# NRCan/geo-deep-learning

Hardware: AMD Instinct MI355X
Metric: 512x512 tiles/s, DOFA-base + UperNet, train step (higher is better)
Workload: dtype bf16; 1 GPU; DOFA-base + UperNet, 3-band 512x512 (configs[1]): training step = fwd + Dice(main)+0.4*Dice(aux) + bwd + clip 1.0 + Adam 6e-5, encoder frozen, DropPat; per_gpu_batch=64, global_batch=64, num_classes=5, parallelism=dp1, weights=random init, inputs_resident_in_hbm=True

## Files before the change

### geo-deep-learning_amd/csrc/attention_v2.hip

```cpp
#include "gdl_common.h"

namespace {

typedef __attribute__((ext_vector_type(4))) short s16x4_t;
typedef __attribute__((ext_vector_type(8))) short s16x8_t;
typedef __attribute__((address_space(3))) s16x4_t* lds_s16x4_ptr;

constexpr unsigned kOob = 0x80000000u;
constexpr int TILE_BYTES = 64 * 128;

__device__ __forceinline__ int tr_swz(int row) { return (((row >> 1) & 1) << 2) | ((row >> 2) & 3); }

__device__ __forceinline__ void decode_block(int nblk, int BH, int& blk, int& bh) {
  const int id = blockIdx.x;
  if ((BH & 7) == 0) {
    const int j = id >> 3;
    bh = (id & 7) + 8 * (j / nblk);
    blk = j % nblk;
  } else {
    bh = id / nblk;
    blk = id % nblk;
  }
}

struct Attn2Args {
  const uint16_t *q, *k, *v, *o, *dout;
  uint16_t *out, *dq, *dk, *dv;
  int64_t q_sB, q_sN, k_sB, k_sN, v_sB, v_sN, o_sB, o_sN, do_sB, do_sN;
  int64_t dq_sB, dq_sN, dk_sB, dk_sN, dv_sB, dv_sN;
  float* lse;
  float* dvec;
  int B, H, Nq, N;
  float scale, scale_log2e;
  int qsplit;
  float* dkv_part;
};

__device__ __forceinline__ void stage_piece(const srd_t& srd, int64_t tok_stride_bytes, int tok0, int ntok, int piece,
                                            unsigned lds_tile, int lane) {
  const int r = piece * 8 + (lane >> 3);
  const int chunk = (lane & 7) ^ tr_swz(r);
  const int tok = tok0 + r;
  const unsigned v = tok < ntok ? (unsigned)(tok * tok_stride_bytes + chunk * 16) : kOob;
  dma16_buf(v, srd, 0u, lds_tile + piece * 1024);
}

__device__ __forceinline__ bf16x8_t row_frag(const unsigned char* tile, int rt, int kk, int lane) {
  const int row = rt * 32 + (lane & 31);
  const uint4 v = *(const uint4*)(tile + row * 128 + (((2 * kk + (lane >> 5)) ^ tr_swz(row)) << 4));
  return __builtin_bit_cast(bf16x8_t, v);
}

__device__ __forceinline__ bf16x8_t col_frag(const unsigned char* tile, int ct, int tt, int s, int lane) {
  const int g = lane >> 4, l = lane & 15;
  const int ch = 32 * ct + 16 * (g & 1) + 4 * (l & 3);
  const int t0 = 32 * tt + 16 * s + 4 * (g >> 1) + (l >> 2);
  const unsigned char* p0 = tile + t0 * 128 + (((ch >> 3) ^ tr_swz(t0)) << 4) + (ch & 7) * 2;
  const int t1 = t0 + 8;
  const unsigned char* p1 = tile + t1 * 128 + (((ch >> 3) ^ tr_swz(t1)) << 4) + (ch & 7) * 2;
  const s16x4_t lo = __builtin_amdgcn_ds_read_tr16_b64_v4i16((lds_s16x4_ptr)p0);
  const s16x4_t hi = __builtin_amdgcn_ds_read_tr16_b64_v4i16((lds_s16x4_ptr)p1);
  const s16x8_t v = {lo[0], lo[1], lo[2], lo[3], hi[0], hi[1], hi[2], hi[3]};
  return __builtin_bit_cast(bf16x8_t, v);
}

__device__ __forceinline__ bf16x8_t acc_as_b(const f32x16_t& a, int s) {
  bf16x8_t r;
#pragma unroll
// ... 127 lines not shown
          ot[1][ct] = MFMA(va, pb1, ot[1][ct]);
        }
      }
  }
  if (!active) return;
#pragma unroll
  for (int qt = 0; qt < 2; ++qt) {
    const float l = l_run[qt] + __shfl_xor(l_run[qt], 32, 64);
    const float inv = 1.f / l;
    const int q = q0 + qt * 32 + frow;
    if (q >= f.Nq) continue;
    if (f.lse && fhalf == 0)
      f.lse[(int64_t)bh * f.Nq + q] = (m_run[qt] * f.scale_log2e + __builtin_amdgcn_logf(l)) * 0.6931471805599453f;
    uint16_t* orow = f.out + (int64_t)b * f.o_sB + (int64_t)q * f.o_sN + (int64_t)h * 64;
#pragma unroll
    for (int ct = 0; ct < 2; ++ct)
#pragma unroll
      for (int g = 0; g < 4; ++g) {
        const int d = ct * 32 + 8 * g + 4 * fhalf;
        *(uint2*)(orow + d) = make_uint2(pack_bf16x2(ot[qt][ct][4 * g] * inv, ot[qt][ct][4 * g + 1] * inv),
                                         pack_bf16x2(ot[qt][ct][4 * g + 2] * inv, ot[qt][ct][4 * g + 3] * inv));
      }
  }
}

template <int NW>
__global__ __launch_bounds__(64 * NW) __attribute__((amdgpu_waves_per_eu(NW == 2 ? 2 : 4, 4))) void flash_fwd3_kernel(const Attn2Args f, const float defer) {
  __shared__ __attribute__((aligned(16))) unsigned char smem[4 * TILE_BYTES];
  const int lane = threadIdx.x & 63;
  const int wave = __builtin_amdgcn_readfirstlane(threadIdx.x >> 6);
  int blk, bh;
  decode_block((f.Nq + 32 * NW - 1) / (32 * NW), f.B * f.H, blk, bh);
  const int b = bh / f.H, h = bh % f.H;
  const int q0 = blk * (32 * NW) + wave * 32;
  const bool active = q0 < f.Nq;
  const int frow = lane & 31, fhalf = lane >> 5;
  const uint16_t* qbase = f.q + (int64_t)b * f.q_sB + (int64_t)h * 64;
  const srd_t srd_k = make_srd(f.k + (int64_t)b * f.k_sB + (int64_t)h * 64, (unsigned)(((int64_t)f.N - 1) * f.k_sN * 2 + 128));
  const srd_t srd_v = make_srd(f.v + (int64_t)b * f.v_sB + (int64_t)h * 64, (unsigned)(((int64_t)f.N - 1) * f.v_sN * 2 + 128));
  const unsigned lds_base = __builtin_amdgcn_readfirstlane((unsigned)(size_t)(__attribute__((address_space(3))) void*)smem);

  bf16x8_t qf[4];
  {
    const int q = q0 + frow;
#pragma unroll
    for (int kk = 0; kk < 4; ++kk) {
      uint4 v = make_uint4(0, 0, 0, 0);
      if (q < f.Nq) v = *(const uint4*)(qbase + (int64_t)q * f.q_sN + kk * 16 + fhalf * 8);
      qf[kk] = __builtin_bit_cast(bf16x8_t, v);
    }
  }
  auto issue = [&](int stage, int kv0) {
#pragma unroll
    for (int i = 0; i < (8 + NW - 1) / NW; ++i) {
      const int p = wave + NW * i;
      if (p < 8) {
        stage_piece(srd_k, f.k_sN * 2, kv0, f.N, p, lds_base + (2 * stage) * TILE_BYTES, lane);
        stage_piece(srd_v, f.v_sN * 2, kv0, f.N, p, lds_base + (2 * stage + 1) * TILE_BYTES, lane);
      }
    }
  };
  f32x16_t ot[2] = {zero16(), zero16()};
  float m_run = -INFINITY, l_run = 0.f;
  const float sl2 = f.scale_log2e;
  const int ntiles = (f.N + 63) / 64;
  issue(0, 0);
// ... 431 lines not shown
    const float4 v = *(const float4*)(p + s * plane);
    a.x += v.x; a.y += v.y; a.z += v.z; a.w += v.w;
  }
  const int b = bh / f.H, h = bh % f.H;
  const bool is_v = d4 >= 16;
  const int d = (d4 & 15) * 4;
  uint16_t* dst = is_v ? f.dv + (int64_t)b * f.dv_sB + (int64_t)key * f.dv_sN + (int64_t)h * 64 + d
                       : f.dk + (int64_t)b * f.dk_sB + (int64_t)key * f.dk_sN + (int64_t)h * 64 + d;
  *(uint2*)dst = make_uint2(pack_bf16x2(a.x, a.y), pack_bf16x2(a.z, a.w));
}

int dkv_qsplit(int B, int H, int Nq, int Nkv) {
  const int64_t base = (int64_t)((Nkv + 127) / 128) * B * H;
  const int ntiles = (Nq + 63) / 64;
  int64_t s = (512 + base - 1) / base;
  if (s > ntiles / 4) s = ntiles / 4;
  if (s > 16) s = 16;
  return s < 1 ? 1 : (int)s;
}

bool strides_ok(int64_t a, int64_t b) { return a % 8 == 0 && b % 8 == 0; }

constexpr int kFlashFwdDefault = 3;
int g_flash_fwd = kFlashFwdDefault;
float g_flash_defer = 6.f;

}

extern "C" void gdl_debug_set_flash_fwd(int version, float defer) { g_flash_fwd = version < 0 ? kFlashFwdDefault : version; g_flash_defer = defer; }

extern "C" int gdl_flash_attn_fwd2(const void* q, int64_t q_sB, int64_t q_sN, const void* k, int64_t k_sB, int64_t k_sN,
                                   const void* v, int64_t v_sB, int64_t v_sN, void* o, int64_t o_sB, int64_t o_sN,
                                   float* lse, int B, int H, int Nq, int Nkv, float scale, gdl_stream_t stream) {
  GDL_CHECK_ARG(q && k && v && o, "gdl_flash_attn_fwd2: null pointer");
  GDL_CHECK_ARG(B > 0 && H > 0 && Nq > 0 && Nkv > 0, "gdl_flash_attn_fwd2: bad dims");
  GDL_CHECK_ARG(((uintptr_t)q % 16 == 0) && ((uintptr_t)k % 16 == 0) && ((uintptr_t)v % 16 == 0) && ((uintptr_t)o % 8 == 0) &&
                    strides_ok(q_sB, q_sN) && strides_ok(k_sB, k_sN) && strides_ok(v_sB, v_sN) && o_sB % 4 == 0 && o_sN % 4 == 0,
                "gdl_flash_attn_fwd2: pointers / strides must keep 16-byte alignment");
  GDL_CHECK_ARG(((int64_t)Nkv - 1) * k_sN * 2 + 128 < 0x7fffffffll && ((int64_t)Nkv - 1) * v_sN * 2 + 128 < 0x7fffffffll,
                "gdl_flash_attn_fwd2: one (batch, head) key / value slab spans more than 2 GiB");
  Attn2Args f = {};
  f.q = (const uint16_t*)q; f.k = (const uint16_t*)k; f.v = (const uint16_t*)v; f.out = (uint16_t*)o; f.lse = lse;
  f.q_sB = q_sB; f.q_sN = q_sN; f.k_sB = k_sB; f.k_sN = k_sN; f.v_sB = v_sB; f.v_sN = v_sN; f.o_sB = o_sB; f.o_sN = o_sN;
  f.B = B; f.H = H; f.Nq = Nq; f.N = Nkv;
  f.scale = scale; f.scale_log2e = scale * 1.4426950408889634f;
  const int nw = Nq > 128 ? 4 : 2;
  const unsigned grid = (unsigned)((Nq + 64 * nw - 1) / (64 * nw) * B * H);
  if (g_flash_fwd >= 4 && Nq > 64) {
    const dim3 g4((unsigned)((Nq + 127) / 128 * B * H));
    if (g_flash_fwd == 5) hipLaunchKernelGGL((flash_fwd4_kernel<4, true>), g4, dim3(256), 0, (hipStream_t)stream, f, g_flash_defer);
    else hipLaunchKernelGGL((flash_fwd4_kernel<4, false>), g4, dim3(256), 0, (hipStream_t)stream, f, g_flash_defer);
  } else if (g_flash_fwd >= 3) {
    if (Nq > 64) hipLaunchKernelGGL(flash_fwd3_kernel<4>, dim3((unsigned)((Nq + 127) / 128 * B * H)), dim3(256), 0, (hipStream_t)stream, f, g_flash_defer);
    else hipLaunchKernelGGL(flash_fwd3_kernel<2>, dim3((unsigned)((Nq + 63) / 64 * B * H)), dim3(128), 0, (hipStream_t)stream, f, g_flash_defer);
  } else if (nw == 4) hipLaunchKernelGGL(flash_fwd2_kernel<4>, dim3(grid), dim3(256), 0, (hipStream_t)stream, f);
  else hipLaunchKernelGGL(flash_fwd2_kernel<2>, dim3(grid), dim3(128), 0, (hipStream_t)stream, f);
  GDL_CHECK_LAUNCH("gdl_flash_attn_fwd2");
  return GDL_OK;
}

extern "C" int64_t gdl_flash_attn_bwd_workspace(int B, int H, int Nq, int Nkv) {
  if (B <= 0 || H <= 0 || Nq <= 0 || Nkv <= 0) return 0;
  const int s = dkv_qsplit(B, H, Nq, Nkv);
  return s > 1 ? (int64_t)s * B * H * Nkv * 128 * (int64_t)sizeof(float) : 0;
}

extern "C" int gdl_flash_attn_bwd(const void* q, int64_t q_sB, int64_t q_sN, const void* k, int64_t k_sB, int64_t k_sN,
                                  const void* v, int64_t v_sB, int64_t v_sN, const void* o, int64_t o_sB, int64_t o_sN,
                                  const void* dout, int64_t do_sB, int64_t do_sN, const float* lse, float* dvec,
                                  void* dq, int64_t dq_sB, int64_t dq_sN, void* dk, int64_t dk_sB, int64_t dk_sN,
                                  void* dv, int64_t dv_sB, int64_t dv_sN, int B, int H, int Nq, int Nkv, float scale,
                                  float* ws, int64_t ws_bytes, gdl_stream_t stream) {
  GDL_CHECK_ARG(q && k && v && o && dout && lse && dvec && dq && dk && dv, "gdl_flash_attn_bwd: null pointer");
  GDL_CHECK_ARG(B > 0 && H > 0 && Nq > 0 && Nkv > 0, "gdl_flash_attn_bwd: bad dims");
  GDL_CHECK_ARG(((uintptr_t)q % 16 == 0) && ((uintptr_t)k % 16 == 0) && ((uintptr_t)v % 16 == 0) && ((uintptr_t)dout % 16 == 0) &&
                    ((uintptr_t)dq % 8 == 0) && ((uintptr_t)dk % 8 == 0) && ((uintptr_t)dv % 8 == 0) &&
                    strides_ok(q_sB, q_sN) && strides_ok(k_sB, k_sN) && strides_ok(v_sB, v_sN) && strides_ok(do_sB, do_sN) &&
// ... 28 lines not shown
```

### geo-deep-learning_amd/csrc/conv3x3_sf.hip

```cpp
#include "conv_gemm_common.h"

using namespace gdlconv;

namespace {

template <typename T>
__global__ __launch_bounds__(512) void conv3x3_sf_kernel(const KArgs k) {
  constexpr int ES = TileTraits<T>::ES;
  constexpr int BKE = TileTraits<T>::BKE;
  constexpr int TM = 4, TN = 2, WARPS_N = 4;
  constexpr int BM = 256, BN = 256;
  constexpr int A_PIECES = 36;
  constexpr int A_BYTES = A_PIECES * 1024, B_BYTES = BN * 128;
  constexpr unsigned kOob = 0x80000000u;
  extern __shared__ __attribute__((aligned(16))) unsigned char smem[];

  const gdl_conv_args& a = k.a;
  const int tid = threadIdx.x, lane = tid & 63;
  const int wave = __builtin_amdgcn_readfirstlane(tid >> 6);
  const int wm = wave / WARPS_N, wn = wave % WARPS_N;
  const int lwave = wave & 3, half = wave >> 2;

  const int lid = xcd_remap(blockIdx.x, k.tiles_m * k.tiles_n);
  int tile_m, tile_n;
  tile_order(k, lid, tile_m, tile_n);
  const int m0 = tile_m * BM, n0 = tile_n * BN;
  const srd_t srd_a = make_srd(a.in, k.in_span);
  const srd_t srd_b = make_srd(a.w, k.w_span);
  const unsigned lds_base =
      __builtin_amdgcn_readfirstlane((unsigned)(size_t)(__attribute__((address_space(3))) void*)smem);
  const int W = a.W, HW = a.H * a.W;
  const int n_macro = k.kc * 3;
  const int KT = n_macro * 3;

  const int lrow = lane >> 3, lslot = lane & 7;
  unsigned b_voff[8];
#pragma unroll
  for (int i = 0; i < 8; ++i) {
    const int r = (i * 4 + lwave) * 8 + lrow;
    const int chunk = lslot ^ ((r >> 1) & 7);
    const int n = n0 + r;
    b_voff[i] = n < a.N ? (unsigned)((n * a.w_sN + chunk * (16 / ES)) * ES) : kOob;
  }
  auto issue_a = [&](int g, int part) {
    const int cc = g / 3, r = g - 3 * cc;
    const int q0 = m0 - 1 + (r - 1) * W;
    const unsigned lds = lds_base + (g & 1) * A_BYTES;
#pragma unroll
    for (int i = 0; i < 3; ++i) {
      const int p = part * 12 + lwave * 3 + i;
      const int j = p * 8 + lrow;
      const int chunk = lslot ^ ((j >> 1) & 7);
      const int q = q0 + j;
      const unsigned v = (unsigned)q < (unsigned)k.M ? (unsigned)((q * a.in_sW + cc * BKE + chunk * (16 / ES)) * ES)
                                                     : kOob;
      dma16_buf(v, srd_a, 0u, lds + p * 1024);
    }
  };
// ... 154 lines not shown
```

### geo-deep-learning_amd/csrc/conv_gemm.hip

```cpp
#include "conv_gemm_common.h"

using namespace gdlconv;

namespace {

typedef __attribute__((address_space(1))) const void* gptr_t;
typedef __attribute__((address_space(3))) void* lptr_t;

template <typename T, int WARPS_M, int WARPS_N, int TM, int TN, bool EXTRA, bool PP = false, bool CT = false,
          bool TP = false, bool TL = false, int S = 2>
__global__ __launch_bounds__(64 * WARPS_M * WARPS_N) void conv_gemm_kernel(const KArgs k) {
  constexpr int ES = TileTraits<T>::ES;
  constexpr int BKE = TileTraits<T>::BKE;
  constexpr int BM = WARPS_M * TM * 32, BN = WARPS_N * TN * 32;
  constexpr int NWALL = WARPS_M * WARPS_N;
  constexpr int NW = PP ? NWALL / 2 : NWALL;
  constexpr int CA = BM / (8 * NW), CB = BN / (8 * NW);
  static_assert(BM % (8 * NW) == 0 && BN % (8 * NW) == 0, "tile/waves mismatch");
  static_assert(!PP || NWALL == 8, "ping-pong needs two waves per SIMD");
  static_assert(!TP || (NW == 4 && !PP && !CT), "tap packing relies on the 4-wave DMA geometry");
  static_assert(S == 2 || (S == 4 && !PP && !TL), "two or four LDS stages; ping-pong loaders and the timeline probe use two");
  static_assert(S == 2 || 3 * (CA + CB) < 64, "vmcnt is a 6-bit counter");

  extern __shared__ __attribute__((aligned(16))) unsigned char smem[];
  constexpr int STAGE_BYTES = (BM + BN) * 128;

  const gdl_conv_args& a = k.a;
  const int tid = threadIdx.x, lane = tid & 63;
  const int wave = __builtin_amdgcn_readfirstlane(tid >> 6);
  const int wm = wave / WARPS_N, wn = wave % WARPS_N;

  const int lid = xcd_remap(blockIdx.x, k.tiles_m * k.tiles_n);
  int tile_m, tile_n;
  tile_order(k, lid, tile_m, tile_n);
  const int m0 = tile_m * BM, n0 = tile_n * BN;
  const int z = blockIdx.y;
  const int z0 = z / a.nz_inner, z1 = z % a.nz_inner;
  const int64_t out_zoff = z0 * a.out_sZ0 + z1 * a.out_sZ1;
  constexpr unsigned kOob = 0x80000000u;
  const srd_t srd_a = make_srd((const unsigned char*)a.in + (z0 * a.in_sZ0 + z1 * a.in_sZ1) * ES, k.in_span);
  const srd_t srd_b = make_srd((const unsigned char*)a.w + (z0 * a.w_sZ0 + z1 * a.w_sZ1) * ES, k.w_span);
  const unsigned lds_base =
      __builtin_amdgcn_readfirstlane((unsigned)(size_t)(__attribute__((address_space(3))) void*)smem);

  const int lrow = lane >> 3, lslot = lane & 7;
  const int lwave = PP ? (wave & 3) : wave;
  const int half = PP ? (wave >> 2) : 0;
  int a_voff[CA];
  unsigned a_mask[CA];
  unsigned a_tail = 0, b_tail = 0;
  const int tp_chunk = lslot ^ ((((lwave & 1) << 2) + (lrow >> 1)) & 7);
  const int tp_ppt = TP ? a.C / (16 / ES) : 1;
  const int tp_tap = tp_chunk / tp_ppt, tp_tpk = 8 / tp_ppt;
  const int HoWo = a.Ho * a.Wo;
#pragma unroll
  for (int i = 0; i < CA; ++i) {
    const int r = (i * NW + lwave) * 8 + lrow;
    const int chunk = TP ? tp_chunk % tp_ppt : lslot ^ ((r >> 1) & 7);
    if (CT && chunk * (16 / ES) < k.c_tail) a_tail |= 1u << i;
    const int m = m0 + r;
    const bool ok = m < k.M;
    const int mm = ok ? m : 0;
    if (k.in_dense) {
      a_voff[i] = ok ? (int)((mm * a.in_sW + chunk * (16 / ES)) * ES) : (int)kOob;
      a_mask[i] = ok ? 1u : 0u;
    } else {
      const int b = mm / HoWo, rem = mm - b * HoWo, oy = rem / a.Wo, ox = rem - oy * a.Wo;
// ... 246 lines not shown
extern "C" void gdl_debug_set_conv_korder(int tap_inner) { g_tap_inner = tap_inner; }

extern "C" int gdl_conv_gemm(const gdl_conv_args* ap, gdl_stream_t stream) {
  GDL_CHECK_ARG(ap != nullptr, "gdl_conv_gemm: null args");
  const gdl_conv_args& a = *ap;
  GDL_CHECK_ARG(a.dtype == GDL_F32 || a.dtype == GDL_BF16, "gdl_conv_gemm: bad dtype %d", a.dtype);
  GDL_CHECK_ARG(a.out_dtype == GDL_F32 || a.out_dtype == GDL_BF16, "gdl_conv_gemm: bad out_dtype");
  const int es = (int)gdl_elem_size(a.dtype);
  const int bke = 128 / es, al = 16 / es;
  GDL_CHECK_ARG(a.in && a.w && a.out, "gdl_conv_gemm: null tensor");
  GDL_CHECK_ARG(a.B > 0 && a.H > 0 && a.W > 0 && a.C > 0 && a.N > 0 && a.Ho > 0 && a.Wo > 0,
                "gdl_conv_gemm: non-positive dims");
  GDL_CHECK_ARG(a.R > 0 && a.S > 0 && a.stride > 0 && a.pad >= 0, "gdl_conv_gemm: bad filter");
  GDL_CHECK_ARG(a.C % al == 0, "gdl_conv_gemm: C=%d must be a multiple of %d", a.C, al);
  GDL_CHECK_ARG(a.in_sB % al == 0 && a.in_sH % al == 0 && a.in_sW % al == 0 && a.w_sN % al == 0 &&
                    a.in_sZ0 % al == 0 && a.in_sZ1 % al == 0 && a.w_sZ0 % al == 0 && a.w_sZ1 % al == 0,
                "gdl_conv_gemm: strides must keep 16-byte alignment");
  GDL_CHECK_ARG(((uintptr_t)a.in % 16 == 0) && ((uintptr_t)a.w % 16 == 0),
                "gdl_conv_gemm: operand pointers must be 16-byte aligned");
  GDL_CHECK_ARG(a.nz >= 1 && a.nz_inner >= 1, "gdl_conv_gemm: nz/nz_inner must be >= 1");
  GDL_CHECK_ARG(a.act >= GDL_ACT_NONE && a.act <= GDL_ACT_RESID_RELU, "gdl_conv_gemm: bad act %d", a.act);
  GDL_CHECK_ARG(a.act != GDL_ACT_RESID_RELU || a.resid, "gdl_conv_gemm: GDL_ACT_RESID_RELU needs `resid`");
  GDL_CHECK_ARG(a.act != GDL_ACT_MUL_GELU_GRAD || (a.resid && !a.aux_out),
                "gdl_conv_gemm: GDL_ACT_MUL_GELU_GRAD takes the pre-activation tensor in `resid`");
  GDL_CHECK_ARG((int64_t)a.B * a.Ho * a.Wo < (1ll << 31), "gdl_conv_gemm: M too large");
  GDL_CHECK_ARG(!a.stats_partial || gdl_conv_gemm_stats_rows(ap) > 0,
                "gdl_conv_gemm: stats_partial set on a call that cannot emit BatchNorm statistics (gdl_conv_gemm_stats_rows() == 0: "
                "needs bf16 in/out, bias-only epilogue, pixel-dense 16-byte aligned output, whole 128/256-row tiles)");
  GDL_CHECK_ARG(a.pad == 0 || a.R * a.S <= 32, "gdl_conv_gemm: padded filters are limited to 32 taps (got %dx%d)", a.R, a.S);
  const int64_t kSpanMax = 0x7ffffff0ll;
  const int64_t in_span = (((int64_t)a.B - 1) * a.in_sB + ((int64_t)a.H - 1) * a.in_sH + ((int64_t)a.W - 1) * a.in_sW + a.C) * es;
  const int64_t w_span = (((int64_t)a.N - 1) * a.w_sN + (int64_t)a.R * a.S * a.C) * es;
  GDL_CHECK_ARG(w_span <= kSpanMax, "gdl_conv_gemm: weight matrix spans more than 2 GiB");
  if (in_span > kSpanMax) {
    GDL_CHECK_ARG(a.B > 1 && a.nz == 1, "gdl_conv_gemm: one image spans more than 2 GiB");
    const int b1 = a.B / 2;
    const int64_t oes = (int64_t)gdl_elem_size(a.out_dtype);
    gdl_conv_args lo = a, hi = a;
    lo.B = b1;
    hi.B = a.B - b1;
    hi.in = (const unsigned char*)a.in + (int64_t)b1 * a.in_sB * es;
    hi.out = (unsigned char*)a.out + (int64_t)b1 * a.out_sB * oes;
    if (a.aux_out) hi.aux_out = (unsigned char*)a.aux_out + (int64_t)b1 * a.out_sB * oes;
    if (a.resid) hi.resid = (const unsigned char*)a.resid + (int64_t)b1 * a.res_sB * (int64_t)gdl_elem_size(a.resid_dtype);
    if (a.batch_scale) hi.batch_scale = a.batch_scale + b1;
    const int st = gdl_conv_gemm(&lo, stream);
    return st != GDL_OK ? st : gdl_conv_gemm(&hi, stream);
  }
  KArgs k;
  k.a = a;
  k.M = a.B * a.Ho * a.Wo;
  k.kc = (a.C + bke - 1) / bke;
  k.c_tail = a.C % bke;
  k.KT = a.R * a.S * k.kc;
  k.tap_inner = g_tap_inner;
  k.n_group = 0;
  k.tiles_m = k.tiles_n = 0;
  k.dbg = g_dbg;
  k.epi_v2 = g_epi_v2;
  k.probe = g_probe;
  k.in_span = (unsigned)in_span;
  k.w_span = (unsigned)w_span;
  k.in_dense = (a.R == 1 && a.S == 1 && a.stride == 1 && a.pad == 0 && a.H == a.Ho && a.W == a.Wo &&
                a.in_sH == (int64_t)a.W * a.in_sW && a.in_sB == (int64_t)a.H * a.in_sH);
  k.out_dense = (a.out_sH == (int64_t)a.Wo * a.out_sW && a.out_sB == (int64_t)a.Ho * a.out_sH);
  k.res_dense = !a.resid || (a.res_sH == (int64_t)a.Wo * a.res_sW && a.res_sB == (int64_t)a.Ho * a.res_sH);
  hipStream_t s = (hipStream_t)stream;
  const int variant = gdl_conv_gemm_plan(ap, nullptr);
  const bool tap_packed = g_tap_packing && variant == 5 && a.R * a.S > 1 && a.R * a.S <= 32 && !k.in_dense &&
                          a.C < bke && bke % a.C == 0 && a.C >= al;
  if (tap_packed) {
    k.kc = (a.R * a.S * a.C + bke - 1) / bke;
    k.KT = k.kc;
    k.c_tail = 0;
  }
  if (variant == 7) return conv3x3_narrow_launch(k, s);
  if (variant == 6) return conv_gemm_dual_launch(k, s);
  if (variant == 8) return conv_gemm_w4_launch(k, s);
  if (variant == 9) return conv_gemm_persist_launch(k, s);
  if (variant == 10) return conv_gemm_w4p_launch(k, s);
  if (variant == 12) {
    const bool extra = a.aux_out || a.act == GDL_ACT_MUL_GELU_GRAD;
    return extra ? launch_x<bf16_tag, 2, 2, 1, 1, true, false, false, false, false, 4>(k, s)
                 : launch_x<bf16_tag, 2, 2, 1, 1, false, false, false, false, false, 4>(k, s);
  }
  if (a.dtype == GDL_BF16) {
    if (variant == 4) return conv3x3_sf_launch(k, s);
    if (variant == 3 && k.dbg == 7) return launch_x<bf16_tag, 2, 4, 4, 2, false, true, false, false, true>(k, s);
    if (variant == 3) return launch_x<bf16_tag, 2, 4, 4, 2, false, true>(k, s);
    if (variant == 2) return launch_x<bf16_tag, 2, 4, 4, 2, false>(k, s);
    if (variant == 5 && tap_packed) return launch_x<bf16_tag, 4, 1, 2, 2, false, false, false, true>(k, s);
    if (variant == 5) return k.c_tail ? launch_x<bf16_tag, 4, 1, 2, 2, false, false, true>(k, s) : launch_x<bf16_tag, 4, 1, 2, 2, false>(k, s);
    if (variant == 1) return launch<bf16_tag, 2, 2, 2, 2>(k, s);
    return launch<bf16_tag, 2, 2, 1, 1>(k, s);
  }
  if (variant == 4) return conv3x3_sf_launch(k, s);
  if (variant == 3) return launch_x<float, 2, 4, 4, 2, false, true>(k, s);
  if (variant == 2) return launch_x<float, 2, 4, 4, 2, false>(k, s);
  if (variant == 5 && tap_packed) return launch_x<float, 4, 1, 2, 2, false, false, false, true>(k, s);
  if (variant == 5) return k.c_tail ? launch_x<float, 4, 1, 2, 2, false, false, true>(k, s) : launch_x<float, 4, 1, 2, 2, false>(k, s);
  if (variant == 1) return launch<float, 2, 2, 2, 2>(k, s);
  return launch<float, 2, 2, 1, 1>(k, s);
}

static std::atomic<int> g_forced_variant{-1};
static std::atomic<int> g_w4_enabled{1};
extern "C" void gdl_debug_set_conv_w4(int on) { g_w4_enabled = on; }
static std::atomic<int> g_persist_enabled{1};
extern "C" void gdl_debug_set_conv_persist(int on) { g_persist_enabled = on; }
static std::atomic<int> g_w4p_enabled{0};
static std::atomic<int> g_w4p_min_n{768};
extern "C" void gdl_debug_set_conv_w4p(int on) { g_w4p_enabled = on != 0; if (on > 1) g_w4p_min_n = on; }
// ... 86 lines not shown
```

### geo-deep-learning_amd/csrc/conv_gemm_common.h

```cpp
#pragma once
#include <type_traits>

#include "gdl_common.h"

namespace gdlconv {

struct KArgs {
  gdl_conv_args a;
  int M;
  int kc;
  int c_tail;
  int KT;
  int tiles_m, tiles_n;
  int n_group;
  int in_dense, out_dense, res_dense;
  unsigned in_span, w_span;
  unsigned out_span;
  int tap_inner;
  int dbg;
  int epi_v2;
  unsigned long long* probe;
};

template <typename T> struct TileTraits;
// ... 11 lines not shown
struct GeluTerms { float half_pe, e; };
__device__ __forceinline__ GeluTerms gelu_terms_fast(float x) {
  const float z = fabsf(x) * 0.70710678118654752440f;
  const float t = __builtin_amdgcn_rcpf(fmaf(0.3275911f, z, 1.0f));
  float p = fmaf(0.5f * 1.061405429f, t, 0.5f * -1.453152027f);
  p = fmaf(p, t, 0.5f * 1.421413741f);
  p = fmaf(p, t, 0.5f * -0.284496736f);
  p = fmaf(p, t, 0.5f * 0.254829592f);
  const float e = __builtin_amdgcn_exp2f(-1.44269504088896341f * z * z);
  return {p * t * e, e};
}
__device__ __forceinline__ float gelu_fast(float x) {
  const float h = gelu_terms_fast(x).half_pe;
  return __builtin_fmaf(-fabsf(x), h, fmaxf(x, 0.f));
}
__device__ __forceinline__ float gelu_grad_fast(float x) {
  const GeluTerms g = gelu_terms_fast(x);
  return (x >= 0.f ? 1.0f - g.half_pe : g.half_pe) + x * 0.3989422804014327f * g.e;
}
__device__ __forceinline__ float4 gelu4_fast(float4 v) {
  return make_float4(gelu_fast(v.x), gelu_fast(v.y), gelu_fast(v.z), gelu_fast(v.w));
}
__device__ __forceinline__ float4 mul_gelu_grad4_fast(float4 v, float4 u) {
  return make_float4(v.x * gelu_grad_fast(u.x), v.y * gelu_grad_fast(u.y), v.z * gelu_grad_fast(u.z),
                     v.w * gelu_grad_fast(u.w));
}

__device__ __forceinline__ int xcd_remap(int id, int n) {
  const int q = n >> 3, r = n & 7, xcd = id & 7, idx = id >> 3;
  return (xcd < r ? xcd * (q + 1) : r * (q + 1) + (xcd - r) * q) + idx;
}


__device__ __forceinline__ void tile_order(const KArgs& k, int lid, int& tile_m, int& tile_n) {
  const int ng = k.n_group;
  if (ng <= 0 || ng >= k.tiles_n) { tile_n = lid % k.tiles_n; tile_m = lid / k.tiles_n; return; }
  const int per_group = k.tiles_m * ng;
  const int g = lid / per_group, idx = lid - g * per_group;
  const int width = min(ng, k.tiles_n - g * ng);
  tile_m = idx / width;
  tile_n = g * ng + idx - tile_m * width;
}
int conv_n_group(const gdl_conv_args& a, int bm, int bn, int conc);

bool conv3x3_sf_applicable(const gdl_conv_args& a);
int conv3x3_sf_launch(const KArgs& k, hipStream_t stream);
bool conv_gemm_dual_applicable(const gdl_conv_args& a);
int conv_gemm_dual_launch(const KArgs& k, hipStream_t stream);
bool conv_gemm_w4_applicable(const gdl_conv_args& a);
int conv_gemm_w4_launch(const KArgs& k, hipStream_t stream);
bool conv_gemm_persist_applicable(const gdl_conv_args& a);
int conv_gemm_persist_launch(const KArgs& k, hipStream_t stream);
bool conv_gemm_w4p_applicable(const gdl_conv_args& a);
int conv_gemm_w4p_launch(const KArgs& k, hipStream_t stream);
bool conv3x3_narrow_applicable(const gdl_conv_args& a);
int conv3x3_narrow_launch(const KArgs& k, hipStream_t stream);


template <int TM, bool EXTRA>
__device__ __forceinline__ bool conv_epilogue_rows(const KArgs& k, f32x16_t (&acc)[TM][2], int m0, int n0, int wm,
                                                   int wn, int lane, int64_t out_zoff, unsigned char* lds,
                                                   unsigned char* ldc) {
  const gdl_conv_args& a = k.a;
  const bool out_bf16 = a.out_dtype == GDL_BF16;
  const bool mulgrad = EXTRA && a.act == GDL_ACT_MUL_GELU_GRAD;
  const bool plain = !a.resid && !a.batch_scale;
  const bool fast = a.dtype == GDL_BF16;
  const int HoWo = a.Ho * a.Wo;
  const bool vec_ok = ((uintptr_t)a.out % 16 == 0) && ((uintptr_t)a.aux_out % 16 == 0) && (a.out_sW % 8 == 0) &&
                      (out_zoff % 8 == 0) && (a.N % 16 == 0);
  const bool res_ok = !a.resid || (((uintptr_t)a.resid % 16 == 0) && (a.res_sW % 4 == 0));
  const bool vecs_ok = ((uintptr_t)a.bias % 16 == 0) && ((uintptr_t)a.scale % 16 == 0) && ((uintptr_t)a.shift % 16 == 0);
  if (!(k.out_dense && k.res_dense && vec_ok && res_ok && vecs_ok && (!a.batch_scale || HoWo >= 32))) return false;
  const int frow = lane & 31, fhalf = lane >> 5;
  const int n_w = n0 + wn * 64;
  const bool packed = plain && out_bf16;
  if (lane < 16) {
    const int n = n_w + 4 * lane;
    const bool in = n < a.N;
    float4 vb = make_float4(0.f, 0.f, 0.f, 0.f), vs = make_float4(1.f, 1.f, 1.f, 1.f), vh = vb;
    if (a.bias && in) vb = *(const float4*)(a.bias + n);
    if (a.scale && in) vs = *(const float4*)(a.scale + n);
    if (a.scale && a.shift && in) vh = *(const float4*)(a.shift + n);
    *(float4*)(ldc + lane * 16) = vb;
    if (a.scale) {
      *(float4*)(ldc + 256 + lane * 16) = vs;
      *(float4*)(ldc + 512 + lane * 16) = vh;
    }
  }
  asm volatile("s_waitcnt lgkmcnt(0)" ::: "memory");
  __builtin_amdgcn_wave_barrier();
  auto channel_terms = [&](const f32x16_t& cacc, int g, int c, float (&v)[4], float (&pre)[4]) {
    const float4 b4 = *(const float4*)(ldc + c * 4);
    const float b[4] = {b4.x, b4.y, b4.z, b4.w};
    float s[4] = {1.f, 1.f, 1.f, 1.f}, h[4] = {0.f, 0.f, 0.f, 0.f};
    if (a.scale) {
      const float4 s4 = *(const float4*)(ldc + 256 + c * 4), h4 = *(const float4*)(ldc + 512 + c * 4);
      s[0] = s4.x; s[1] = s4.y; s[2] = s4.z; s[3] = s4.w;
      h[0] = h4.x; h[1] = h4.y; h[2] = h4.z; h[3] = h4.w;
    }
#pragma unroll
    for (int e = 0; e < 4; ++e) {
      float x = cacc[4 * g + e] * a.alpha + b[e];
      pre[e] = x;
      if (a.scale) x = x * s[e] + h[e];
      if (a.act == GDL_ACT_RELU) x = fmaxf(x, 0.f);
      v[e] = x;
    }
    if (a.act == GDL_ACT_GELU) {
      const float4 t = fast ? gelu4_fast(make_float4(v[0], v[1], v[2], v[3])) : gelu4(make_float4(v[0], v[1], v[2], v[3]));
      v[0] = t.x; v[1] = t.y; v[2] = t.z; v[3] = t.w;
    }
  };
#pragma unroll
  for (int i = 0; i < TM; ++i) {
    const int mp = m0 + (wm * TM + i) * 32;
    if (mp >= k.M) break;
    float rv[8][4];
    float rs0 = 1.f, rs1 = 1.f;
    int rem0 = 0;
    if (!packed && !plain) {
      if (a.batch_scale) {
        const int b0 = mp / HoWo;
        rem0 = mp - b0 * HoWo;
        rs0 = a.batch_scale[b0];
        rs1 = b0 + 1 < a.B ? a.batch_scale[b0 + 1] : 0.f;
      }
#pragma unroll
      for (int t = 0; t < 8; ++t) {
        const int m = mp + (lane >> 4) + 4 * t, n = n_w + 4 * (lane & 15);
        rv[t][0] = rv[t][1] = rv[t][2] = rv[t][3] = 0.f;
        if (a.resid && m < k.M && n < a.N) {
          const int64_t ro = (int64_t)m * a.res_sW + n;
          if (a.resid_dtype == GDL_BF16) {
            const uint2 u = *(const uint2*)((const uint16_t*)a.resid + ro);
            rv[t][0] = __uint_as_float(u.x << 16); rv[t][1] = __uint_as_float(u.x & 0xffff0000u);
            rv[t][2] = __uint_as_float(u.y << 16); rv[t][3] = __uint_as_float(u.y & 0xffff0000u);
          } else {
            const float4 u = *(const float4*)((const float*)a.resid + ro);
            rv[t][0] = u.x; rv[t][1] = u.y; rv[t][2] = u.z; rv[t][3] = u.w;
          }
        }
      }
    }
    auto to_lds = [&](int which) {
#pragma unroll
      for (int j = 0; j < 2; ++j) {
        if (packed) {
#pragma unroll
          for (int p2 = 0; p2 < 2; ++p2) {
            float va[4], vb[4], pa[4], pb[4];
            channel_terms(acc[i][j], 2 * p2, 32 * j + 16 * p2 + 4 * fhalf, va, pa);
            channel_terms(acc[i][j], 2 * p2 + 1, 32 * j + 16 * p2 + 8 + 4 * fhalf, vb, pb);
            const float (&xa)[4] = which ? pa : va;
            const float (&xb)[4] = which ? pb : vb;
            unsigned a0 = pack_bf16x2(xa[0], xa[1]), a1 = pack_bf16x2(xa[2], xa[3]);
            unsigned b0 = pack_bf16x2(xb[0], xb[1]), b1 = pack_bf16x2(xb[2], xb[3]);
            const auto s0 = __builtin_amdgcn_permlane32_swap(a0, b0, false, false);
            const auto s1 = __builtin_amdgcn_permlane32_swap(a1, b1, false, false);
            const int slot = 4 * j + 2 * p2 + fhalf;
            *(uint4*)(lds + frow * 128 + ((slot ^ (frow & 7)) << 4)) = make_uint4(s0[0], s1[0], s0[1], s1[1]);
          }
        } else {
#pragma unroll
          for (int g = 0; g < 4; ++g) {
            float v[4], pre[4];
            channel_terms(acc[i][j], g, 32 * j + 8 * g + 4 * fhalf, v, pre);
            const float (&x)[4] = which ? pre : v;
            const int slot = 8 * j + 2 * g + fhalf;
            *(float4*)(lds + frow * 256 + ((slot ^ (frow & 7)) << 4)) = make_float4(x[0], x[1], x[2], x[3]);
          }
        }
      }
    };
    auto from_lds = [&](void* base, bool row_terms) {
      asm volatile("s_waitcnt lgkmcnt(0)" ::: "memory");
      __builtin_amdgcn_wave_barrier();
      if (packed) {
#pragma unroll
        for (int t = 0; t < 4; ++t) {
          const int rr = (lane >> 3) + 8 * t, slot = lane & 7;
          const uint4 v = *(const uint4*)(lds + rr * 128 + ((slot ^ (rr & 7)) << 4));
          const int m = mp + rr, n = n_w + 8 * slot;
          if (m < k.M && n < a.N) *(uint4*)((uint16_t*)base + (int64_t)m * a.out_sW + out_zoff + n) = v;
        }
      } else {
#pragma unroll
        for (int t = 0; t < 8; ++t) {
          const int rr = (lane >> 4) + 4 * t, slot = lane & 15;
          const float4 q = *(const float4*)(lds + rr * 256 + ((slot ^ (rr & 7)) << 4));
          float v[4] = {q.x, q.y, q.z, q.w};
          const int m = mp + rr, n = n_w + 4 * slot;
          if (m >= k.M || n >= a.N) continue;
          if (row_terms && !plain) {
            if (a.batch_scale) {
              const float rs = rem0 + rr >= HoWo ? rs1 : rs0;
#pragma unroll
              for (int e = 0; e < 4; ++e) v[e] *= rs;
            }
            if (EXTRA && mulgrad) {
              const float4 u = make_float4(rv[t][0], rv[t][1], rv[t][2], rv[t][3]);
              const float4 x = fast ? mul_gelu_grad4_fast(make_float4(v[0], v[1], v[2], v[3]), u)
                                    : mul_gelu_grad4(make_float4(v[0], v[1], v[2], v[3]), u);
              v[0] = x.x; v[1] = x.y; v[2] = x.z; v[3] = x.w;
            } else {
#pragma unroll
              for (int e = 0; e < 4; ++e) {
                float x = v[e] + rv[t][e];
                if (a.act == GDL_ACT_RESID_RELU) x = fmaxf(x, 0.f);
                v[e] = x;
              }
            }
          }
          const int64_t off = (int64_t)m * a.out_sW + out_zoff + n;
          if (out_bf16) *(uint2*)((uint16_t*)base + off) = make_uint2(pack_bf16x2(v[0], v[1]), pack_bf16x2(v[2], v[3]));
          else *(float4*)((float*)base + off) = make_float4(v[0], v[1], v[2], v[3]);
        }
      }
      __builtin_amdgcn_wave_barrier();
    };
    if (EXTRA && a.aux_out) {
      to_lds(1);
      from_lds(a.aux_out, false);
    }
    to_lds(0);
    from_lds(a.out, true);
  }
  return true;
}


#ifndef GDL_EPI_MASK
#define GDL_EPI_MASK 15
#endif
#define GDL_EPI_ON(bit) ((GDL_EPI_MASK & (bit)) != 0)
constexpr int EPI_RUNTIME = 0, EPI_FIXED = 1, EPI_SCALE = 2, EPI_DROPPATH = 4, EPI_RELU = 8, EPI_GELU = 16;
constexpr int EPI_STATS = 32;

template <int TM, int CH, bool RESID, int EF = EPI_RUNTIME>
__device__ __forceinline__ void conv_epilogue_rows2_impl(const KArgs& k, f32x16_t (&acc)[TM][2], int m0, int n0, int wm, int wn,
                                                        int lane, int64_t out_zoff, unsigned char* lds) {
#pragma clang fp contract(off)
  constexpr int NT = CH == 8 ? 4 : 8;
  constexpr int LPR = 64 / CH;
  const gdl_conv_args& a = k.a;
  constexpr bool RT = EF == EPI_RUNTIME;
  const bool has_scale = RT ? a.scale != nullptr : (EF & EPI_SCALE) != 0;
  const bool has_bs = RT ? a.batch_scale != nullptr : (EF & EPI_DROPPATH) != 0;
  const int act = RT ? a.act : (EF & EPI_RELU) ? GDL_ACT_RELU : (EF & EPI_GELU) ? GDL_ACT_GELU : GDL_ACT_NONE;
  const bool plain = !RESID && !has_bs;
  const bool fast = a.dtype == GDL_BF16;
  const int HoWo = a.Ho * a.Wo;
  const int frow = lane & 31, fhalf = lane >> 5;
  const int srow = lane / LPR, slot = lane % LPR;
  const int n_l = n0 + wn * 64 + CH * slot;
  float cb[CH], cs[CH], chh[CH];
#pragma unroll
  for (int e = 0; e < CH; ++e) { cb[e] = 0.f; cs[e] = 1.f; chh[e] = 0.f; }
  {
#pragma unroll
    for (int q = 0; q < CH / 4; ++q) {
      if (a.bias) { const float4 t = *(const float4*)(a.bias + n_l + 4 * q); cb[4 * q] = t.x; cb[4 * q + 1] = t.y; cb[4 * q + 2] = t.z; cb[4 * q + 3] = t.w; }
      if (has_scale) { const float4 t = *(const float4*)(a.scale + n_l + 4 * q); cs[4 * q] = t.x; cs[4 * q + 1] = t.y; cs[4 * q + 2] = t.z; cs[4 * q + 3] = t.w; }
      if (has_scale && a.shift) { const float4 t = *(const float4*)(a.shift + n_l + 4 * q); chh[4 * q] = t.x; chh[4 * q + 1] = t.y; chh[4 * q + 2] = t.z; chh[4 * q + 3] = t.w; }
    }
  }
  constexpr int RW = 4;
  constexpr int OES = CH == 8 ? 2 : 4;
  const int m_w = m0 + wm * TM * 32;
  const __amdgpu_buffer_rsrc_t res_rs = __builtin_amdgcn_make_buffer_rsrc(
      (void*)((const unsigned char*)a.resid + ((int64_t)m_w * a.res_sW + n0 + wn * 64) * OES), 0, 0x7fffffff, 0x00020000);
  const __amdgpu_buffer_rsrc_t out_rs = __builtin_amdgcn_make_buffer_rsrc(
      (void*)((unsigned char*)a.out + ((int64_t)m_w * a.out_sW + out_zoff + n0 + wn * 64) * OES), 0, 0x7fffffff, 0x00020000);
  const unsigned res_lo = (unsigned)((srow * (int)a.res_sW + CH * slot) * OES);
  const unsigned out_lo = (unsigned)((srow * (int)a.out_sW + CH * slot) * OES);
  typedef __attribute__((ext_vector_type(4))) unsigned epi_u4;
  auto load_resid_t = [&](int mp, int t, uint32_t (&rw)[NT][RW]) {
    const unsigned ru = (unsigned)((mp - m_w + (64 / LPR) * t) * (int)a.res_sW * OES);
    const epi_u4 u = __builtin_amdgcn_raw_buffer_load_b128(res_rs, res_lo, ru, 0);
    rw[t][0] = u.x; rw[t][1] = u.y; rw[t][2] = u.z; rw[t][3] = u.w;
  };
  auto resid_value = [&](const uint32_t (&w)[RW], int e) -> float {
    if constexpr (CH == 8) return __uint_as_float((e & 1) ? (w[e >> 1] & 0xffff0000u) : (w[e >> 1] << 16));
    else return __uint_as_float(w[e]);
  };
  float rs0 = 1.f, rs1 = 1.f;
  int rem0 = 0;
  if (has_bs) {
    const int b0 = m0 / HoWo;
    rem0 = m0 - b0 * HoWo;
    rs0 = a.batch_scale[b0];
    rs1 = b0 + 1 < a.B ? a.batch_scale[b0 + 1] : 0.f;
  }
  float st1[8] = {0.f, 0.f, 0.f, 0.f, 0.f, 0.f, 0.f, 0.f}, st2[8] = {0.f, 0.f, 0.f, 0.f, 0.f, 0.f, 0.f, 0.f};
  uint32_t rva[NT][RW];
  if constexpr (RESID) {
#pragma unroll
    for (int t = 0; t < NT; ++t) load_resid_t(m0 + wm * TM * 32, t, rva);
  }
#pragma unroll
  for (int i = 0; i < TM; ++i) {
    const int mp = m0 + (wm * TM + i) * 32;
#pragma unroll
    for (int j = 0; j < 2; ++j)
#pragma unroll
      for (int g = 0; g < 4; ++g) {
        const int sl = 8 * j + 2 * g + fhalf;
        *(float4*)(lds + frow * 256 + ((sl ^ (frow & 7)) << 4)) =
            make_float4(acc[i][j][4 * g], acc[i][j][4 * g + 1], acc[i][j][4 * g + 2], acc[i][j][4 * g + 3]);
      }
    asm volatile("s_waitcnt lgkmcnt(0)" ::: "memory");
    __builtin_amdgcn_wave_barrier();
#pragma unroll
    for (int t = 0; t < NT; ++t) {
      const int rr = srow + (64 / LPR) * t;
      float v[CH];
#pragma unroll
      for (int q = 0; q < CH / 4; ++q) {
        const int sl = (CH / 4) * slot + q;
        const float4 x = *(const float4*)(lds + rr * 256 + ((sl ^ (rr & 7)) << 4));
        v[4 * q] = x.x; v[4 * q + 1] = x.y; v[4 * q + 2] = x.z; v[4 * q + 3] = x.w;
      }
#pragma unroll
      for (int e = 0; e < CH; ++e) {
        float x = __builtin_fmaf(v[e], a.alpha, cb[e]);
        if (has_scale) x = __builtin_fmaf(x, cs[e], chh[e]);
        if (act == GDL_ACT_RELU) x = fmaxf(x, 0.f);
        v[e] = x;
      }
      if (act == GDL_ACT_GELU) {
#pragma unroll
        for (int q = 0; q < CH / 4; ++q) {
          const float4 x4 = make_float4(v[4 * q], v[4 * q + 1], v[4 * q + 2], v[4 * q + 3]);
          const float4 y4 = fast ? gelu4_fast(x4) : gelu4(x4);
          v[4 * q] = y4.x; v[4 * q + 1] = y4.y; v[4 * q + 2] = y4.z; v[4 * q + 3] = y4.w;
        }
      }
      if (!plain) {
        if (has_bs) {
          const float rs = rem0 + (wm * TM + i) * 32 + rr >= HoWo ? rs1 : rs0;
#pragma unroll
          for (int e = 0; e < CH; ++e) v[e] *= rs;
        }
        if constexpr (RESID) {
#pragma unroll
          for (int e = 0; e < CH; ++e) {
            float x = v[e] + resid_value(rva[t], e);
            if (act == GDL_ACT_RESID_RELU) x = fmaxf(x, 0.f);
            v[e] = x;
          }
          if (i + 1 < TM) load_resid_t(mp + 32, t, rva);
        }
      }
      const unsigned ou = (unsigned)((i * 32 + (64 / LPR) * t) * (int)a.out_sW * OES);
      epi_u4 o;
      if constexpr (CH == 8) {
        o = epi_u4{pack_bf16x2(v[0], v[1]), pack_bf16x2(v[2], v[3]), pack_bf16x2(v[4], v[5]), pack_bf16x2(v[6], v[7])};
      } else {
        o = epi_u4{__float_as_uint(v[0]), __float_as_uint(v[1]), __float_as_uint(v[2]), __float_as_uint(v[3])};
      }
      if constexpr ((EF & EPI_STATS) != 0 && CH == 8) {
        const uint32_t ow[4] = {o.x, o.y, o.z, o.w};
#pragma unroll
        for (int e = 0; e < 4; ++e) {
          const float lo = __uint_as_float(ow[e] << 16), hi = __uint_as_float(ow[e] & 0xffff0000u);
          st1[2 * e] += lo; st2[2 * e] = __builtin_fmaf(lo, lo, st2[2 * e]);
          st1[2 * e + 1] += hi; st2[2 * e + 1] = __builtin_fmaf(hi, hi, st2[2 * e + 1]);
        }
      }
      __builtin_amdgcn_raw_buffer_store_b128(o, out_rs, out_lo + ou, 0, 0);
    }
    __builtin_amdgcn_wave_barrier();
  }
  if constexpr ((EF & EPI_STATS) != 0 && CH == 8) {
#pragma unroll
    for (int e = 0; e < 8; ++e) {
#pragma unroll
      for (int o2 = 8; o2 < 64; o2 <<= 1) { st1[e] += __shfl_xor(st1[e], o2, 64); st2[e] += __shfl_xor(st2[e], o2, 64); }
    }
    if (lane < 8) {
      const int64_t row = (int64_t)(m0 + wm * TM * 32) / (TM * 32);
      float* dst = a.stats_partial + (row * 2) * a.N + n0 + wn * 64 + lane * 8;
      *(float4*)dst = make_float4(st1[0], st1[1], st1[2], st1[3]);
      *(float4*)(dst + 4) = make_float4(st1[4], st1[5], st1[6], st1[7]);
      *(float4*)(dst + a.N) = make_float4(st2[0], st2[1], st2[2], st2[3]);
      *(float4*)(dst + a.N + 4) = make_float4(st2[4], st2[5], st2[6], st2[7]);
    }
  }
}

template <int TM>
__device__ __forceinline__ bool conv_epilogue_rows2(const KArgs& k, f32x16_t (&acc)[TM][2], int m0, int n0, int wm, int wn, int lane,
                                                   int64_t out_zoff, unsigned char* lds) {
  const gdl_conv_args& a = k.a;
  const bool out_bf16 = a.out_dtype == GDL_BF16;
  const int HoWo = a.Ho * a.Wo;
  const bool vec_ok = ((uintptr_t)a.out % 16 == 0) && (a.out_sW % 8 == 0) && (out_zoff % 8 == 0) && (a.N % 16 == 0);
  const bool res_ok = !a.resid || (((uintptr_t)a.resid % 16 == 0) && (a.res_sW % 8 == 0) && (a.resid_dtype == a.out_dtype));
  const bool vecs_ok = ((uintptr_t)a.bias % 16 == 0) && ((uintptr_t)a.scale % 16 == 0) && ((uintptr_t)a.shift % 16 == 0);
  if (!k.epi_v2 || a.aux_out || a.act == GDL_ACT_MUL_GELU_GRAD ||
      !(k.out_dense && k.res_dense && vec_ok && res_ok && vecs_ok && (!a.batch_scale || HoWo >= 256)))
    return false;
  if (m0 + (wm + 1) * TM * 32 > k.M || n0 + (wn + 1) * 64 > a.N) return false;
  const bool sc = a.scale != nullptr, bs = a.batch_scale != nullptr, rs = a.resid != nullptr;
  if (a.stats_partial) {
    conv_epilogue_rows2_impl<TM, 8, false, EPI_FIXED | EPI_STATS>(k, acc, m0, n0, wm, wn, lane, out_zoff, lds);
    return true;
  }
  if (k.epi_v2 != 2) {
    if (GDL_EPI_ON(1) && !rs && !bs && !sc && a.act == GDL_ACT_NONE) {
      if (out_bf16) conv_epilogue_rows2_impl<TM, 8, false, EPI_FIXED>(k, acc, m0, n0, wm, wn, lane, out_zoff, lds);
      else conv_epilogue_rows2_impl<TM, 4, false, EPI_FIXED>(k, acc, m0, n0, wm, wn, lane, out_zoff, lds);
      return true;
    }
    if (GDL_EPI_ON(2) && !rs && !bs && !sc && a.act == GDL_ACT_GELU && out_bf16) {
      conv_epilogue_rows2_impl<TM, 8, false, EPI_FIXED | EPI_GELU>(k, acc, m0, n0, wm, wn, lane, out_zoff, lds);
      return true;
    }
    if (GDL_EPI_ON(4) && !rs && !bs && sc && a.act == GDL_ACT_RELU && out_bf16) {
      conv_epilogue_rows2_impl<TM, 8, false, EPI_FIXED | EPI_SCALE | EPI_RELU>(k, acc, m0, n0, wm, wn, lane, out_zoff, lds);
      return true;
    }
    if (GDL_EPI_ON(8) && rs && sc && a.act == GDL_ACT_NONE && !out_bf16) {
      if (bs) conv_epilogue_rows2_impl<TM, 4, true, EPI_FIXED | EPI_SCALE | EPI_DROPPATH>(k, acc, m0, n0, wm, wn, lane, out_zoff, lds);
      else conv_epilogue_rows2_impl<TM, 4, true, EPI_FIXED | EPI_SCALE>(k, acc, m0, n0, wm, wn, lane, out_zoff, lds);
      return true;
    }
  }
  if (a.resid) {
    if (out_bf16) conv_epilogue_rows2_impl<TM, 8, true>(k, acc, m0, n0, wm, wn, lane, out_zoff, lds);
    else conv_epilogue_rows2_impl<TM, 4, true>(k, acc, m0, n0, wm, wn, lane, out_zoff, lds);
  } else {
    if (out_bf16) conv_epilogue_rows2_impl<TM, 8, false>(k, acc, m0, n0, wm, wn, lane, out_zoff, lds);
    else conv_epilogue_rows2_impl<TM, 4, false>(k, acc, m0, n0, wm, wn, lane, out_zoff, lds);
  }
  return true;
}

template <int TM, int TN, bool EXTRA>
__device__ __forceinline__ void conv_epilogue(const KArgs& k, f32x16_t (&acc)[TM][TN], int m0, int n0, int wm, int wn,
                                              int lane, int64_t out_zoff, unsigned char* lds_wave = nullptr,
                                              unsigned char* lds_consts = nullptr) {
  const gdl_conv_args& a = k.a;
  const int frow = lane & 31, fhalf = lane >> 5;
  const int HoWo = a.Ho * a.Wo;
  if constexpr (TN == 2) {
    if (lds_wave && conv_epilogue_rows2<TM>(k, acc, m0, n0, wm, wn, lane, out_zoff, lds_wave)) return;
    if (lds_wave && conv_epilogue_rows<TM, EXTRA>(k, acc, m0, n0, wm, wn, lane, out_zoff, lds_wave, lds_consts)) return;
  }
  const bool out_bf16 = a.out_dtype == GDL_BF16;
  const int oes = out_bf16 ? 2 : 4;
  const bool mulgrad = EXTRA && a.act == GDL_ACT_MUL_GELU_GRAD;
  const bool plain = !a.resid && !a.batch_scale;
  const bool vec_ok = ((uintptr_t)a.out % 16 == 0) && ((uintptr_t)a.aux_out % 16 == 0) && (a.out_sW % 8 == 0) &&
                      (a.out_sH % 8 == 0) && (a.out_sB % 8 == 0) && (out_zoff % 8 == 0) && (a.N % 16 == 0);
  const bool res_vec = !a.resid || (((uintptr_t)a.resid % 16 == 0) && (a.res_sW % 4 == 0) && (a.res_sH % 4 == 0) &&
                                    (a.res_sB % 4 == 0));
  int64_t row_o[TM], row_r[TM];
  float row_s[TM];
  bool m_ok[TM];
#pragma unroll
  for (int i = 0; i < TM; ++i) {
    const int m = m0 + (wm * TM + i) * 32 + frow;
    m_ok[i] = m < k.M;
    row_s[i] = 1.f;
    if (k.out_dense && k.res_dense && !a.batch_scale) {
      row_o[i] = (int64_t)m * a.out_sW + out_zoff;
      row_r[i] = (int64_t)m * a.res_sW;
    } else {
      const int mm = m_ok[i] ? m : 0;
      const int b = mm / HoWo, rem = mm - b * HoWo, oy = rem / a.Wo, ox = rem - oy * a.Wo;
      row_o[i] = (int64_t)b * a.out_sB + (int64_t)oy * a.out_sH + (int64_t)ox * a.out_sW + out_zoff;
      row_r[i] = (int64_t)b * a.res_sB + (int64_t)oy * a.res_sH + (int64_t)ox * a.res_sW;
      if (a.batch_scale) row_s[i] = a.batch_scale[b];
    }
  }
  auto load4 = [&](const float* p, int n, float dflt, float (&o)[4]) {
    if (!p) { o[0] = o[1] = o[2] = o[3] = dflt; return; }
    if (n + 3 < a.N && ((uintptr_t)p % 16 == 0)) {
      const float4 t = *(const float4*)(p + n);
      o[0] = t.x; o[1] = t.y; o[2] = t.z; o[3] = t.w;
    } else {
#pragma unroll
      for (int e = 0; e < 4; ++e) o[e] = n + e < a.N ? p[n + e] : dflt;
    }
  };
  auto finish = [&](int i, int j, int g, int n, const float (&bias4)[4], const float (&sc4)[4], const float (&sh4)[4],
                    float (&v)[4], float (&pre)[4]) {
#pragma unroll
    for (int e = 0; e < 4; ++e) {
      float x = acc[i][j][4 * g + e] * a.alpha + bias4[e];
      pre[e] = x;
      if (a.scale) x = x * sc4[e] + sh4[e];
      if (a.act == GDL_ACT_RELU) x = fmaxf(x, 0.f);
      v[e] = x;
    }
    if (a.act == GDL_ACT_GELU) {
      const float4 t = gelu4(make_float4(v[0], v[1], v[2], v[3]));
      v[0] = t.x; v[1] = t.y; v[2] = t.z; v[3] = t.w;
    }
    if (!plain && m_ok[i]) {
      float rv[4] = {0.f, 0.f, 0.f, 0.f};
      if (a.resid) {
        const int64_t ro = row_r[i] + n;
// ... 98 lines not shown
```

### geo-deep-learning_amd/csrc/conv_gemm_dual.hip

```cpp
#include "conv_gemm_common.h"

using namespace gdlconv;

namespace {

constexpr int DBM = 256, DBN = 128;
constexpr int A_STAGE = DBM * 128;
constexpr int B_OFF = 2 * A_STAGE;
constexpr int DUAL_LDS = B_OFF + DBN * 128;

template <bool DENSE>
__global__ __launch_bounds__(256, 2) void conv_gemm_dual_kernel(const KArgs k) {
  constexpr int ES = 2, BKE = 64;
  constexpr int TM = 4, TN = 2, WARPS_N = 2;
  constexpr int CA = 8, CB = 4;
  constexpr unsigned kOob = 0x80000000u;
  extern __shared__ __attribute__((aligned(16))) unsigned char smem[];

  const gdl_conv_args& a = k.a;
  const int tid = threadIdx.x, lane = tid & 63;
  const int wave = __builtin_amdgcn_readfirstlane(tid >> 6);
  const int wm = wave / WARPS_N, wn = wave % WARPS_N;

  const int lid = xcd_remap(blockIdx.x, k.tiles_m * k.tiles_n);
  int tile_m, tile_n;
  tile_order(k, lid, tile_m, tile_n);
  const int m0 = tile_m * DBM, n0 = tile_n * DBN;
  const int z = blockIdx.y;
  const int z0 = z / a.nz_inner, z1 = z % a.nz_inner;
  const int64_t out_zoff = z0 * a.out_sZ0 + z1 * a.out_sZ1;
  const srd_t srd_a = make_srd((const unsigned char*)a.in + (z0 * a.in_sZ0 + z1 * a.in_sZ1) * ES, k.in_span);
  const srd_t srd_b = make_srd((const unsigned char*)a.w + (z0 * a.w_sZ0 + z1 * a.w_sZ1) * ES, k.w_span);
  const unsigned lds_base =
      __builtin_amdgcn_readfirstlane((unsigned)(size_t)(__attribute__((address_space(3))) void*)smem);
  if (k.dbg == 8 && (lid & 1)) __builtin_amdgcn_s_setprio(1);
  if ((k.dbg == 9 || k.dbg == 10) && blockIdx.x < 512 && blockIdx.y == 0) {
    const unsigned slot = (blockIdx.x >> 3) & 63;
    const unsigned long long period = (unsigned long long)k.KT * 2600 + 12000;
    const unsigned long long wait = k.dbg == 9 ? (slot >= 32 ? period / 2 : 0) : period * slot / 64;
    const unsigned long long t_end = __builtin_readcyclecounter() + wait;
    while (__builtin_readcyclecounter() < t_end) __builtin_amdgcn_s_sleep(16);
  }

  const int lrow = lane >> 3, lslot = lane & 7;
  const int HoWo = a.Ho * a.Wo;
  int a_voff[CA];
  unsigned a_mask[DENSE ? 1 : CA];
#pragma unroll
  for (int i = 0; i < CA; ++i) {
    const int r = (i * 4 + wave) * 8 + lrow;
    const int chunk = lslot ^ ((r >> 1) & 7);
    const int m = m0 + r;
    const bool ok = m < k.M;
    const int mm = ok ? m : 0;
    if constexpr (DENSE) {
      a_voff[i] = ok ? (int)((mm * a.in_sW + chunk * 8) * ES) : (int)kOob;
    } else {
      const int b = mm / HoWo, rem = mm - b * HoWo, oy = rem / a.Wo, ox = rem - oy * a.Wo;
      const int iy0 = oy * a.stride - a.pad, ix0 = ox * a.stride - a.pad;
// ... 151 lines not shown
```

### geo-deep-learning_amd/csrc/conv_gemm_persist.hip

```cpp
#include "conv_gemm_common.h"

using namespace gdlconv;

namespace {

constexpr int PS_STAGE = 65536;
constexpr int PS_LDS = 2 * PS_STAGE + 8192;

__global__ __launch_bounds__(512) void conv_gemm_persist_kernel(const KArgs) {
  constexpr int ES = 2;
  constexpr int TM = 4, TN = 2, WARPS_N = 4;
  extern __shared__ __attribute__((aligned(16))) unsigned char smem[];
  typedef const __attribute__((address_space(4))) KArgs* kargs_ptr;
  using yes = std::integral_constant<bool, true>;
  using no = std::integral_constant<bool, false>;

  f32x16_t acc[TM][TN];
  int v = blockIdx.x;
  bool first_tile = true;
  for (;;) {
    kargs_ptr kp = (kargs_ptr)__builtin_amdgcn_kernarg_segment_ptr();
    int tid = threadIdx.x;
    asm volatile("" : "+s"(kp), "+v"(tid));
    const KArgs& k = *(const KArgs*)kp;
    const gdl_conv_args& a = k.a;
    const int lane = tid & 63;
    const int wave = __builtin_amdgcn_readfirstlane(tid >> 6);
    const int wm = wave / WARPS_N, wn = wave % WARPS_N;
    const int ntiles = k.tiles_m * k.tiles_n;
    const srd_t srd_a = make_srd(a.in, k.in_span);
    const srd_t srd_b = make_srd(a.w, k.w_span);
    const unsigned lds_base =
        __builtin_amdgcn_readfirstlane((unsigned)(size_t)(__attribute__((address_space(3))) void*)smem);

    const int lrow = lane >> 3, lslot = lane & 7;
    const int lwave = wave & 3, half = wave >> 2;
    const int chunk = lslot ^ ((((lwave & 1) << 2) + (lrow >> 1)) & 7);
    const unsigned a_row = (unsigned)a.in_sW * ES, b_row = (unsigned)a.w_sN * ES;
    const unsigned a_lane = (unsigned)(lwave * 8 + lrow) * a_row + chunk * 16;
    const unsigned b_lane = (unsigned)(lwave * 8 + lrow) * b_row + chunk * 16;
    auto issue = [&](int stage, unsigned a_v, unsigned b_v, unsigned wk) {
      const unsigned lds_a = lds_base + stage * PS_STAGE + lwave * 1024;
      const unsigned lds_b = lds_a + 256 * 128;
#pragma unroll
      for (int i = 0; i < 8; ++i) dma16_buf(a_v + i * 32 * a_row, srd_a, wk, lds_a + i * 4096);
#pragma unroll
      for (int i = 0; i < 8; ++i) dma16_buf(b_v + i * 32 * b_row, srd_b, wk, lds_b + i * 4096);
    };

    const int frow = lane & 31, fhalf = lane >> 5;
    const int fswz = (frow >> 1) & 7;
    const int a_lds0 = (wm * TM * 32 + frow) * 128;
    const int b_lds0 = 256 * 128 + (wn * TN * 32 + frow) * 128;
    uint4 fa[2][TM], fb[2][TN];
    auto fetch = [&](const unsigned char* st, int kk, int buf) {
      const int coff = (((2 * kk + fhalf) ^ fswz) << 4);
#pragma unroll
      for (int i = 0; i < TM; ++i) fa[buf][i] = *(const uint4*)(st + a_lds0 + i * 32 * 128 + coff);
#pragma unroll
      for (int j = 0; j < TN; ++j) fb[buf][j] = *(const uint4*)(st + b_lds0 + j * 32 * 128 + coff);
    };
    auto mfmas = [&](int buf, auto first) {
      constexpr bool FIRST = decltype(first)::value;
      const f32x16_t zero = {0.f, 0.f, 0.f, 0.f, 0.f, 0.f, 0.f, 0.f, 0.f, 0.f, 0.f, 0.f, 0.f, 0.f, 0.f, 0.f};
#pragma unroll
      for (int i = 0; i < TM; ++i)
#pragma unroll
        for (int j = 0; j < TN; ++j)
          acc[i][j] = __builtin_amdgcn_mfma_f32_32x32x16_bf16(__builtin_bit_cast(bf16x8_t, fb[buf][j]),
                                                              __builtin_bit_cast(bf16x8_t, fa[buf][i]), FIRST ? zero : acc[i][j], 0, 0, 0);
    };

    int tile_m, tile_n;
    tile_order(k, xcd_remap(v, ntiles), tile_m, tile_n);
    const int m0 = tile_m * 256, n0 = tile_n * 256;
    const unsigned a_v = a_lane + (unsigned)m0 * a_row, b_v = b_lane + (unsigned)n0 * b_row;
    if (first_tile && half == 0) issue(0, a_v, b_v, 0u);
    first_tile = false;

    const unsigned long long t0c = k.probe ? __builtin_readcyclecounter() : 0;
    const unsigned long long t0r = k.probe ? __builtin_amdgcn_s_memrealtime() : 0;
    if (half == 0) asm volatile("s_waitcnt vmcnt(0)" ::: "memory");
    __syncthreads();
    if (k.KT > 1 && half == 1) issue(1, a_v, b_v, 128u);
    __builtin_amdgcn_s_waitcnt(0xC07F);
    fetch(smem, 0, 0);
    auto kstep = [&](auto first, int kt) {
      const unsigned char* st = smem + (kt & 1) * PS_STAGE;
#pragma unroll
      for (int kk = 0; kk < 3; ++kk) {
        fetch(st, kk + 1, (kk + 1) & 1);
        __builtin_amdgcn_sched_barrier(0);
        if (kk == 0) mfmas(0, first); else mfmas(kk & 1, no{});
        __builtin_amdgcn_sched_barrier(0);
      }
      if (kt + 1 < k.KT) {
        asm volatile("s_waitcnt vmcnt(0)" ::: "memory");
        __syncthreads();
        if (kt + 2 < k.KT && half == (kt & 1)) issue(kt & 1, a_v, b_v, (unsigned)(kt + 2) * 128u);
        fetch(smem + ((kt + 1) & 1) * PS_STAGE, 0, 0);
      }
      __builtin_amdgcn_sched_barrier(0);
      mfmas(1, no{});
      __builtin_amdgcn_sched_barrier(0);
    };
    kstep(yes{}, 0);
    for (int kt = 1; kt < k.KT; ++kt) kstep(no{}, kt);
    if (k.probe && tid == 0 && v < 2048) {
      k.probe[2 * v] = __builtin_readcyclecounter() - t0c;
      k.probe[2 * v + 1] = __builtin_amdgcn_s_memrealtime() - t0r;
    }
    __syncthreads();
    const int vn = v + (int)gridDim.x;
    const bool more = vn < ntiles;
    if (more && half == 0 && k.dbg != 11) {
      int tm2, tn2;
      tile_order(k, xcd_remap(vn, ntiles), tm2, tn2);
      issue(0, a_lane + (unsigned)(tm2 * 256) * a_row, b_lane + (unsigned)(tn2 * 256) * b_row, 0u);
    }
    {
      kargs_ptr kq = (kargs_ptr)__builtin_amdgcn_kernarg_segment_ptr();
      int tid_e = threadIdx.x, m0_e = m0, n0_e = n0;
      asm volatile("" : "+s"(kq), "+v"(tid_e), "+s"(m0_e), "+s"(n0_e));
      const KArgs& ke = *(const KArgs*)kq;
      const int wave_e = __builtin_amdgcn_readfirstlane(tid_e >> 6);
      conv_epilogue<TM, TN, false>(ke, acc, m0_e, n0_e, wave_e / WARPS_N, wave_e % WARPS_N, tid_e & 63, 0,
                                   smem + PS_STAGE + wave_e * 8192, smem + 2 * PS_STAGE + wave_e * 1024);
      if (ke.probe && tid_e == 0 && v < 2048) {
        ke.probe[4096 + v] = __builtin_readcyclecounter() - t0c;
        ke.probe[8192 + 2 * v] = t0r;
        ke.probe[8192 + 2 * v + 1] = __builtin_amdgcn_s_memrealtime();
      }
      if (!more) break;
      if (ke.dbg == 11 && wave_e < 4) first_tile = true;
    }
    v = vn;
  }
}

int num_cus() {
  static int n = [] {
    int dev = 0, cus = 0;
    if (hipGetDevice(&dev) != hipSuccess || hipDeviceGetAttribute(&cus, hipDeviceAttributeMultiprocessorCount, dev) != hipSuccess || cus <= 0)
      cus = 256;
    return cus;
  }();
  return n;
}

}
// ... 25 lines not shown
```

### geo-deep-learning_amd/csrc/conv_gemm_w4.hip

```cpp
#include "conv_gemm_common.h"

using namespace gdlconv;

namespace {

constexpr int W4_STAGE = 65536;
constexpr int W4_LDS = 2 * W4_STAGE;

template <bool DENSE>
__global__ __launch_bounds__(256) __attribute__((amdgpu_waves_per_eu(1, 1))) void conv_gemm_w4_kernel(const KArgs k) {
  constexpr int ES = 2, BKE = 64;
  constexpr unsigned kOob = 0x80000000u;
  extern __shared__ __attribute__((aligned(16))) unsigned char smem[];

  const gdl_conv_args& a = k.a;
  const int tid = threadIdx.x, lane = tid & 63;
  const int wave = __builtin_amdgcn_readfirstlane(tid >> 6);
  const int wm = wave >> 1, wn = wave & 1;

  const int lid = xcd_remap(blockIdx.x, k.tiles_m * k.tiles_n);
  int tile_m, tile_n;
  tile_order(k, lid, tile_m, tile_n);
  const int m0 = tile_m * 256, n0 = tile_n * 256;
  const int z = blockIdx.y;
  const int z0 = z / a.nz_inner, z1 = z % a.nz_inner;
  const int64_t out_zoff = z0 * a.out_sZ0 + z1 * a.out_sZ1;
  const srd_t srd_a = make_srd((const unsigned char*)a.in + (z0 * a.in_sZ0 + z1 * a.in_sZ1) * ES, k.in_span);
  const srd_t srd_b = make_srd((const unsigned char*)a.w + (z0 * a.w_sZ0 + z1 * a.w_sZ1) * ES, k.w_span);
  const unsigned lds_base =
      __builtin_amdgcn_readfirstlane((unsigned)(size_t)(__attribute__((address_space(3))) void*)smem);

  const int lrow = lane >> 3, lslot = lane & 7;
  const int HoWo = a.Ho * a.Wo;
  int a_voff[8];
  unsigned a_mask[DENSE ? 1 : 8];
  unsigned b_voff[8];
#pragma unroll
  for (int i = 0; i < 8; ++i) {
    const int r = (i * 4 + wave) * 8 + lrow;
    const int chunk = lslot ^ ((r >> 1) & 7);
    const int m = m0 + r;
    const bool ok = m < k.M;
    const int mm = ok ? m : 0;
    if constexpr (DENSE) {
      a_voff[i] = ok ? (int)((mm * a.in_sW + chunk * 8) * ES) : (int)kOob;
    } else {
      const int b = mm / HoWo, rem = mm - b * HoWo, oy = rem / a.Wo, ox = rem - oy * a.Wo;
      const int iy0 = oy * a.stride - a.pad, ix0 = ox * a.stride - a.pad;
      a_voff[i] = (int)((b * a.in_sB + iy0 * a.in_sH + ix0 * a.in_sW + chunk * 8) * ES);
      unsigned mask = 0;
      if (ok) {
        if (a.pad == 0) {
          mask = 0xffffffffu;
        } else {
          for (int tr = 0; tr < a.R; ++tr)
// ... 170 lines not shown
```

### geo-deep-learning_amd/csrc/conv_gemm_w4p.hip

```cpp
#include "conv_gemm_common.h"

using namespace gdlconv;

namespace {

constexpr int P_STAGE = 65536;
constexpr int P_LDS = 2 * P_STAGE;

typedef __attribute__((ext_vector_type(4))) unsigned pu4;

template <int V> using ic = std::integral_constant<int, V>;
using yes = std::integral_constant<bool, true>;
using no = std::integral_constant<bool, false>;

template <bool SR, bool ST, bool K12>
__global__ __launch_bounds__(256) __attribute__((amdgpu_waves_per_eu(1, 1))) void conv_gemm_w4p_kernel(const KArgs k) {
#pragma clang fp contract(off)
  constexpr int ES = 2;
  constexpr int CH = 8;
  constexpr int OES = 2;
  constexpr int LPR = 64 / CH;
  constexpr int RPG = 64 / LPR;
  constexpr int NT = 32 / RPG;
  constexpr int HW = 4;
// ... 216 lines not shown
      if constexpr (p + 1 < 8) wr(ic<p + 1>{});
      __builtin_amdgcn_wave_barrier();
      if constexpr (p < 8) rd(pc);
      __builtin_amdgcn_wave_barrier();
      if constexpr (p >= 1) fin(ic<p - 1>{});
    };
    wr(ic<0>{});
    iter(ic<0>{}); iter(ic<1>{}); iter(ic<2>{}); iter(ic<3>{}); iter(ic<4>{}); iter(ic<5>{}); iter(ic<6>{}); iter(ic<7>{}); iter(ic<8>{});
    if constexpr (ST) {
#pragma unroll
      for (int h = 0; h < 2; ++h) {
#pragma unroll
        for (int e = 0; e < 8; ++e) {
#pragma unroll
          for (int o2 = 8; o2 < 64; o2 <<= 1) { st1[h][e] += __shfl_xor(st1[h][e], o2, 64); st2[h][e] += __shfl_xor(st2[h][e], o2, 64); }
        }
        if (lane < 8) {
          const int64_t row = (int64_t)(m0 + wm * 128) / 128;
          float* dst = a.stats_partial + (row * 2) * a.N + n_w + h * 64 + lane * 8;
          *(float4*)dst = make_float4(st1[h][0], st1[h][1], st1[h][2], st1[h][3]);
          *(float4*)(dst + 4) = make_float4(st1[h][4], st1[h][5], st1[h][6], st1[h][7]);
          *(float4*)(dst + a.N) = make_float4(st2[h][0], st2[h][1], st2[h][2], st2[h][3]);
          *(float4*)(dst + a.N + 4) = make_float4(st2[h][4], st2[h][5], st2[h][6], st2[h][7]);
        }
      }
    }
    d_out_lane = (unsigned)(m0 + wm * 128 + srow) * ((unsigned)a.out_sW * OES) + (unsigned)((n_w + CH * slot) * OES);
    d_span = k.out_span;
  };

  int v = blockIdx.x;
  {
    int tm, tn;
    tile_order(k, xcd_remap(v, ntiles), tm, tn);
    unsigned a_lane, b_lane;
    lane_ab(a_lane, b_lane);
    a_v = a_lane + (unsigned)(tm * 256) * a_row;
    b_v = b_lane + (unsigned)(tn * 256) * b_row;
    cc = 0;
    begin_kstep();
    const Fresh f = fresh();
#pragma unroll
    for (int p = 0; p < 16; ++p) piece_at(f, 0, p, a_v, b_v, cur_wk);
  }
  for (;;) {
    int tile_m, tile_n;
    tile_order(k, xcd_remap(v, ntiles), tile_m, tile_n);
    const int m0 = tile_m * 256, n0 = tile_n * 256;
    cc = 1;
    const unsigned long long t0c = k.probe ? __builtin_readcyclecounter() : 0;
    const unsigned long long t0r = k.probe ? __builtin_amdgcn_s_memrealtime() : 0;
    asm volatile("s_waitcnt vmcnt(0)" ::: "memory");
    __builtin_amdgcn_s_barrier();
    {
      begin_kstep();
      const Fresh f = fresh();
#pragma unroll
      for (int p = 0; p < 4; ++p) piece_at(f, 1, p, a_v, b_v, cur_wk);
    }
    __builtin_amdgcn_s_waitcnt(0xC07F);
    {
      unsigned fab0, fbb0;
      frag_bases(fab0, fbb0);
#pragma unroll
      for (int i = 0; i < 4; ++i) {
        fa[0][i] = *(const uint4*)(smem + fab0 + i * 4096);
        fb[0][i] = *(const uint4*)(smem + fbb0 + i * 4096);
      }
    }
#pragma unroll
    for (int h = 0; h < 2; ++h)
#pragma unroll
      for (int i = 0; i < 4; ++i)
#pragma unroll
        for (int j = 0; j < 2; ++j)
#pragma unroll
          for (int r = 0; r < 16; ++r) acc[h][i][j][r] = 0.f;

    step(yes{}, yes{}, ic<0>{}, 0); step(yes{}, yes{}, ic<1>{}, 1); step(yes{}, yes{}, ic<2>{}, 2); step(yes{}, yes{}, ic<3>{}, 3);
    step(yes{}, yes{}, ic<4>{}, 4); step(yes{}, yes{}, ic<5>{}, 5); step(yes{}, yes{}, ic<6>{}, 6); step(yes{}, yes{}, ic<7>{}, 7);
    step(yes{}, yes{}, ic<8>{}, 8); step(yes{}, yes{}, ic<9>{}, 9);
    if constexpr (K12) {
      step(yes{}, no{}, ic<10>{}, 10);
      step(no{}, no{}, ic<-1>{}, 11);
    } else {
      step(yes{}, yes{}, ic<10>{}, 10);
      int kt = 11;
      for (; kt + 2 < k.KT; ++kt) step(yes{}, yes{}, ic<-1>{}, kt);
      step(yes{}, no{}, ic<-1>{}, kt); ++kt;
      step(no{}, no{}, ic<-1>{}, kt);
    }
    if (k.probe && tid == 0 && v < 2048) {
      k.probe[2 * v] = __builtin_readcyclecounter() - t0c;
      k.probe[2 * v + 1] = __builtin_amdgcn_s_memrealtime() - t0r;
    }
    __builtin_amdgcn_s_barrier();
    const int vn = v + (int)gridDim.x;
    const bool more = vn < ntiles;
    if (more) {
      int tm2, tn2;
      tile_order(k, xcd_remap(vn, ntiles), tm2, tn2);
      unsigned a_lane, b_lane;
      lane_ab(a_lane, b_lane);
      a_v = a_lane + (unsigned)(tm2 * 256) * a_row;
      b_v = b_lane + (unsigned)(tn2 * 256) * b_row;
      const Fresh f = fresh();
#pragma unroll
      for (int p = 0; p < 16; ++p) piece_at(f, 0, p, a_v, b_v, 0u);
    }
    if (k.dbg != 21) park(m0, n0);
    if (k.dbg == 20) d_span = 0;
    if (k.probe && tid == 0 && v < 2048) {
      k.probe[4096 + v] = __builtin_readcyclecounter() - t0c;
      k.probe[8192 + 2 * v] = t0r;
      k.probe[8192 + 2 * v + 1] = __builtin_amdgcn_s_memrealtime();
    }
    if (!more) break;
    v = vn;
  }
  const Fresh f = fresh();
  auto all = [&](auto self, auto uc) {
    constexpr int u = decltype(uc)::value;
    if constexpr (u < UNITS) { drain_store(f, uc); self(self, ic<u + 1>{}); }
  };
  all(all, ic<0>{});
}

int num_cus() {
  static int n = [] {
    int dev = 0, cus = 0;
    if (hipGetDevice(&dev) != hipSuccess || hipDeviceGetAttribute(&cus, hipDeviceAttributeMultiprocessorCount, dev) != hipSuccess || cus <= 0)
      cus = 256;
    return cus;
  }();
// ... 65 lines not shown
```

### geo-deep-learning_amd/csrc/misc.hip

```cpp
#include <type_traits>

#include <atomic>
#include <cmath>

#include "gdl_common.h"
#include "bilinear_index.h"

namespace {

template <typename T>
__global__ __launch_bounds__(256) void v_transpose_kernel(const T* __restrict__ v, int N, int H, int hd,
                                                          int64_t v_sB, int64_t v_sN, T* __restrict__ vt, int Npad) {
  __shared__ T tile[32][33];
  const int bh = blockIdx.z, b = bh / H, h = bh % H;
  const int n0 = blockIdx.x * 32, d0 = blockIdx.y * 32;
  const int tx = threadIdx.x & 31, ty = threadIdx.x >> 5;
  const int64_t rowstride = v_sN;
  const T* src = v + (int64_t)b * v_sB + (int64_t)h * hd;
  for (int j = ty; j < 32; j += 8) {
    const int n = n0 + j, d = d0 + tx;
    tile[j][tx] = (n < N && d < hd) ? src[(int64_t)n * rowstride + d] : (T)0;
  }
  __syncthreads();
  T* dst = vt + ((int64_t)bh * hd) * Npad;
// ... 1348 lines not shown

extern "C" int gdl_clip_coef(const float* sumsq, float max_norm, float* coef, gdl_stream_t stream) {
  GDL_CHECK_ARG(sumsq && coef, "gdl_clip_coef: null pointer");
  hipLaunchKernelGGL(clip_coef_kernel, dim3(1), dim3(1), 0, (hipStream_t)stream, sumsq, max_norm, coef);
  GDL_CHECK_LAUNCH("gdl_clip_coef");
  return GDL_OK;
}

extern "C" int gdl_adam_step(float* p, const float* g, float* m, float* v, int64_t n, float lr, float beta1,
                             float beta2, float eps, float weight_decay, float bc1, float bc2,
                             const float* clip_coef, gdl_stream_t stream) {
  GDL_CHECK_ARG(p && g && m && v, "gdl_adam_step: null pointer");
  if (n <= 0) return GDL_OK;
  hipLaunchKernelGGL(adam_kernel, dim3(grid_for(n, 1024)), dim3(256), 0, (hipStream_t)stream, p, g, m, v, n, lr, beta1, beta2,
                     eps, weight_decay, bc1, bc2, clip_coef);
  GDL_CHECK_LAUNCH("gdl_adam_step");
  return GDL_OK;
}

extern "C" int gdl_iou_counts(const int64_t* pred, const int64_t* target, int B, int64_t P, int K, int64_t* counts,
                              gdl_stream_t stream) {
  GDL_CHECK_ARG(pred && target && counts && B > 0 && P > 0, "gdl_iou_counts: bad args");
  GDL_CHECK_ARG(K > 0 && K <= 64, "gdl_iou_counts: 1..64 classes");
  GDL_CHECK_ARG(P / 64 < (1ll << 32), "gdl_iou_counts: sample too large");
  hipStream_t s = (hipStream_t)stream;
  (void)hipMemsetAsync(counts, 0, (size_t)B * 3 * K * sizeof(int64_t), s);
  int64_t chunks = (P + 65535) / 65536;
  if (chunks > 1024) chunks = 1024;
  hipLaunchKernelGGL(iou_counts_kernel, dim3((unsigned)chunks, B), dim3(256), 0, s, pred, target, P, K,
                     (unsigned long long*)counts);
  GDL_CHECK_LAUNCH("gdl_iou_counts");
  return GDL_OK;
}
```

### geo-deep-learning_amd/csrc/norm.hip

```cpp
#include "gdl_common.h"

namespace {

template <int VPL>
__global__ __launch_bounds__(256) void layernorm_fwd_kernel(const float* __restrict__ x,
                                                            int64_t x_stride,
                                                            const float* __restrict__ gamma,
                                                            const float* __restrict__ beta, void* y,
                                                            int y_dtype, int64_t rows, int D,
                                                            float eps) {
  const int lane = threadIdx.x & 63;
  const int lpp = (VPL == 1 && D <= 128) ? (D <= 64 ? 16 : 32) : 64;
  const int nsub = 64 / lpp, cl = lane % lpp;
  const int64_t row = ((int64_t)blockIdx.x * 4 + (threadIdx.x >> 6)) * nsub + lane / lpp;
  if (row >= rows) return;
  auto group_sum = [&](float t) {
    for (int o = lpp >> 1; o > 0; o >>= 1) t += __shfl_xor(t, o, 64);
    return t;
  };
  const float* xr = x + row * x_stride;
  float4 v[VPL];
  float s = 0.f;
#pragma unroll
  for (int i = 0; i < VPL; ++i) {
    const int c = (i * 64 + cl) * 4;
    v[i] = c < D ? *(const float4*)(xr + c) : make_float4(0, 0, 0, 0);
    s += (v[i].x + v[i].y) + (v[i].z + v[i].w);
  }
  const float mean = group_sum(s) / (float)D;
  float q = 0.f;
#pragma unroll
  for (int i = 0; i < VPL; ++i) {
    const int c = (i * 64 + cl) * 4;
    if (c < D) {
      const float a = v[i].x - mean, b = v[i].y - mean, cc = v[i].z - mean, d = v[i].w - mean;
      q += (a * a + b * b) + (cc * cc + d * d);
    }
  }
  const float rstd = rsqrtf(group_sum(q) / (float)D + eps);
#pragma unroll
  for (int i = 0; i < VPL; ++i) {
    const int c = (i * 64 + cl) * 4;
    if (c >= D) continue;
    const float4 g = *(const float4*)(gamma + c), b = *(const float4*)(beta + c);
    const float o0 = (v[i].x - mean) * rstd * g.x + b.x, o1 = (v[i].y - mean) * rstd * g.y + b.y;
    const float o2 = (v[i].z - mean) * rstd * g.z + b.z, o3 = (v[i].w - mean) * rstd * g.w + b.w;
    if (y_dtype == GDL_BF16) {
      *(uint2*)((uint16_t*)y + row * D + c) = make_uint2(pack_bf16x2(o0, o1), pack_bf16x2(o2, o3));
    } else {
      *(float4*)((float*)y + row * D + c) = make_float4(o0, o1, o2, o3);
    }
  }
}
// ... 881 lines not shown
  if (n > 2048 / cg) n = 2048 / cg;
  return (int)n;
}

int bn_gelu_blocks(int64_t P, int C, int dtype) {
  const int G = C / (dtype == GDL_BF16 ? 8 : 4), R = BNG_T / G;
  int64_t n = P / (4 * R);
  if (n > 4096) n = 4096;
  if (n < 1) n = 1;
  return (int)n;
}

bool bn_gelu_shape_ok(int dtype, int C, int64_t a, int64_t b, int64_t c, const void* p0, const void* p1, const void* p2) {
  const int v = dtype == GDL_BF16 ? 8 : 4;
  return (dtype == GDL_F32 || dtype == GDL_BF16) && C > 0 && C % v == 0 && C / v <= BNG_T && a % v == 0 && b % v == 0 && c % v == 0 &&
         (uintptr_t)p0 % 16 == 0 && (uintptr_t)p1 % 16 == 0 && (uintptr_t)p2 % 16 == 0;
}

}

extern "C" void gdl_debug_set_bn_wide(int on) { g_bn_wide = on; }

extern "C" int gdl_layernorm_fwd(const float* x, int64_t x_stride, const float* gamma,
                                 const float* beta, void* y, int y_dtype, int64_t rows, int D, float eps,
                                 gdl_stream_t stream) {
  GDL_CHECK_ARG(x && gamma && beta && y, "gdl_layernorm_fwd: null pointer");
  GDL_CHECK_ARG(D > 0 && D % 4 == 0 && D <= 2048, "gdl_layernorm_fwd: D=%d must be a multiple of 4, <= 2048", D);
  GDL_CHECK_ARG(x_stride % 4 == 0, "gdl_layernorm_fwd: x_stride must be a multiple of 4");
  if (rows <= 0) return GDL_OK;
  hipStream_t s = (hipStream_t)stream;
  const int rpb = 4 * (D <= 64 ? 4 : (D <= 128 ? 2 : 1));
  const unsigned grid = (unsigned)((rows + rpb - 1) / rpb);
  const int vpl = (D + 255) / 256;
#define LN_LAUNCH(V) hipLaunchKernelGGL(layernorm_fwd_kernel<V>, dim3(grid), dim3(256), 0, s, x, x_stride, gamma, beta, y, y_dtype, rows, D, eps)
  if (vpl <= 1) LN_LAUNCH(1);
  else if (vpl <= 2) LN_LAUNCH(2);
  else if (vpl <= 4) LN_LAUNCH(4);
  else LN_LAUNCH(8);
#undef LN_LAUNCH
  GDL_CHECK_LAUNCH("gdl_layernorm_fwd");
  return GDL_OK;
}

extern "C" int64_t gdl_bn_stats_workspace(int64_t P, int C) {
  return (int64_t)bn_nsplit(P, C) * 2 * C * sizeof(float);
}

extern "C" int gdl_bn_small_fwd(const void* x, void* y, int dtype, int64_t P, int C, int64_t x_sP, int64_t y_sP, const float* gamma,
                                const float* beta, float eps, int relu, float* mean, float* var, float* running_mean,
                                float* running_var, float momentum, gdl_stream_t stream) {
  GDL_CHECK_ARG(x && y && gamma && beta && mean && var, "gdl_bn_small_fwd: null pointer");
  GDL_CHECK_ARG(dtype == GDL_F32 || dtype == GDL_BF16, "gdl_bn_small_fwd: bad dtype");
  GDL_CHECK_ARG(C % 4 == 0 && x_sP % 4 == 0 && y_sP % 4 == 0 && P > 0, "gdl_bn_small_fwd: C and strides must be multiples of 4");
  if (dtype == GDL_BF16)
    hipLaunchKernelGGL(bn_small_fwd_kernel<uint16_t>, dim3(C / 4), dim3(BNS_T), 0, (hipStream_t)stream, x, y, P, C, x_sP, y_sP, gamma, beta,
                       eps, relu, mean, var, running_mean, running_var, momentum);
  else
    hipLaunchKernelGGL(bn_small_fwd_kernel<float>, dim3(C / 4), dim3(BNS_T), 0, (hipStream_t)stream, x, y, P, C, x_sP, y_sP, gamma, beta,
                       eps, relu, mean, var, running_mean, running_var, momentum);
  GDL_CHECK_LAUNCH("gdl_bn_small_fwd");
  return GDL_OK;
}

extern "C" int gdl_bn_small_bwd(const void* x, const void* dy, void* dx, int dtype, int64_t P, int C, int64_t x_sP, int64_t dy_sP,
                                int64_t dx_sP, const float* mean, const float* var, const float* gamma, const float* beta, float eps,
                                int relu, float* dgamma, float* dbeta, gdl_stream_t stream) {
  GDL_CHECK_ARG(x && dy && dx && mean && var && gamma && beta && dgamma && dbeta, "gdl_bn_small_bwd: null pointer");
  GDL_CHECK_ARG(dtype == GDL_F32 || dtype == GDL_BF16, "gdl_bn_small_bwd: bad dtype");
  GDL_CHECK_ARG(C % 4 == 0 && x_sP % 4 == 0 && dy_sP % 4 == 0 && dx_sP % 4 == 0 && P > 0, "gdl_bn_small_bwd: C and strides must be multiples of 4");
  if (dtype == GDL_BF16)
    hipLaunchKernelGGL(bn_small_bwd_kernel<uint16_t>, dim3(C / 4), dim3(BNS_T), 0, (hipStream_t)stream, x, dy, dx, P, C, x_sP, dy_sP, dx_sP,
                       mean, var, gamma, beta, eps, relu, dgamma, dbeta);
  else
// ... 234 lines not shown
```

### geo-deep-learning_amd/gdlhip/_lib.py

```python

from __future__ import annotations

import ctypes as C
import os
from pathlib import Path

LIB_PATH = Path(os.environ.get("GDL_LIB_PATH") or Path(__file__).resolve().parent / "libgdlhip.so")

F32, BF16 = 0, 1
ACT_NONE, ACT_RELU, ACT_GELU, ACT_MUL_GELU_GRAD, ACT_RESID_RELU = 0, 1, 2, 3, 4

c_i, c_l, c_f, c_p = C.c_int, C.c_int64, C.c_float, C.c_void_p


class ConvArgs(C.Structure):

    _fields_ = [
        ("inp", c_p), ("dtype", c_i), ("B", c_i), ("H", c_i), ("W", c_i), ("C", c_i),
        ("in_sB", c_l), ("in_sH", c_l), ("in_sW", c_l),
        ("Ho", c_i), ("Wo", c_i), ("R", c_i), ("S", c_i), ("stride", c_i), ("pad", c_i),
        ("w", c_p), ("w_sN", c_l), ("N", c_i),
        ("out", c_p), ("out_dtype", c_i), ("out_sB", c_l), ("out_sH", c_l), ("out_sW", c_l),
        ("alpha", c_f), ("bias", c_p), ("scale", c_p), ("shift", c_p), ("act", c_i),
        ("batch_scale", c_p), ("resid", c_p), ("resid_dtype", c_i),
        ("res_sB", c_l), ("res_sH", c_l), ("res_sW", c_l),
        ("nz", c_i), ("nz_inner", c_i),
        ("in_sZ0", c_l), ("in_sZ1", c_l), ("w_sZ0", c_l), ("w_sZ1", c_l),
        ("out_sZ0", c_l), ("out_sZ1", c_l),
        ("aux_out", c_p), ("stats_partial", c_p),
    ]


class WgradArgs(C.Structure):

    _fields_ = [
        ("inp", c_p), ("dy", c_p), ("dtype", c_i), ("B", c_i), ("H", c_i), ("W", c_i), ("C", c_i),
        ("in_sB", c_l), ("in_sH", c_l), ("in_sW", c_l),
        ("Ho", c_i), ("Wo", c_i), ("R", c_i), ("S", c_i), ("stride", c_i), ("pad", c_i),
        ("N", c_i), ("dy_sB", c_l), ("dy_sH", c_l), ("dy_sW", c_l),
        ("dw", c_p), ("dw_sN", c_l), ("accumulate", c_i),
        ("workspace", c_p), ("workspace_bytes", c_l),
        ("nz", c_i), ("nz_inner", c_i),
        ("in_sZ0", c_l), ("in_sZ1", c_l), ("dy_sZ0", c_l), ("dy_sZ1", c_l), ("dw_sZ0", c_l), ("dw_sZ1", c_l),
    ]


class DiceOptions(C.Structure):

    _fields_ = [
        ("has_ignore_index", c_i), ("ignore_index", c_l), ("smooth", c_f), ("log_loss", c_i),
        ("classes", C.POINTER(c_i)), ("num_classes", c_i),
    ]


OVERLAP_JACCARD, OVERLAP_TVERSKY = 1, 2


class OverlapOptions(C.Structure):

    _fields_ = [
        ("kind", c_i), ("has_ignore", c_i), ("ignore_index", c_l), ("smooth", c_f), ("log_loss", c_i),
        ("alpha", c_f), ("beta", c_f), ("gamma", c_f), ("classes", C.POINTER(c_i)), ("nclasses", c_i),
    ]


FOCAL_AUTO, FOCAL_GATHER, FOCAL_TILE = 0, 1, 2
_FOCAL_OPT = (c_f, c_i, c_f, c_i, c_f, c_i, c_l, c_i)
_LOVASZ_OPT = (c_i, c_i, c_l)

SIGNATURES = {
    "gdl_version": (c_i, []),
    "gdl_last_error": (C.c_char_p, []),
    "gdl_conv_gemm": (c_i, [C.POINTER(ConvArgs), c_p]),
    "gdl_conv_gemm_plan": (c_i, [C.POINTER(ConvArgs), C.POINTER(c_l)]),
    "gdl_conv_gemm_stats_rows": (c_l, [C.POINTER(ConvArgs)]),
    "gdl_conv_wgrad_workspace": (c_l, [C.POINTER(WgradArgs)]),
    "gdl_conv_wgrad": (c_i, [C.POINTER(WgradArgs), c_p]),
    "gdl_layernorm_fwd": (c_i, [c_p, c_l, c_p, c_p, c_p, c_i, c_l, c_i, c_f, c_p]),
    "gdl_colreduce_workspace": (c_l, [c_l, c_i, c_i]),
    "gdl_layernorm_bwd": (c_i, [c_p, c_l, c_p, c_i, c_p, c_p, c_l, c_p, c_l, c_l, c_i, c_f, c_p, c_p, c_i, c_p, c_l,
                                c_p]),
    "gdl_colsum": (c_i, [c_p, c_i, c_l, c_i, c_l, c_p, c_i, c_p, c_l, c_p]),
    "gdl_layerscale_bwd": (c_i, [c_p, c_p, c_i, c_p, c_p, c_l, c_l, c_i, c_p, c_i, c_p, c_i, c_p, c_l, c_p]),
    "gdl_softmax_bwd_rows": (c_i, [c_p, c_p, c_p, c_i, c_l, c_i, c_i, c_f, c_p]),
    "gdl_dwconv3x3_gelu_bwd": (c_i, [c_p, c_p, c_i, c_i, c_i, c_i, c_i, c_p, c_p, c_p, c_p, c_p, c_i, c_p, c_l,
                                     c_p]),
    "gdl_col2im": (c_i, [c_p, c_i, c_i, c_i, c_i, c_i, c_i, c_i, c_i, c_i, c_i, c_i, c_p, c_i, c_l, c_l, c_l, c_p]),
    "gdl_chan_weights_fwd": (c_i, [c_p, c_i, c_i, c_i, c_i, c_i, c_p, c_p, c_p, c_p, c_p, c_l, c_p, c_p, c_p, c_p, c_p]),
    "gdl_chan_weights_bwd": (c_i, [c_p, c_i, c_i, c_i, c_i, c_i, c_p, c_p, c_p, c_p, c_p, c_p, c_p, c_p, c_p, c_p, c_p,
                                   c_p]),
    "gdl_chan_pool_fwd": (c_i, [c_p, c_i, c_i, c_l, c_i, c_i, c_p, c_p, c_l, c_p, c_p, c_f, c_p, c_p, c_p]),
    "gdl_chan_pool_workspace": (c_l, [c_i, c_i, c_l, c_i, c_i]),
    "gdl_chan_pool_bwd": (c_i, [c_p, c_i, c_i, c_l, c_i, c_i, c_p, c_p, c_l, c_p, c_p, c_f, c_p, c_p, c_p, c_p, c_l,
                                c_p]),
    "gdl_maxpool3x3s2_fwd": (c_i, [c_p, c_i, c_i, c_i, c_i, c_i, c_l, c_l, c_l, c_p, c_l, c_l, c_l, c_p]),
    "gdl_maxpool3x3s2_bwd": (c_i, [c_p, c_p, c_p, c_i, c_i, c_i, c_i, c_i, c_l, c_l, c_l, c_l, c_l, c_l, c_l, c_l, c_l,
                                   c_p]),
    "gdl_nearest2x_fwd": (c_i, [c_p, c_i, c_i, c_i, c_i, c_i, c_l, c_l, c_l, c_p, c_l, c_l, c_l, c_p]),
    "gdl_nearest2x_bwd": (c_i, [c_p, c_i, c_i, c_i, c_i, c_i, c_l, c_l, c_l, c_p, c_l, c_l, c_l, c_p]),
    "gdl_add_relu": (c_i, [c_p, c_p, c_p, c_i, c_l, c_p]),
    "gdl_relu_bwd": (c_i, [c_p, c_p, c_p, c_i, c_l, c_p]),
    "gdl_pad_channels": (c_i, [c_p, c_i, c_l, c_i, c_p, c_i, c_i, c_p]),
    "gdl_bn_stats": (c_i, [c_p, c_i, c_l, c_i, c_l, c_p, c_p, c_p, c_p, c_f, c_p, c_l, c_p]),
    "gdl_bn_stats_workspace": (c_l, [c_l, c_i]),
    "gdl_bn_apply": (c_i, [c_p, c_p, c_i, c_l, c_i, c_l, c_l, c_p, c_p, c_p, c_p, c_f, c_i, c_p]),
    "gdl_bn_bwd_reduce": (c_i, [c_p, c_p, c_i, c_l, c_i, c_l, c_l, c_p, c_p, c_p, c_p, c_f, c_i,
                                c_p, c_p, c_p, c_l, c_p]),
    "gdl_bn_bwd_dx": (c_i, [c_p, c_p, c_p, c_i, c_l, c_i, c_l, c_l, c_l, c_p, c_p, c_p, c_p, c_f,
                            c_i, c_p, c_p, c_l, c_p]),
    "gdl_syncbn_pack": (c_i, [c_p, c_p, C.c_double, c_i, c_p, c_p]),
    "gdl_syncbn_unpack": (c_i, [c_p, c_i, c_p, c_p, c_p, c_p, c_f, c_p]),
    "gdl_bn_bwd_dx_sync": (c_i, [c_p, c_p, c_p, c_i, c_l, c_i, c_l, c_l, c_l, c_p, c_p, c_p, c_p, c_f, c_i, c_p, c_p, c_p, c_p]),
    "gdl_bn_small_fwd": (c_i, [c_p, c_p, c_i, c_l, c_i, c_l, c_l, c_p, c_p, c_f, c_i, c_p, c_p, c_p, c_p, c_f, c_p]),
    "gdl_bn_small_bwd": (c_i, [c_p, c_p, c_p, c_i, c_l, c_i, c_l, c_l, c_l, c_p, c_p, c_p, c_p, c_f, c_i, c_p, c_p, c_p]),
    "gdl_bilinear_fwd": (c_i, [c_p, c_i, c_i, c_i, c_i, c_i, c_l, c_l, c_l, c_p, c_i, c_i, c_i,
                               c_l, c_l, c_l, c_i, c_p]),
    "gdl_bilinear_fwd_add": (c_i, [c_p, c_i, c_i, c_i, c_i, c_i, c_l, c_l, c_l, c_p, c_p, c_i, c_i, c_i,
                                   c_l, c_l, c_l, c_p]),
    "gdl_resize_conv3x3_bwd_gather": (c_i, [c_p, c_i, c_i, c_i, c_i, c_i, c_p, c_i, c_i, c_p]),
    "gdl_resize_conv3x3_bwd_gather_one_pass": (c_i, [c_i, c_i, c_i, c_i, c_i, c_i, c_i]),
    "gdl_resize_conv3x3_bwd_gather_bn": (c_i, [c_p, c_p, c_i, c_i, c_i, c_i, c_i, c_p, c_i, c_i, c_p, c_p, c_p, c_p, c_f, c_i, c_p, c_p,
                                               c_l, c_p, c_p]),
    "gdl_resize_conv3x3_bwd_gather_workspace": (c_l, [c_i, c_i, c_i, c_i, c_i]),
    "gdl_resize_conv3x3_bwd_gather2": (c_i, [c_p, c_i, c_i, c_i, c_i, c_i, c_p, c_i, c_i, c_p, c_l, c_p]),
    "gdl_resize_conv3x3_fwd_sum": (c_i, [c_p, c_p, c_p, c_i, c_i, c_i, c_i, c_p, c_i, c_i, c_p, c_i, c_p]),
    "gdl_resize_conv3x3_fwd_sum_any": (c_i, [c_p, c_i, c_i, c_i, c_i, c_i, c_p, c_i, c_i, c_i, c_p, c_i, c_p]),
    "gdl_resize_conv3x3_fwd_sum_bn_rows": (c_l, [c_i, c_i, c_i]),
    "gdl_resize_conv3x3_fwd_sum_bn": (c_i, [c_p, c_p, c_p, c_i, c_i, c_i, c_i, c_p, c_i, c_i, c_p, c_p, c_l, c_p, c_p, c_p, c_p, c_f, c_p]),
    "gdl_bn_stats_finalize": (c_i, [c_p, c_i, c_i, c_l, c_p, c_p, c_p, c_p, c_f, c_p]),
    "gdl_copy_cast": (c_i, [c_p, c_i, c_i, c_i, c_i, c_i, c_l, c_l, c_l, c_p, c_i, c_l, c_l, c_l, c_p]),
    "gdl_bilinear_sum_fwd": (c_i, [c_p, c_p, c_p, c_i, c_i, c_i, c_i, c_p, c_i, c_i, c_p]),
    "gdl_bilinear_bwd": (c_i, [c_p, c_i, c_i, c_i, c_i, c_i, c_l, c_l, c_l, c_p, c_i, c_i, c_i,
                               c_l, c_l, c_l, c_i, c_p]),
    "gdl_adaptive_avgpool_fwd": (c_i, [c_p, c_i, c_i, c_i, c_i, c_i, c_l, c_l, c_l, c_p, c_i, c_i,
                                       c_p]),
    "gdl_adaptive_avgpool_bwd": (c_i, [c_p, c_i, c_i, c_i, c_i, c_p, c_i, c_i, c_i, c_l, c_l, c_l,
                                       c_i, c_p]),
    "gdl_v_transpose": (c_i, [c_p, c_i, c_i, c_i, c_i, c_i, c_l, c_l, c_p, c_i, c_p]),
    "gdl_softmax_rows": (c_i, [c_p, c_p, c_i, c_l, c_i, c_i, c_p]),
    "gdl_flash_attn_fwd": (c_i, [c_p, c_l, c_l, c_p, c_l, c_l, c_p, c_p, c_i, c_i, c_i, c_i, c_i, c_f, c_p]),
    "gdl_flash_attn_fwd2": (c_i, [c_p, c_l, c_l, c_p, c_l, c_l, c_p, c_l, c_l, c_p, c_l, c_l, c_p, c_i, c_i, c_i, c_i, c_f, c_p]),
    "gdl_flash_attn_bwd": (c_i, [c_p, c_l, c_l, c_p, c_l, c_l, c_p, c_l, c_l, c_p, c_l, c_l, c_p, c_l, c_l, c_p, c_p,
                                 c_p, c_l, c_l, c_p, c_l, c_l, c_p, c_l, c_l, c_i, c_i, c_i, c_i, c_f, c_p, c_l, c_p]),
    "gdl_flash_attn_bwd_workspace": (c_l, [c_i, c_i, c_i, c_i]),
    "gdl_patchify": (c_i, [c_p, c_i, c_i, c_i, c_i, c_i, c_i, c_i, c_i, c_i, c_p, c_i, c_i, c_p]),
    "gdl_dwconv3x3": (c_i, [c_p, c_i, c_i, c_i, c_i, c_i, c_p, c_p, c_i, c_p, c_i, c_p]),
    "gdl_dofa_pack_kernel": (c_i, [c_p, c_i, c_i, c_i, c_f, c_p, c_i, c_i, c_p]),
    "gdl_dofa_unpack_grad": (c_i, [c_p, c_i, c_i, c_i, c_f, c_i, c_p, c_p]),
    "gdl_sincos_embed": (c_i, [c_p, c_p, c_i, c_i, c_p, c_p]),
    "gdl_bn_fold": (c_i, [c_p, c_p, c_p, c_p, c_f, c_i, c_p, c_p, c_p]),
    "gdl_pack_dgrad": (c_i, [c_p, c_i, c_i, c_i, c_i, c_p, c_i, c_p]),
    "gdl_cast": (c_i, [c_p, c_i, c_p, c_i, c_l, c_p]),
    "gdl_scale_f32": (c_i, [c_p, c_p, c_l, c_f, c_p]),
    "gdl_add_rows": (c_i, [c_p, c_l, c_l, c_p, c_l, c_l, c_p, c_l, c_l, c_i, c_p]),
    "gdl_normalize_u8": (c_i, [c_p, c_p, c_i, c_i, c_l, c_p, c_p, c_p]),
    "gdl_normalize_raw": (c_i, [c_p, c_i, c_p, c_i, c_i, c_l, c_p, c_p, c_p]),
    "gdl_augment": (c_i, [c_p, c_i, c_p, c_p, c_p, c_i, c_i, c_i, c_i, c_p, c_p, c_p, c_p]),
    "gdl_scale_outer": (c_i, [c_p, c_i, c_p, c_l, c_l, c_p]),
    "gdl_head_1x1": (c_i, [c_p, c_i, c_l, c_i, c_l, c_p, c_p, c_p, c_l, c_p, c_i, c_p]),
    "gdl_head_1x1_bwd_workspace": (c_l, [c_l, c_i, c_i]),
    "gdl_head_1x1_bwd": (c_i, [c_p, c_i, c_p, c_l, c_i, c_l, c_p, c_p, c_l, c_p, c_l, c_p, c_p, c_i,
                               c_p, c_l, c_p]),
    "gdl_bilinear_fwd_add_bn_ok": (c_i, [c_i, c_i, c_i, c_i, c_i, c_i, c_i]),
    "gdl_bilinear_fwd_add_bn": (c_i, [c_p, c_i, c_i, c_i, c_i, c_i, c_p, c_p, c_p, c_p, c_p, c_f, c_i, c_p, c_i, c_i, c_p]),
    "gdl_head_1x1_bn_ok": (c_i, [c_i, c_l, c_i, c_i]),
    "gdl_head_1x1_bn": (c_i, [c_p, c_i, c_l, c_i, c_p, c_p, c_p, c_p, c_f, c_i, c_p, c_p, c_p, c_i, c_p]),
    "gdl_bn_head_bwd_ok": (c_i, [c_i, c_l, c_i, c_i]),
    "gdl_bn_head_bwd_workspace": (c_l, [c_l, c_i, c_i]),
    "gdl_bn_head_bwd_reduce": (c_i, [c_p, c_i, c_p, c_l, c_i, c_i, c_p, c_p, c_p, c_p, c_p, c_f, c_i, c_p, c_p, c_p, c_p, c_p, c_l, c_p]),
    "gdl_bn_head_bwd_dx": (c_i, [c_p, c_i, c_p, c_p, c_l, c_i, c_i, c_p, c_p, c_p, c_p, c_p, c_f, c_i, c_p, c_p, c_l, c_p]),
    "gdl_upsample_logits": (c_i, [c_p, c_i, c_i, c_i, c_i, c_p, c_i, c_i, c_p]),
    "gdl_upsample_logits_bwd_workspace": (c_l, [c_i, c_i, c_i, c_i]),
    "gdl_upsample_logits_bwd": (c_i, [c_p, c_i, c_i, c_i, c_i, c_p, c_i, c_i, c_p, c_l, c_p]),
    "gdl_softmax_argmax": (c_i, [c_p, c_i, c_i, c_l, c_p, c_p]),
# ... 158 lines not shown
```

### geo-deep-learning_amd/gdlhip/nn.py

```python

from __future__ import annotations

import contextlib
import math
import os

import logging
import weakref
from typing import NamedTuple

import torch
import torch.distributed as dist
from torch import Tensor, nn
from torch.autograd import Function

from . import ops
from .ops import ACT_GELU, ACT_NONE, ACT_RELU, ACT_RESID_RELU


_log = logging.getLogger(__name__)
_WARNED_FP16 = False
_WARNED_FALLBACK: set = set()


def warn_unfused(what: str, why: str) -> None:
    if (what, why) not in _WARNED_FALLBACK:
        _WARNED_FALLBACK.add((what, why))
        _log.warning("gdlhip: %s runs UNFUSED (%s): correct, but several times slower", what, why)


LAUNCH_FUSION = os.environ.get("GDL_LAUNCH_FUSION", "1") != "0"
_COUNTER_BATCH: list | None = None


@contextlib.contextmanager
def counter_batch():
    global _COUNTER_BATCH
    if _COUNTER_BATCH is not None or not LAUNCH_FUSION:
        yield
        return
    _COUNTER_BATCH = []
    try:
        yield
    finally:
        pending, _COUNTER_BATCH = _COUNTER_BATCH, None
        if pending:
            torch._foreach_add_(pending, 1)


def bump(counter: Tensor | None) -> None:
    if counter is None:
        return
    if _COUNTER_BATCH is None:
        counter.add_(1)
    else:
        _COUNTER_BATCH.append(counter)


_KEEP_CACHE: dict = {}


def drop_path_scales(probs: list[float], batch: int, device) -> list[tuple[Tensor | None, Tensor | None]]:
    live = [i for i, p_ in enumerate(probs) if p_ > 0.0]
    out: list[tuple[Tensor | None, Tensor | None]] = [(None, None)] * len(probs)
    if not live:
        return out
    if not LAUNCH_FUSION:
        for i in live:
            out[i] = tuple((torch.empty(batch, device=device, dtype=torch.float32).bernoulli_(1.0 - probs[i]) / (1.0 - probs[i]))
                           for _ in (0, 1))
        return out
    key = (str(device), tuple(probs[i] for i in live))
    keep = _KEEP_CACHE.get(key)
    if keep is None:
        keep = torch.tensor([1.0 - probs[i] for i in live for _ in (0, 1)], dtype=torch.float32, device=device).view(-1, 1)
        _KEEP_CACHE[key] = keep
    scales = torch.bernoulli(keep.expand(-1, batch)) / keep
    for j, i in enumerate(live):
        out[i] = (scales[2 * j], scales[2 * j + 1])
    return out


def compute_dtype() -> torch.dtype:
    if torch.is_autocast_enabled("cuda"):
        global _WARNED_FP16
        if not _WARNED_FP16 and torch.get_autocast_dtype("cuda") == torch.float16:
            _log.warning("gdlhip: fp16 autocast is computed in bf16 (f32 accumulation) by the HIP kernels; no loss scaling is "
                         "needed or applied")
            _WARNED_FP16 = True
        return torch.bfloat16
    return torch.float32


_RAW_WRITES: dict = {}
_CACHE: dict = {}
_CACHE_BUILDS = [0]


def mark_updated(p: Tensor) -> None:
    if id(p) not in _RAW_WRITES:
        weakref.finalize(p, _RAW_WRITES.pop, id(p), None)
    _RAW_WRITES[id(p)] = _RAW_WRITES.get(id(p), 0) + 1


def _mark_running(running_mean: Tensor | None, running_var: Tensor | None) -> None:
    if running_mean is not None:
        mark_updated(running_mean)
        mark_updated(running_var)


def cached(params: tuple, kind: str, builder):
    key = (kind, *[id(p) for p in params])
    ver = tuple((p._version, _RAW_WRITES.get(id(p), 0), p.data_ptr()) for p in params)
# ... 1727 lines not shown
```

### geo-deep-learning_amd/gdlhip/ops.py

```python

from __future__ import annotations

import ctypes as C
import os
from typing import NamedTuple

import torch
from torch import Tensor

from . import _lib
from ._lib import (ACT_GELU, ACT_MUL_GELU_GRAD, ACT_NONE, ACT_RELU, ACT_RESID_RELU, BF16, F32, ConvArgs,
                   WgradArgs, check)

_DT = {torch.float32: F32, torch.bfloat16: BF16}


def dt(t: Tensor | torch.dtype) -> int:
    d = t if isinstance(t, torch.dtype) else t.dtype
    try:
        return _DT[d]
    except KeyError:
        raise ValueError(f"gdlhip: unsupported dtype {d}") from None


# ... 25 lines not shown
                        f"gdlhip.ops.normalize_raw or the host path of SampleProcessor)")
    return img.float().contiguous()


def as_nhwc(x: Tensor) -> Tensor:
    v = x.permute(0, 2, 3, 1)
    return v if v.stride(-1) == 1 else v.contiguous()


def as_nchw(x: Tensor) -> Tensor:
    return x.permute(0, 3, 1, 2)


def _nhwc4(x: Tensor, name: str) -> Tensor:
    if x.dim() == 2:
        x = x.unsqueeze(0).unsqueeze(0)
    if x.dim() != 4 or (x.stride(-1) != 1 and x.shape[-1] != 1):
        raise ValueError(f"{name}: expected NHWC tensor with unit channel stride, got "
                         f"shape {tuple(x.shape)} strides {x.stride()}")
    B, H, W, Cc = x.shape
    sB, sH, sW, _ = x.stride()
    nW = sW if W > 1 else Cc
    nH = sH if H > 1 else W * nW
    nB = sB if B > 1 else H * nH
    if (nB, nH, nW) != (sB, sH, sW) or x.stride(-1) != 1:
        x = x.as_strided((B, H, W, Cc), (nB, nH, nW, 1))
    return x


def conv_gemm(x: Tensor, w: Tensor, *, R: int = 1, S: int = 1, stride: int = 1, pad: int = 0,
              bias: Tensor | None = None, scale: Tensor | None = None, shift: Tensor | None = None,
              act: int = ACT_NONE, batch_scale: Tensor | None = None, resid: Tensor | None = None,
              out: Tensor | None = None, out_dtype: torch.dtype | None = None,
              alpha: float = 1.0, aux_out: Tensor | None = None, want_stats: bool = False):
    _need_cuda(x, w)
    two_d = x.dim() == 2
    x4 = _nhwc4(x, "conv_gemm input")
    B, H, W, Cc = x4.shape
    N = w.shape[0]
    if w.dim() != 2 or w.shape[1] != R * S * Cc or w.stride(1) != 1 or w.dtype != x.dtype:
        raise ValueError(f"conv_gemm: weight must be [{N}, {R * S * Cc}] {x.dtype} K-contiguous, "
                         f"got {tuple(w.shape)} {w.dtype}")
    Ho = (H + 2 * pad - R) // stride + 1
    Wo = (W + 2 * pad - S) // stride + 1
    if out is None:
        out = torch.empty((B, Ho, Wo, N), device=x.device, dtype=out_dtype or x.dtype)
        out4 = out
    else:
        out4 = _nhwc4(out, "conv_gemm out")
        if tuple(out4.shape) != (B, Ho, Wo, N):
            raise ValueError(f"conv_gemm: out shape {tuple(out4.shape)} != {(B, Ho, Wo, N)}")
    a = ConvArgs()
    a.inp, a.dtype = x4.data_ptr(), dt(x)
    a.B, a.H, a.W, a.C = B, H, W, Cc
    a.in_sB, a.in_sH, a.in_sW = x4.stride(0), x4.stride(1), x4.stride(2)
    a.Ho, a.Wo, a.R, a.S, a.stride, a.pad = Ho, Wo, R, S, stride, pad
    a.w, a.w_sN, a.N = w.data_ptr(), w.stride(0), N
    a.out, a.out_dtype = out4.data_ptr(), dt(out4)
    a.out_sB, a.out_sH, a.out_sW = out4.stride(0), out4.stride(1), out4.stride(2)
    a.alpha = alpha
    a.bias = None if bias is None else _f32vec(bias, N, "bias").data_ptr()
    a.scale = None if scale is None else _f32vec(scale, N, "scale").data_ptr()
    a.shift = None if shift is None else _f32vec(shift, N, "shift").data_ptr()
    a.act = act
    a.batch_scale = None if batch_scale is None else _f32vec(batch_scale, B, "batch_scale").data_ptr()
    if resid is not None:
        r4 = _nhwc4(resid, "conv_gemm resid")
        if r4.shape[-1] != N or r4.shape[1:3] != out4.shape[1:3]:
            raise ValueError("conv_gemm: resid shape mismatch")
        a.resid, a.resid_dtype = r4.data_ptr(), dt(r4)
        a.res_sB = r4.stride(0) if r4.shape[0] == B else 0
        a.res_sH, a.res_sW = r4.stride(1), r4.stride(2)
    if aux_out is not None:
        x4a = _nhwc4(aux_out, "conv_gemm aux_out")
        if x4a.shape != out4.shape or x4a.stride() != out4.stride() or x4a.dtype != out4.dtype:
            raise ValueError("conv_gemm: aux_out must match out in shape, strides and dtype")
        a.aux_out = x4a.data_ptr()
    a.nz, a.nz_inner = 1, 1
    partials, rows = None, 0
    if want_stats:
        rows = int(_lib.load().gdl_conv_gemm_stats_rows(C.byref(a)))
        if rows:
            partials = torch.empty((rows, 2, N), device=x.device, dtype=torch.float32)
            a.stats_partial = partials.data_ptr()
    _launch_conv_gemm(a, "gdl_conv_gemm")
    if two_d and out4 is out:
        out = out.view(Wo, N)
    return (out, partials, rows) if want_stats else out


class KernelTimer:

    VARIANT = {0: "conv_gemm_kernel<{dt},2,2,1,1> (64x64 tiles)", 1: "conv_gemm_kernel<{dt},2,2,2,2> (128x128 tiles)",
               2: "conv_gemm_kernel<{dt},2,4,4,2> (256x256 tiles)",
               3: "conv_gemm_kernel<{dt},2,4,4,2,pingpong> (256x256 tiles, alternating loader halves)",
               4: "conv3x3_sf_kernel<{dt}> (256x256 tiles, 3x3 taps share one staged activation tile)",
               5: "conv_gemm_kernel<{dt},4,1,2,2> (256x64 tiles, narrow outputs)",
               6: "conv_gemm_dual_kernel (256x128 tiles, four waves, two workgroups resident per CU)",
               8: "conv_gemm_w4_kernel (256x256 tiles, one wave per SIMD, every load in an MFMA shadow)",
               9: "conv_gemm_persist_kernel (256x256 ping-pong tiles, one persistent workgroup per CU, next tile's first stage under the epilogue)",
               10: "conv_gemm_w4p_kernel (256x256 tiles, one persistent workgroup per CU, one wave per SIMD, finished tile parked in registers and stored from the next tile's MFMA shadows)",
               7: "conv3x3_narrow_kernel (direct 3x3, C <= 32, one staged window per 4 x 64 pixels x 32 output channels)",
               12: "conv_gemm_kernel<{dt},2,2,1,1,stages=4> (64x64 tiles, four LDS stages: few tiles, long K)"}

    def __init__(self) -> None:
        self.records: list = []
        self.variants: list = []

    def launch(self, a: ConvArgs, what: str) -> None:
        lib = _lib.load()
        fl = C.c_int64()
# ... 116 lines not shown
    nbytes = lib.gdl_conv_wgrad_workspace(C.byref(a))
    ws = torch.empty(max(nbytes, 4) // 4, device=x.device, dtype=torch.float32)
    a.workspace, a.workspace_bytes = ws.data_ptr(), nbytes
    check(lib.gdl_conv_wgrad(C.byref(a), _stream()), "gdl_conv_wgrad(grouped)")
    return dw


def conv_wgrad(x: Tensor, dy: Tensor, *, R: int, S: int, stride: int = 1, pad: int = 0,
               dw: Tensor | None = None, accumulate: bool = False) -> Tensor:
    _need_cuda(x, dy)
    x4, dy4 = _nhwc4(x, "wgrad x"), _nhwc4(dy, "wgrad dy")
    if x4.dtype != dy4.dtype:
        raise ValueError("conv_wgrad: x and dy dtypes differ")
    B, H, W, Cc = x4.shape
    _, Ho, Wo, N = dy4.shape
    if dw is None:
        dw = torch.empty((N, R * S * Cc), device=x.device, dtype=torch.float32)
    a = WgradArgs()
    a.inp, a.dy, a.dtype = x4.data_ptr(), dy4.data_ptr(), dt(x4)
    a.B, a.H, a.W, a.C = B, H, W, Cc
    a.in_sB, a.in_sH, a.in_sW = x4.stride(0), x4.stride(1), x4.stride(2)
    a.Ho, a.Wo, a.R, a.S, a.stride, a.pad, a.N = Ho, Wo, R, S, stride, pad, N
    a.dy_sB, a.dy_sH, a.dy_sW = dy4.stride(0), dy4.stride(1), dy4.stride(2)
    a.dw, a.dw_sN, a.accumulate = dw.data_ptr(), dw.stride(0), int(accumulate)
    a.nz, a.nz_inner = 1, 1
    lib = _lib.load()
    nbytes = lib.gdl_conv_wgrad_workspace(C.byref(a))
    ws = torch.empty(max(nbytes, 4) // 4, device=x.device, dtype=torch.float32)
    a.workspace, a.workspace_bytes = ws.data_ptr(), nbytes
    check(lib.gdl_conv_wgrad(C.byref(a), _stream()), "gdl_conv_wgrad")
    return dw


def layernorm(x: Tensor, gamma: Tensor, beta: Tensor, eps: float, out_dtype: torch.dtype) -> Tensor:
    _need_cuda(x)
    if x.dtype != torch.float32 or x.stride(-1) != 1:
        raise ValueError("layernorm: x must be f32 with unit last stride")
    D = x.shape[-1]
    x2 = x.reshape(-1, D)
    y = torch.empty((x2.shape[0], D), device=x.device, dtype=out_dtype)
    check(_lib.load().gdl_layernorm_fwd(_p(x2), x2.stride(0), _p(_f32vec(gamma, D, "gamma")),
                                        _p(_f32vec(beta, D, "beta")), _p(y), dt(y), x2.shape[0], D,
                                        eps, _stream()), "gdl_layernorm_fwd")
    return y.reshape(x.shape)


def _pix(x: Tensor, name: str):
    x4 = _nhwc4(x, name)
    B, H, W, Cc = x4.shape
    sB, sH, sW = x4.stride(0), x4.stride(1), x4.stride(2)
    if W > 1:
        sP = sW
    elif H > 1:
        sP = sH
    else:
        sP = sB if B > 1 else Cc
    ok = (H == 1 or W == 1 or sH == W * sP) and (B == 1 or H * W == 1 or sB == H * W * sP)
    if not ok:
        raise ValueError(f"{name}: pixels must be uniformly strided, got strides {x4.stride()}")
    return B * H * W, Cc, sP


def bn_stats(x: Tensor, running_mean: Tensor | None = None, running_var: Tensor | None = None,
             momentum: float = 0.1):
    _need_cuda(x)
    P, Cc, sP = _pix(x, "bn_stats x")
    mean = torch.empty(Cc, device=x.device, dtype=torch.float32)
    var = torch.empty_like(mean)
    lib = _lib.load()
    nbytes = lib.gdl_bn_stats_workspace(P, Cc)
    ws = torch.empty(nbytes // 4, device=x.device, dtype=torch.float32)
# ... 599 lines not shown
    a.inp, a.dtype = q.data_ptr(), dt(q)
    a.B, a.H, a.W, a.C = 1, 1, Nq, hd
    a.in_sB, a.in_sH, a.in_sW = Nq * q.stride(1), Nq * q.stride(1), q.stride(1)
    a.Ho, a.Wo, a.R, a.S, a.stride, a.pad = 1, Nq, 1, 1, 1, 0
    a.w, a.w_sN, a.N = k.data_ptr(), k.stride(1), Nkv
    a.out, a.out_dtype = scores.data_ptr(), dt(scores)
    a.out_sB, a.out_sH, a.out_sW = Nq * npad, Nq * npad, npad
    a.alpha, a.act = float(hd) ** -0.5, ACT_NONE
    a.nz, a.nz_inner = B * num_heads, num_heads
    a.in_sZ0, a.in_sZ1 = q.stride(0), hd
    a.w_sZ0, a.w_sZ1 = k.stride(0), hd
    a.out_sZ0, a.out_sZ1 = num_heads * Nq * npad, Nq * npad
    batched_gemm_raw(a)
    check(lib.gdl_softmax_rows(_p(scores), _p(scores), dt(scores), B * num_heads * Nq, Nkv, npad,
                               _stream()), "gdl_softmax_rows")
    out = torch.empty((B, Nq, D), device=q.device, dtype=q.dtype)
    a = ConvArgs()
    a.inp, a.dtype = scores.data_ptr(), dt(scores)
    a.B, a.H, a.W, a.C = 1, 1, Nq, npad
    a.in_sB, a.in_sH, a.in_sW = Nq * npad, Nq * npad, npad
    a.Ho, a.Wo, a.R, a.S, a.stride, a.pad = 1, Nq, 1, 1, 1, 0
    a.w, a.w_sN, a.N = vt.data_ptr(), npad, hd
    a.out, a.out_dtype = out.data_ptr(), dt(out)
    a.out_sB, a.out_sH, a.out_sW = Nq * D, Nq * D, D
    a.alpha, a.act = 1.0, ACT_NONE
    a.nz, a.nz_inner = B * num_heads, num_heads
    a.in_sZ0, a.in_sZ1 = num_heads * Nq * npad, Nq * npad
    a.w_sZ0, a.w_sZ1 = num_heads * hd * npad, hd * npad
    a.out_sZ0, a.out_sZ1 = Nq * D, hd
    batched_gemm_raw(a)
    return out


def attention_flash(q: Tensor, k: Tensor, v: Tensor, num_heads: int, return_lse: bool = False):
    B, Nq, Nkv, D, hd = _attn_check(q, k, v, num_heads)
    if q.dtype != torch.bfloat16 or hd != 64:
        raise ValueError("attention_flash: needs bf16 and head_dim 64")
    out = torch.empty((B, Nq, D), device=q.device, dtype=q.dtype)
    lse = torch.empty((B, num_heads, Nq), device=q.device, dtype=torch.float32) if return_lse else None
    check(_lib.load().gdl_flash_attn_fwd2(_p(q), q.stride(0), q.stride(1), _p(k), k.stride(0), k.stride(1),
                                          _p(v), v.stride(0), v.stride(1), _p(out), out.stride(0), out.stride(1),
                                          _p(lse), B, num_heads, Nq, Nkv, float(hd) ** -0.5, _stream()),
          "gdl_flash_attn_fwd2")
    return (out, lse) if return_lse else out


def attention_flash_v1(q: Tensor, k: Tensor, v: Tensor, num_heads: int) -> Tensor:
    B, Nq, Nkv, D, hd = _attn_check(q, k, v, num_heads)
    npad = (Nkv + 63) // 64 * 64
    vt = _v_transposed(v, num_heads, hd, npad)
    out = torch.empty((B, Nq, D), device=q.device, dtype=q.dtype)
    check(_lib.load().gdl_flash_attn_fwd(_p(q), q.stride(0), q.stride(1), _p(k), k.stride(0), k.stride(1),
                                         _p(vt), _p(out), B, num_heads, Nq, Nkv, npad, float(hd) ** -0.5,
                                         _stream()), "gdl_flash_attn_fwd")
    return out


def flash_ok(q: Tensor, num_heads: int) -> bool:
    return q.dtype == torch.bfloat16 and q.shape[2] // num_heads == 64


def attention(q: Tensor, k: Tensor, v: Tensor, num_heads: int, return_lse: bool = False):
    if flash_ok(q, num_heads):
        return attention_flash(q, k, v, num_heads, return_lse)
    out = attention_unfused(q, k, v, num_heads)
    return (out, None) if return_lse else out


def attention_flash_bwd(q: Tensor, k: Tensor, v: Tensor, o: Tensor, do: Tensor, lse: Tensor, num_heads: int,
                        dq: Tensor, dk: Tensor, dv: Tensor) -> None:
    B, Nq, Nkv, D, hd = _attn_check(q, k, v, num_heads)
    for t, n in ((o, Nq), (do, Nq), (dq, Nq), (dk, Nkv), (dv, Nkv)):
        if t.shape != (B, n, D) or t.dtype != torch.bfloat16 or t.stride(2) != 1:
            raise ValueError("attention_flash_bwd: tensor shape / dtype / stride mismatch")
    if lse.shape != (B, num_heads, Nq) or lse.dtype != torch.float32 or not lse.is_contiguous():
        raise ValueError("attention_flash_bwd: lse must be contiguous f32 [B,H,Nq]")
    dvec = torch.empty_like(lse)
    nbytes = _lib.load().gdl_flash_attn_bwd_workspace(B, num_heads, Nq, Nkv)
    ws = torch.empty(nbytes // 4, device=q.device, dtype=torch.float32) if nbytes else None
    check(_lib.load().gdl_flash_attn_bwd(
        _p(q), q.stride(0), q.stride(1), _p(k), k.stride(0), k.stride(1), _p(v), v.stride(0), v.stride(1),
        _p(o), o.stride(0), o.stride(1), _p(do), do.stride(0), do.stride(1), _p(lse), _p(dvec),
        _p(dq), dq.stride(0), dq.stride(1), _p(dk), dk.stride(0), dk.stride(1), _p(dv), dv.stride(0), dv.stride(1),
        B, num_heads, Nq, Nkv, float(hd) ** -0.5, _p(ws), nbytes, _stream()), "gdl_flash_attn_bwd")


def split_qkv(qkv: Tensor):
    D = qkv.shape[-1] // 3
    return qkv[..., :D], qkv[..., D:2 * D], qkv[..., 2 * D:]


def dwconv3x3(x: Tensor, w9: Tensor, bias: Tensor, gelu: bool, out_dtype: torch.dtype | None = None) -> Tensor:
    _need_cuda(x)
    if x.dim() != 4 or not x.is_contiguous():
        raise ValueError("dwconv3x3: contiguous NHWC input expected")
    B, H, W, Cc = x.shape
    if w9.shape != (9, Cc) or w9.dtype != torch.float32 or not w9.is_contiguous():
# ... 1120 lines not shown
```

### geo-deep-learning_amd/gdlhip/tnn.py

```python

from __future__ import annotations

import torch
from torch import Tensor
from torch.autograd import Function

from . import ops
from .nn import cached, conv_weight_matrix, gemm_weight, to_compute
from .ops import ACT_GELU, ACT_MUL_GELU_GRAD, ACT_NONE


def _wmat32(weight: Tensor) -> Tensor:
    w = weight.detach() if weight.dim() == 2 else conv_weight_matrix(weight)
    return w if w.is_contiguous() else w.contiguous()


def t_weight(weight: Tensor, cd: torch.dtype) -> Tensor:
    def build():
        wm = _wmat32(weight)
        return ops.pack_dgrad(wm, wm.shape[0], 1, wm.shape[1], cd)
    return cached((weight,), f"wT:{cd}", build)


def flipped_weight(weight: Tensor, cd: torch.dtype) -> Tensor:
    def build():
        n, c, r, s = weight.shape
        return ops.pack_dgrad(conv_weight_matrix(weight), n, r * s, c, cd)
    return cached((weight,), f"dgrad:{cd}", build)


def _dense(g: Tensor) -> Tensor:
    if g.is_contiguous():
        return g
    shape = g.shape
    g4 = g if g.dim() == 4 else g.reshape(shape[0], 1, -1, shape[-1]) if g.dim() == 3 else g.unsqueeze(0).unsqueeze(0)
    return ops.copy_cast(g4, out_dtype=g.dtype).view(shape)


def _to_cd(g: Tensor, cd: torch.dtype) -> Tensor:
# ... 238 lines not shown
        dkv = torch.empty_like(kv)
        ops.attention_bwd(q, kv[..., :c], kv[..., c:], da, heads, dq, dkv[..., :c], dkv[..., c:], o=a, lse=lse)
        kv_in = xn if sr > 1 else h1
        dkvw, dkvb = linear_dw(kv_in, dkv)
        dxn = linear_dx(dkv, kvw)
        dqw, dqb = linear_dw(h1, dq)
        extra = ()
        if sr > 1:
            srw, srb, nsw, nsb = prm[16:20]
            dred, dnsw, dnsb = ops.layernorm_bwd(red.view(b, -1, c), dxn, nsw.detach(), eps_sr)
            dred = (dred if cd == torch.float32 else ops.cast(dred, cd)).view(red.shape)
            h1_img = h1.view(b, hh, ww, c)
            dsrw = _as_param_grad(ops.conv_wgrad(h1_img, dred, R=sr, S=sr, stride=sr), srw)
            dsrb = ops.colsum(dred)
            side = conv_dx(dred, srw, sr, 0, (hh, ww)).view(b, n, c)
            extra = (dsrw, dsrb, dnsw, dnsb)
        else:
            side = dxn
        dh1 = linear_dx(dq, qw, resid=side)
        gx, dn1w, dn1b = ops.layernorm_bwd(x, dh1, n1w.detach(), eps1, dres=gx1)
        ddww = dw9.t().reshape(dww.shape)
        return (gx, None, None, None, None, None, None, None, None, None,
                dn1w, dn1b, dqw, dqb, dkvw, dkvb, dpw, dpb, dn2w, dn2b, df1w, df1b, ddww, ddwb, df2w, df2b, *extra)


def mit_block(x: Tensor, s1, s2, hh: int, ww: int, heads: int, sr: int, eps1: float, eps_sr: float,
              cd: torch.dtype, params: tuple) -> Tensor:
    return _MitBlock.apply(x, s1, s2, hh, ww, heads, sr, eps1, eps_sr, cd, *params)


class _VitBlock(Function):

    @staticmethod
    def forward(ctx, x, s1, s2, heads, eps, cd, *prm):
        n1w, n1b, qkvw, qkvb, pw, pb, g1, n2w, n2b, f1w, f1b, f2w, f2b, g2 = prm
        b, n, c = x.shape
        d = [None if p is None else p.detach() for p in prm]
        h1 = ops.layernorm(x, d[0], d[1], eps, cd)
        qkv = ops.linear(h1, gemm_weight(qkvw, cd), d[3])
        qv, kv_, vv = ops.split_qkv(qkv)
        a, lse = ops.attention(qv, kv_, vv, heads, return_lse=True)
        train = any(ctx.needs_input_grad)
        x1, z1 = torch.empty_like(x), (torch.empty_like(x) if train else None)
        ops.conv_gemm(a.view(b, 1, n, c), gemm_weight(pw, cd), bias=d[5], scale=d[6], batch_scale=s1,
                      resid=x.view(b, 1, n, c), out=x1.view(b, 1, n, c),
                      aux_out=z1.view(b, 1, n, c) if train else None)
        h2 = ops.layernorm(x1, d[7], d[8], eps, cd)
        u = torch.empty((b, n, f1w.shape[0]), device=x.device, dtype=cd) if train else None
        f = ops.linear(h2, gemm_weight(f1w, cd), d[10], act=ACT_GELU, aux_out=u)
        x2, z2 = torch.empty_like(x), (torch.empty_like(x) if train else None)
        ops.conv_gemm(f.view(b, 1, n, -1), gemm_weight(f2w, cd), bias=d[12], scale=d[13], batch_scale=s2,
                      resid=x1.view(b, 1, n, c), out=x2.view(b, 1, n, c),
                      aux_out=z2.view(b, 1, n, c) if train else None)
        if train:
            ctx.save_for_backward(x, s1, s2, h1, qkv, a, z1, x1, h2, u, f, z2, lse, *prm)
            ctx.cfg = (heads, eps, cd)
        return x2

    @staticmethod
    def backward(ctx, gx2):
        x, s1, s2, h1, qkv, a, z1, x1, h2, u, f, z2, lse, *prm = ctx.saved_tensors
        n1w, n1b, qkvw, qkvb, pw, pb, g1, n2w, n2b, f1w, f1b, f2w, f2b, g2 = prm
        heads, eps, cd = ctx.cfg
        b, n, c = x.shape
        gx2 = _dense(gx2)
        dz2, dg2 = ops.layerscale_bwd(gx2, z2, None if g2 is None else g2.detach(), s2, cd)
        df2w, df2b = linear_dw(f, dz2)
        du = linear_dx(dz2, f2w, resid=u, act=ACT_MUL_GELU_GRAD)
        df1w, df1b = linear_dw(h2, du)
        dh2 = linear_dx(du, f1w)
        gx1, dn2w, dn2b = ops.layernorm_bwd(x1, dh2, n2w.detach(), eps, dres=gx2)
        dz1, dg1 = ops.layerscale_bwd(gx1, z1, None if g1 is None else g1.detach(), s1, cd)
        dpw, dpb = linear_dw(a, dz1)
        da = linear_dx(dz1, pw)
        dqkv = torch.empty_like(qkv)
        qv, kv_, vv = ops.split_qkv(qkv)
        dq_, dk_, dv_ = ops.split_qkv(dqkv)
        ops.attention_bwd(qv, kv_, vv, da, heads, dq_, dk_, dv_, o=a, lse=lse)
        dqkvw, dqkvb = linear_dw(h1, dqkv)
        dh1 = linear_dx(dqkv, qkvw)
        gx, dn1w, dn1b = ops.layernorm_bwd(x, dh1, n1w.detach(), eps, dres=gx1)
        return (gx, None, None, None, None, None,
                dn1w, dn1b, dqkvw, dqkvb, dpw, dpb, dg1, dn2w, dn2b, df1w, df1b, df2w, df2b, dg2)


def vit_block(x: Tensor, s1, s2, heads: int, eps: float, cd: torch.dtype, params: tuple) -> Tensor:
    return _VitBlock.apply(x, s1, s2, heads, eps, cd, *params)


class _DofaTokens(Function):

    @staticmethod
    def forward(ctx, cols, wq, bias, cls_token, pos_embed):
        b, n, kp = cols.shape
        d = wq.shape[0]
        tok = torch.empty((b, n + 1, d), device=cols.device, dtype=torch.float32)
        ops.add_rows(cls_token.detach().view(1, d), None, tok[:, 0, :], b)
        wq_c = wq.detach() if wq.dtype == cols.dtype else ops.cast(wq.detach().contiguous(), cols.dtype)
        ops.conv_gemm(cols.view(b, 1, n, kp), wq_c, bias=bias.detach(),
                      resid=pos_embed.detach()[0, 1:, :].view(1, 1, n, d), out=tok[:, 1:, :].unsqueeze(1))
        ctx.save_for_backward(cols)
        return tok

    @staticmethod
    def backward(ctx, g):
        (cols,) = ctx.saved_tensors
        g = _dense(g)
        d = g.shape[-1]
        dcls = ops.colsum(g[:, 0, :]).view(1, 1, d) if ctx.needs_input_grad[3] else None
        dwq = dbias = None
        if ctx.needs_input_grad[1] or ctx.needs_input_grad[2]:
            dwq, dbias = linear_dw(cols, _to_cd(g[:, 1:, :], cols.dtype))
        return None, dwq, dbias, dcls, None


def dofa_tokens(cols: Tensor, wq: Tensor, bias: Tensor, cls_token: Tensor, pos_embed: Tensor) -> Tensor:
    return _DofaTokens.apply(cols, wq, bias, cls_token, pos_embed)


class _Tap(Function):
# ... 102 lines not shown
```

### geo-deep-learning_amd/geo_deep_learning/models/encoders/dofa_v2.py

```python

from __future__ import annotations

import torch
from torch import Tensor, nn

from gdlhip import nn as gnn
from gdlhip import ops, tnn


def position_embedding(embed_dim: int, pos: Tensor) -> Tensor:
    if embed_dim % 2 != 0:
        msg = "embed_dim must be even"
        raise ValueError(msg)
    return ops.sincos_embed(pos, embed_dim)


class FCResLayer(nn.Module):

    def __init__(self, linear_size: int = 128) -> None:
        super().__init__()
        self.l_size = linear_size
        self.w1 = nn.Linear(self.l_size, self.l_size)
        self.w2 = nn.Linear(self.l_size, self.l_size)

# ... 150 lines not shown
class _Mlp(nn.Module):
    def __init__(self, dim: int, hidden: int) -> None:
        super().__init__()
        self.fc1 = nn.Linear(dim, hidden)
        self.fc2 = nn.Linear(hidden, dim)


class Block(nn.Module):

    def __init__(self, dim: int, num_heads: int, mlp_ratio: float = 4.0, qkv_bias: bool = True,
                 proj_drop: float = 0.0, attn_drop: float = 0.0, drop_path: float = 0.0,
                 norm_layer=nn.LayerNorm, init_values: float | None = 1e-5) -> None:
        super().__init__()
        if not qkv_bias or proj_drop or attn_drop or init_values is None:
            msg = "gdlhip Block implements the DOFA configuration (qkv_bias, LayerScale, no dropout)"
            raise NotImplementedError(msg)
        self.norm1 = norm_layer(dim)
        self.attn = _Attention(dim, num_heads)
        self.ls1 = _LayerScale(dim, init_values)
        self.norm2 = norm_layer(dim)
        self.mlp = _Mlp(dim, int(dim * mlp_ratio))
        self.ls2 = _LayerScale(dim, init_values)
        self.drop_prob = float(drop_path)

    def _drop_scale(self, batch: int, device, mask: Tensor | None) -> Tensor | None:
        if self.drop_prob == 0.0 or not self.training:
            return None
        keep = 1.0 - self.drop_prob
        if mask is None:
            mask = torch.empty(batch, device=device, dtype=torch.float32).bernoulli_(keep)
        return (mask.to(device=device, dtype=torch.float32) / keep).contiguous()

    def forward(self, x: Tensor, masks: tuple[Tensor, Tensor] | None = None,
                scales: tuple[Tensor | None, Tensor | None] | None = None) -> Tensor:
        b = x.shape[0]
        if scales is not None and masks is None:
            s1, s2 = scales
        else:
            s1 = self._drop_scale(b, x.device, None if masks is None else masks[0])
            s2 = self._drop_scale(b, x.device, None if masks is None else masks[1])
        at, m = self.attn, self.mlp
        prm = (self.norm1.weight, self.norm1.bias, at.qkv.weight, at.qkv.bias, at.proj.weight, at.proj.bias,
               self.ls1.gamma, self.norm2.weight, self.norm2.bias, m.fc1.weight, m.fc1.bias, m.fc2.weight, m.fc2.bias,
               self.ls2.gamma)
        return tnn.vit_block(x, s1, s2, at.num_heads, self.norm1.eps, gnn.compute_dtype(), prm)


class DOFAv2(nn.Module):

    def __init__(
        self,
        encoder_name: str = "dofa_base",
        img_size: int | tuple[int, int] = 224,
        patch_size: int = 14,
        embed_dim: int = 768,
        depth: int = 12,
        num_heads: int = 12,
        mlp_ratio: float = 4.0,
        drop_rate: float = 0.0,
        drop_path_rate: float = 0.1,
        out_indices: list[int] | None = None,
        norm_layer: nn.Module = nn.LayerNorm,
        init_values: float = 1e-5,
        *,
        convert_patch_to_16: bool = False,
        pretrained: bool = True,
    ) -> None:
        super().__init__()
        if drop_rate != 0.0:
            msg = "gdlhip DOFAv2: drop_rate must be 0 (the reference's value)"
            raise NotImplementedError(msg)
        self.encoder_name = encoder_name
        self.pretrained = pretrained
        if isinstance(img_size, int):
            img_size = (img_size, img_size)
        self.img_size = tuple(img_size)
        self.patch_size = patch_size
        self.embed_dim = embed_dim
# ... 131 lines not shown
        gen = pe.weight_generator
        if len(gen.transformer_encoder.layers) != 1:
            msg = "gdlhip DOFAv2: the generator backward is built for num_layers=1 (the reference's value)"
            raise NotImplementedError(msg)
        layer = gen.transformer_encoder.layers[0]
        sa = layer.self_attn
        dev = pe.fclayer.w1.weight.device
        pos = (host * 1000).to(dev)
        emb = position_embedding(pe.dynamic_embed_dim, pos)
        prm = (pe.fclayer.w1.weight, pe.fclayer.w1.bias, pe.fclayer.w2.weight, pe.fclayer.w2.bias, gen.weight_tokens,
               gen.bias_token, sa.in_proj_weight, sa.in_proj_bias, sa.out_proj.weight, sa.out_proj.bias,
               layer.linear1.weight, layer.linear1.bias, layer.linear2.weight, layer.linear2.bias, layer.norm1.weight,
               layer.norm1.bias, layer.norm2.weight, layer.norm2.bias, gen.fc_weight.weight, gen.fc_weight.bias,
               gen.fc_bias.weight, gen.fc_bias.bias)
        kpad = pe.k_padded(host.numel(), pe.kernel_size, cd)
        return tnn.dofa_generator(emb, sa.num_heads, pe.kernel_size * pe.kernel_size, pe.embed_dim, pe.scaler, kpad,
                                  layer.norm1.eps, layer.norm2.eps, prm)

    def _tokens(self, x: Tensor, wavelengths: Tensor, drop_masks):
        cd = gnn.compute_dtype()
        b, c, h, w_ = x.shape
        k = self.patch_size
        gh, gw = (h + 2 - k) // k + 1, (w_ + 2 - k) // k + 1
        n = gh * gw
        if n + 1 != self.pos_embed.shape[1]:
            msg = f"image {h}x{w_} gives {n} patches but pos_embed has {self.pos_embed.shape[1] - 1}"
            raise ValueError(msg)
        if torch.is_grad_enabled() and any(p.requires_grad for p in self.patch_embed.parameters()):
            wq, bias = self._trainable_operands(wavelengths, cd)
        else:
            wq, bias = self._dynamic_operands(wavelengths, x.device, cd)
        cols = ops.patchify(ops.image_f32(x, "DOFAv2"), k, 1, gh, gw, wq.shape[1], cd)
        tok = tnn.dofa_tokens(cols.view(b, n, -1), wq, bias, self.cls_token, self.pos_embed)
        scales = None
        if self.training and drop_masks is None:
            scales = gnn.drop_path_scales([blk.drop_prob for blk in self.blocks], b, tok.device)
        for i, blk in enumerate(self.blocks):
            tok = blk(tok, None if drop_masks is None else drop_masks[i], None if scales is None else scales[i])
            yield i, tok

    def forward_features_nhwc(self, x: Tensor, wavelengths: Tensor, drop_masks=None) -> list[Tensor]:
        cd = gnn.compute_dtype()
        feats = []
        for i, tok in self._tokens(x, wavelengths, drop_masks):
            if i in self.out_indices:
                feats.append(tnn.tap(tok, int((tok.shape[1] - 1) ** 0.5), cd))
        return feats

    def forward_features(self, x: Tensor, wavelengths: Tensor,
                         drop_masks: list[tuple[Tensor, Tensor]] | None = None) -> list[Tensor]:
        feats = []
        for i, tok in self._tokens(x, wavelengths, drop_masks):
            if i in self.out_indices:
                hw = int((tok.shape[1] - 1) ** 0.5)
                feats.append(tok[:, 1:, :].unflatten(1, (hw, hw)).permute(0, 3, 1, 2))
        return feats

    def forward(self, x: Tensor, wavelengths: Tensor, drop_masks=None) -> list[Tensor]:
        return self.forward_features(x, wavelengths, drop_masks)


def create_dofa_base(img_size=224, out_indices=None, *, pretrained: bool = True, **kwargs) -> DOFAv2:
    return DOFAv2(encoder_name="dofa_base", img_size=img_size, patch_size=14, embed_dim=768,
                  num_heads=12, depth=12, out_indices=out_indices or [4, 6, 10, 11],
                  pretrained=pretrained, **kwargs)


def create_dofa_large(img_size=224, out_indices=None, *, pretrained: bool = True, **kwargs) -> DOFAv2:
    return DOFAv2(encoder_name="dofa_large", img_size=img_size, patch_size=14, embed_dim=1024,
                  num_heads=16, depth=24, out_indices=out_indices or [5, 9, 15, 21],
                  pretrained=pretrained, **kwargs)
# ... 1 lines not shown
```

### include/gdlhip.h

```cpp
#ifndef GDLHIP_H_
#define GDLHIP_H_

#include <stdint.h>

#ifdef __cplusplus
extern "C" {
#endif

typedef void* gdl_stream_t;

enum { GDL_F32 = 0, GDL_BF16 = 1 };
enum {
  GDL_ACT_NONE = 0,
  GDL_ACT_RELU = 1,
  GDL_ACT_GELU = 2,
  GDL_ACT_MUL_GELU_GRAD = 3,
  GDL_ACT_RESID_RELU = 4
};
enum {
  GDL_OK = 0,
  GDL_ERR_INVALID = -1,
  GDL_ERR_LAUNCH = -2,
  GDL_ERR_UNSUPPORTED = -3
};

int gdl_version(void);
const char* gdl_last_error(void);

typedef struct {
  const void* in;
  int dtype;
  int B, H, W, C;
  int64_t in_sB, in_sH, in_sW;
  int Ho, Wo, R, S, stride, pad;
  const void* w;
  int64_t w_sN;
  int N;
  void* out;
  int out_dtype;
  int64_t out_sB, out_sH, out_sW;
  float alpha;
  const float* bias;
  const float* scale;
  const float* shift;
  int act;
  const float* batch_scale;
  const void* resid;
  int resid_dtype;
  int64_t res_sB, res_sH, res_sW;
  int nz, nz_inner;
  int64_t in_sZ0, in_sZ1, w_sZ0, w_sZ1, out_sZ0, out_sZ1;
  void* aux_out;
  float* stats_partial;
} gdl_conv_args;

int gdl_conv_gemm(const gdl_conv_args* a, gdl_stream_t stream);
int64_t gdl_conv_gemm_stats_rows(const gdl_conv_args* a);
int gdl_conv_gemm_plan(const gdl_conv_args* a, int64_t* flops);

typedef struct {
  const void* in;
  const void* dy;
  int dtype;
  int B, H, W, C;
  int64_t in_sB, in_sH, in_sW;
  int Ho, Wo, R, S, stride, pad;
  int N;
  int64_t dy_sB, dy_sH, dy_sW;
  float* dw;
  int64_t dw_sN;
  int accumulate;
  float* workspace;
  int64_t workspace_bytes;
  int nz, nz_inner;
  int64_t in_sZ0, in_sZ1, dy_sZ0, dy_sZ1, dw_sZ0, dw_sZ1;
} gdl_wgrad_args;

int64_t gdl_conv_wgrad_workspace(const gdl_wgrad_args* a);
int gdl_conv_wgrad(const gdl_wgrad_args* a, gdl_stream_t stream);

int gdl_layernorm_fwd(const float* x, int64_t x_stride, const float* gamma, const float* beta,
                      void* y, int y_dtype, int64_t rows, int D, float eps, gdl_stream_t stream);

int gdl_bn_stats(const void* x, int dtype, int64_t P, int C, int64_t x_sP, float* mean,
                 float* var_biased, float* running_mean, float* running_var, float momentum,
                 float* workspace, int64_t workspace_bytes, gdl_stream_t stream);
int64_t gdl_bn_stats_workspace(int64_t P, int C);
int gdl_bn_apply(const void* x, void* y, int dtype, int64_t P, int C, int64_t x_sP, int64_t y_sP,
                 const float* mean, const float* var, const float* gamma, const float* beta,
                 float eps, int relu, gdl_stream_t stream);
int gdl_bn_bwd_reduce(const void* x, const void* dy, int dtype, int64_t P, int C, int64_t x_sP,
                      int64_t dy_sP, const float* mean, const float* var, const float* gamma,
                      const float* beta, float eps, int relu, float* dgamma, float* dbeta,
                      float* workspace, int64_t workspace_bytes, gdl_stream_t stream);
int gdl_bn_bwd_dx(const void* x, const void* dy, void* dx, int dtype, int64_t P, int C, int64_t x_sP,
                  int64_t dy_sP, int64_t dx_sP, const float* mean, const float* var,
                  const float* gamma, const float* beta, float eps, int relu,
                  const float* dgamma_sum, const float* dbeta_sum, int64_t P_total,
                  gdl_stream_t stream);
int gdl_syncbn_pack(const float* mean, const float* var, double count, int C, float* out, gdl_stream_t stream);
int gdl_syncbn_unpack(const float* packed, int C, float* mean, float* var, float* running_mean, float* running_var, float momentum,
                      gdl_stream_t stream);
int gdl_bn_bwd_dx_sync(const void* x, const void* dy, void* dx, int dtype, int64_t P, int C, int64_t x_sP, int64_t dy_sP, int64_t dx_sP,
                       const float* mean, const float* var, const float* gamma, const float* beta, float eps, int relu,
                       const float* dgamma_sum, const float* dbeta_sum, const float* total_count, gdl_stream_t stream);
int gdl_bn_small_fwd(const void* x, void* y, int dtype, int64_t P, int C, int64_t x_sP, int64_t y_sP, const float* gamma,
                     const float* beta, float eps, int relu, float* mean, float* var, float* running_mean, float* running_var,
                     float momentum, gdl_stream_t stream);
int gdl_bn_small_bwd(const void* x, const void* dy, void* dx, int dtype, int64_t P, int C, int64_t x_sP, int64_t dy_sP, int64_t dx_sP,
                     const float* mean, const float* var, const float* gamma, const float* beta, float eps, int relu,
                     float* dgamma, float* dbeta, gdl_stream_t stream);

int gdl_bn_gelu_apply(const void* x, void* y, int dtype, int64_t P, int C, int64_t x_sP, int64_t y_sP, const float* mean,
                      const float* var, const float* gamma, const float* beta, float eps, gdl_stream_t stream);
int gdl_bn_gelu_bwd_reduce(const void* x, const void* dy, int dtype, int64_t P, int C, int64_t x_sP, int64_t dy_sP,
// ... 84 lines not shown
                                   const float* addvec, int relu, gdl_stream_t stream);
int64_t gdl_resize_conv3x3_fwd_sum_bn_rows(int B, int Ho, int Wo);
int gdl_resize_conv3x3_fwd_sum_bn(const void* const* zs, const int* hs, const int* ws, int nsrc, int dtype, int B, int N, void* out,
                                  int Ho, int Wo, const float* addvec, float* workspace, int64_t ws_bytes, float* mean, float* var,
                                  float* running_mean, float* running_var, float momentum, gdl_stream_t stream);
int gdl_bn_stats_finalize(const float* partials, int nsplit, int C, int64_t P, float* mean, float* var, float* running_mean,
                          float* running_var, float momentum, gdl_stream_t stream);
int gdl_copy_cast(const void* in, int in_dtype, int B, int H, int W, int C, int64_t in_sB, int64_t in_sH, int64_t in_sW,
                  void* out, int out_dtype, int64_t out_sB, int64_t out_sH, int64_t out_sW, gdl_stream_t stream);
int gdl_bilinear_sum_fwd(const void* const* srcs, const int* hs, const int* ws, int nsrc, int dtype, int B, int C,
                         void* out, int Ho, int Wo, gdl_stream_t stream);
int gdl_bilinear_bwd(const void* dout, int dout_dtype, int B, int Ho, int Wo, int C,
                     int64_t dout_sB, int64_t dout_sH, int64_t dout_sW, void* din, int din_dtype,
                     int Hi, int Wi, int64_t din_sB, int64_t din_sH, int64_t din_sW, int accumulate,
                     gdl_stream_t stream);
int gdl_adaptive_avgpool_fwd(const void* in, int dtype, int B, int Hi, int Wi, int C, int64_t in_sB,
                             int64_t in_sH, int64_t in_sW, void* out, int out_dtype, int So,
                             gdl_stream_t stream);
int gdl_adaptive_avgpool_bwd(const void* dout, int dtype, int B, int So, int C, void* din,
                             int din_dtype, int Hi, int Wi, int64_t din_sB, int64_t din_sH,
                             int64_t din_sW, int accumulate, gdl_stream_t stream);

int gdl_v_transpose(const void* v, int dtype, int B, int N, int H, int hd, int64_t v_sB, int64_t v_sN,
                    void* vt, int Npad, gdl_stream_t stream);
int gdl_softmax_rows(const void* in, void* out, int dtype, int64_t rows, int n_valid, int n_cols,
                     gdl_stream_t stream);
int gdl_flash_attn_fwd(const void* q, int64_t q_sB, int64_t q_sN, const void* k, int64_t k_sB,
                       int64_t k_sN, const void* vt, void* o, int B, int H, int Nq, int Nkv, int Npad,
                       float scale, gdl_stream_t stream);

int gdl_flash_attn_fwd2(const void* q, int64_t q_sB, int64_t q_sN, const void* k, int64_t k_sB, int64_t k_sN,
                        const void* v, int64_t v_sB, int64_t v_sN, void* o, int64_t o_sB, int64_t o_sN, float* lse,
                        int B, int H, int Nq, int Nkv, float scale, gdl_stream_t stream);
int gdl_flash_attn_bwd(const void* q, int64_t q_sB, int64_t q_sN, const void* k, int64_t k_sB, int64_t k_sN,
                       const void* v, int64_t v_sB, int64_t v_sN, const void* o, int64_t o_sB, int64_t o_sN,
                       const void* dout, int64_t do_sB, int64_t do_sN, const float* lse, float* dvec,
                       void* dq, int64_t dq_sB, int64_t dq_sN, void* dk, int64_t dk_sB, int64_t dk_sN,
                       void* dv, int64_t dv_sB, int64_t dv_sN, int B, int H, int Nq, int Nkv, float scale,
                       float* ws, int64_t ws_bytes, gdl_stream_t stream);
int64_t gdl_flash_attn_bwd_workspace(int B, int H, int Nq, int Nkv);

int gdl_patchify(const float* img, int B, int C, int H, int W, int P, int stride, int pad, int Gh,
                 int Gw, void* cols, int out_dtype, int Kpad, gdl_stream_t stream);
int gdl_dwconv3x3(const void* in, int dtype, int B, int H, int W, int C, const float* w9,
                  const float* bias, int gelu, void* out, int out_dtype, gdl_stream_t stream);
int gdl_dofa_pack_kernel(const float* g, int C, int PP, int D, float scaler, void* out,
                         int out_dtype, int Kpad, gdl_stream_t stream);
int gdl_dofa_unpack_grad(const float* dw, int C, int PP, int D, float scaler, int Kpad, float* dg, gdl_stream_t stream);

int gdl_sincos_embed(const float* pos, const float* omega, int M, int D, float* out, gdl_stream_t stream);
int gdl_bn_fold(const float* gamma, const float* beta, const float* mean, const float* var, float eps,
                int C, float* scale, float* shift, gdl_stream_t stream);
int gdl_pack_dgrad(const void* w, int w_dtype, int N, int T, int C, void* out, int out_dtype,
                   gdl_stream_t stream);

int gdl_cast(const void* in, int in_dtype, void* out, int out_dtype, int64_t n, gdl_stream_t stream);
int gdl_scale_f32(const float* in, float* out, int64_t n, float s, gdl_stream_t stream);
int gdl_add_rows(const float* a, int64_t a_rows, int64_t a_stride, const float* b, int64_t b_rows,
                 int64_t b_stride, float* out, int64_t out_stride, int64_t rows, int D,
                 gdl_stream_t stream);
int gdl_normalize_u8(const uint8_t* in, float* out, int B, int C, int64_t HW, const float* mean,
                     const float* std, gdl_stream_t stream);
enum { GDL_RAW_U8 = 0, GDL_RAW_U16 = 1, GDL_RAW_I16 = 2, GDL_RAW_F32 = 3 };
int gdl_normalize_raw(const void* in, int kind, float* out, int B, int C, int64_t HW, const float* mean,
                      const float* stdv, gdl_stream_t stream);
int gdl_scale_outer(void* x, int dtype, const float* s, int64_t outer, int64_t inner,
// ... 214 lines not shown
```

Baseline: 998.9 tiles/s.

## Skip dropped samples in frozen ViT blocks via live-order gather and early exit

When the encoder is frozen and DropPath is active, each block computes a permutation that packs the surviving samples first plus a live count. LayerNorm, the QKV/FC1 GEMMs, attention and the residual-add GEMMs then process only live rows and scatter results back through batch_perm. Dropped samples are copied through unchanged. This is meant to avoid spending encoder compute on samples whose branch output is zeroed anyway, at the cost of more kernel plumbing, device-side live counts that force grid over-launch with early exits, and an extra copy kernel.

Measured after the change: 1007 tiles/s (median of 6 runs). Within noise of the previous version (+0.8%).

```diff
diff --git a/geo-deep-learning_amd/csrc/attention_v2.hip b/geo-deep-learning_amd/csrc/attention_v2.hip
--- a/geo-deep-learning_amd/csrc/attention_v2.hip
+++ b/geo-deep-learning_amd/csrc/attention_v2.hip
@@ -34,6 +34,7 @@
   float scale, scale_log2e;
   int qsplit;
   float* dkv_part;
+  const int* live_b;
 };
 
 __device__ __forceinline__ void stage_piece(const srd_t& srd, int64_t tok_stride_bytes, int tok0, int ntok, int piece,
@@ -227,6 +228,7 @@
   int blk, bh;
   decode_block((f.Nq + 32 * NW - 1) / (32 * NW), f.B * f.H, blk, bh);
   const int b = bh / f.H, h = bh % f.H;
+  if (f.live_b && b >= *f.live_b) return;
   const int q0 = blk * (32 * NW) + wave * 32;
   const bool active = q0 < f.Nq;
   const int frow = lane & 31, fhalf = lane >> 5;
@@ -724,6 +726,13 @@
 extern "C" int gdl_flash_attn_fwd2(const void* q, int64_t q_sB, int64_t q_sN, const void* k, int64_t k_sB, int64_t k_sN,
                                    const void* v, int64_t v_sB, int64_t v_sN, void* o, int64_t o_sB, int64_t o_sN,
                                    float* lse, int B, int H, int Nq, int Nkv, float scale, gdl_stream_t stream) {
+  return gdl_flash_attn_fwd2_live(q, q_sB, q_sN, k, k_sB, k_sN, v, v_sB, v_sN, o, o_sB, o_sN, lse, B, H, Nq, Nkv, scale, nullptr, stream);
+}
+
+extern "C" int gdl_flash_attn_fwd2_live(const void* q, int64_t q_sB, int64_t q_sN, const void* k, int64_t k_sB, int64_t k_sN,
+                                        const void* v, int64_t v_sB, int64_t v_sN, void* o, int64_t o_sB, int64_t o_sN,
+                                        float* lse, int B, int H, int Nq, int Nkv, float scale, const int* live_batch,
+                                        gdl_stream_t stream) {
   GDL_CHECK_ARG(q && k && v && o, "gdl_flash_attn_fwd2: null pointer");
   GDL_CHECK_ARG(B > 0 && H > 0 && Nq > 0 && Nkv > 0, "gdl_flash_attn_fwd2: bad dims");
   GDL_CHECK_ARG(((uintptr_t)q % 16 == 0) && ((uintptr_t)k % 16 == 0) && ((uintptr_t)v % 16 == 0) && ((uintptr_t)o % 8 == 0) &&
@@ -735,6 +744,7 @@
   f.q = (const uint16_t*)q; f.k = (const uint16_t*)k; f.v = (const uint16_t*)v; f.out = (uint16_t*)o; f.lse = lse;
   f.q_sB = q_sB; f.q_sN = q_sN; f.k_sB = k_sB; f.k_sN = k_sN; f.v_sB = v_sB; f.v_sN = v_sN; f.o_sB = o_sB; f.o_sN = o_sN;
   f.B = B; f.H = H; f.Nq = Nq; f.N = Nkv;
+  f.live_b = live_batch;
   f.scale = scale; f.scale_log2e = scale * 1.4426950408889634f;
   const int nw = Nq > 128 ? 4 : 2;
   const unsigned grid = (unsigned)((Nq + 64 * nw - 1) / (64 * nw) * B * H);
diff --git a/geo-deep-learning_amd/csrc/conv3x3_sf.hip b/geo-deep-learning_amd/csrc/conv3x3_sf.hip
--- a/geo-deep-learning_amd/csrc/conv3x3_sf.hip
+++ b/geo-deep-learning_amd/csrc/conv3x3_sf.hip
@@ -23,7 +23,7 @@
 
   const int lid = xcd_remap(blockIdx.x, k.tiles_m * k.tiles_n);
   int tile_m, tile_n;
-  tile_order(k, lid, tile_m, tile_n);
+  tile_order(k, k.tiles_m, lid, tile_m, tile_n);
   const int m0 = tile_m * BM, n0 = tile_n * BN;
   const srd_t srd_a = make_srd(a.in, k.in_span);
   const srd_t srd_b = make_srd(a.w, k.w_span);
diff --git a/geo-deep-learning_amd/csrc/conv_gemm.hip b/geo-deep-learning_amd/csrc/conv_gemm.hip
--- a/geo-deep-learning_amd/csrc/conv_gemm.hip
+++ b/geo-deep-learning_amd/csrc/conv_gemm.hip
@@ -30,9 +30,11 @@
   const int wave = __builtin_amdgcn_readfirstlane(tid >> 6);
   const int wm = wave / WARPS_N, wn = wave % WARPS_N;
 
-  const int lid = xcd_remap(blockIdx.x, k.tiles_m * k.tiles_n);
+  const int tiles_m = live_tiles_m(k, BM);
+  if ((int)blockIdx.x >= tiles_m * k.tiles_n) return;
+  const int lid = xcd_remap(blockIdx.x, tiles_m * k.tiles_n);
   int tile_m, tile_n;
-  tile_order(k, lid, tile_m, tile_n);
+  tile_order(k, tiles_m, lid, tile_m, tile_n);
   const int m0 = tile_m * BM, n0 = tile_n * BN;
   const int z = blockIdx.y;
   const int z0 = z / a.nz_inner, z1 = z % a.nz_inner;
@@ -345,6 +347,15 @@
   const int64_t in_span = (((int64_t)a.B - 1) * a.in_sB + ((int64_t)a.H - 1) * a.in_sH + ((int64_t)a.W - 1) * a.in_sW + a.C) * es;
   const int64_t w_span = (((int64_t)a.N - 1) * a.w_sN + (int64_t)a.R * a.S * a.C) * es;
   GDL_CHECK_ARG(w_span <= kSpanMax, "gdl_conv_gemm: weight matrix spans more than 2 GiB");
+  if (a.live_rows || a.batch_perm) {
+    const int64_t oes = (int64_t)gdl_elem_size(a.out_dtype), res_es = (int64_t)gdl_elem_size(a.resid_dtype);
+    GDL_CHECK_ARG(a.nz == 1 && !a.stats_partial && in_span <= kSpanMax && a.R == 1 && a.S == 1,
+                  "gdl_conv_gemm: live_rows / batch_perm need a 1x1 filter, nz == 1, no stats_partial and an input below 2 GiB");
+    GDL_CHECK_ARG(!a.batch_perm || ((((int64_t)a.B - 1) * a.out_sB + ((int64_t)a.Ho - 1) * a.out_sH + ((int64_t)a.Wo - 1) * a.out_sW + a.N) * oes <= kSpanMax &&
+                                    (!a.resid || (((int64_t)a.B - 1) * a.res_sB + ((int64_t)a.Ho - 1) * a.res_sH + ((int64_t)a.Wo - 1) * a.res_sW + a.N) * res_es <= kSpanMax)),
+                  "gdl_conv_gemm: batch_perm needs out and resid to span less than 2 GiB");
+    GDL_CHECK_ARG(!a.batch_perm || !a.resid || a.res_sB != 0 || a.B == 1, "gdl_conv_gemm: batch_perm needs a per-image residual");
+  }
   if (in_span > kSpanMax) {
     GDL_CHECK_ARG(a.B > 1 && a.nz == 1, "gdl_conv_gemm: one image spans more than 2 GiB");
     const int b1 = a.B / 2;
@@ -391,6 +402,7 @@
   if (variant == 6) return conv_gemm_dual_launch(k, s);
   if (variant == 8) return conv_gemm_w4_launch(k, s);
   if (variant == 9) return conv_gemm_persist_launch(k, s);
+  if (variant == 10 && a.batch_perm) return conv_gemm_persist_launch(k, s);
   if (variant == 10) return conv_gemm_w4p_launch(k, s);
   if (variant == 12) {
     const bool extra = a.aux_out || a.act == GDL_ACT_MUL_GELU_GRAD;
diff --git a/geo-deep-learning_amd/csrc/conv_gemm_common.h b/geo-deep-learning_amd/csrc/conv_gemm_common.h
--- a/geo-deep-learning_amd/csrc/conv_gemm_common.h
+++ b/geo-deep-learning_amd/csrc/conv_gemm_common.h
@@ -67,10 +67,17 @@
 }
 
 
-__device__ __forceinline__ void tile_order(const KArgs& k, int lid, int& tile_m, int& tile_n) {
+__device__ __forceinline__ int live_rows(const KArgs& k) {
+  return k.a.live_rows ? min(k.M, *k.a.live_rows) : k.M;
+}
+__device__ __forceinline__ int live_tiles_m(const KArgs& k, int bm) {
+  return k.a.live_rows ? (live_rows(k) + bm - 1) / bm : k.tiles_m;
+}
+
+__device__ __forceinline__ void tile_order(const KArgs& k, int tiles_m, int lid, int& tile_m, int& tile_n) {
   const int ng = k.n_group;
   if (ng <= 0 || ng >= k.tiles_n) { tile_n = lid % k.tiles_n; tile_m = lid / k.tiles_n; return; }
-  const int per_group = k.tiles_m * ng;
+  const int per_group = tiles_m * ng;
   const int g = lid / per_group, idx = lid - g * per_group;
   const int width = min(ng, k.tiles_n - g * ng);
   tile_m = idx / width;
@@ -106,7 +113,8 @@
                       (out_zoff % 8 == 0) && (a.N % 16 == 0);
   const bool res_ok = !a.resid || (((uintptr_t)a.resid % 16 == 0) && (a.res_sW % 4 == 0));
   const bool vecs_ok = ((uintptr_t)a.bias % 16 == 0) && ((uintptr_t)a.scale % 16 == 0) && ((uintptr_t)a.shift % 16 == 0);
-  if (!(k.out_dense && k.res_dense && vec_ok && res_ok && vecs_ok && (!a.batch_scale || HoWo >= 32))) return false;
+  if (!(k.out_dense && k.res_dense && vec_ok && res_ok && vecs_ok && ((!a.batch_scale && !a.batch_perm) || HoWo >= 32))) return false;
+  const int M = live_rows(k);
   const int frow = lane & 31, fhalf = lane >> 5;
   const int n_w = n0 + wn * 64;
   const bool packed = plain && out_bf16;
@@ -150,23 +158,34 @@
 #pragma unroll
   for (int i = 0; i < TM; ++i) {
     const int mp = m0 + (wm * TM + i) * 32;
-    if (mp >= k.M) break;
+    if (mp >= M) break;
     float rv[8][4];
     float rs0 = 1.f, rs1 = 1.f;
     int rem0 = 0;
+    int d0 = 0, d1 = 0;
+    if (a.batch_scale || a.batch_perm) {
+      const int b0 = mp / HoWo;
+      rem0 = mp - b0 * HoWo;
+      int p0 = b0, p1 = b0 + 1;
+      if (a.batch_perm) {
+        p0 = a.batch_perm[b0];
+        p1 = b0 + 1 < a.B ? a.batch_perm[b0 + 1] : p0;
+        d0 = (p0 - b0) * HoWo;
+        d1 = (p1 - b0 - 1) * HoWo;
+      }
+      if (a.batch_scale && !packed && !plain) {
+        rs0 = a.batch_scale[p0];
+        rs1 = b0 + 1 < a.B ? a.batch_scale[p1] : 0.f;
+      }
+    }
+    auto real_row = [&](int rr) { return mp + rr + (rem0 + rr >= HoWo ? d1 : d0); };
     if (!packed && !plain) {
-      if (a.batch_scale) {
-        const int b0 = mp / HoWo;
-        rem0 = mp - b0 * HoWo;
-        rs0 = a.batch_scale[b0];
-        rs1 = b0 + 1 < a.B ? a.batch_scale[b0 + 1] : 0.f;
-      }
 #pragma unroll
       for (int t = 0; t < 8; ++t) {
         const int m = mp + (lane >> 4) + 4 * t, n = n_w + 4 * (lane & 15);
         rv[t][0] = rv[t][1] = rv[t][2] = rv[t][3] = 0.f;
-        if (a.resid && m < k.M && n < a.N) {
-          const int64_t ro = (int64_t)m * a.res_sW + n;
+        if (a.resid && m < M && n < a.N) {
+          const int64_t ro = (int64_t)real_row((lane >> 4) + 4 * t) * a.res_sW + n;
           if (a.resid_dtype == GDL_BF16) {
             const uint2 u = *(const uint2*)((const uint16_t*)a.resid + ro);
             rv[t][0] = __uint_as_float(u.x << 16); rv[t][1] = __uint_as_float(u.x & 0xffff0000u);
@@ -217,7 +236,7 @@
           const int rr = (lane >> 3) + 8 * t, slot = lane & 7;
           const uint4 v = *(const uint4*)(lds + rr * 128 + ((slot ^ (rr & 7)) << 4));
           const int m = mp + rr, n = n_w + 8 * slot;
-          if (m < k.M && n < a.N) *(uint4*)((uint16_t*)base + (int64_t)m * a.out_sW + out_zoff + n) = v;
+          if (m < M && n < a.N) *(uint4*)((uint16_t*)base + (int64_t)real_row(rr) * a.out_sW + out_zoff + n) = v;
         }
       } else {
 #pragma unroll
@@ -226,7 +245,7 @@
           const float4 q = *(const float4*)(lds + rr * 256 + ((slot ^ (rr & 7)) << 4));
           float v[4] = {q.x, q.y, q.z, q.w};
           const int m = mp + rr, n = n_w + 4 * slot;
-          if (m >= k.M || n >= a.N) continue;
+          if (m >= M || n >= a.N) continue;
           if (row_terms && !plain) {
             if (a.batch_scale) {
               const float rs = rem0 + rr >= HoWo ? rs1 : rs0;
@@ -247,7 +266,7 @@
               }
             }
           }
-          const int64_t off = (int64_t)m * a.out_sW + out_zoff + n;
+          const int64_t off = (int64_t)real_row(rr) * a.out_sW + out_zoff + n;
           if (out_bf16) *(uint2*)((uint16_t*)base + off) = make_uint2(pack_bf16x2(v[0], v[1]), pack_bf16x2(v[2], v[3]));
           else *(float4*)((float*)base + off) = make_float4(v[0], v[1], v[2], v[3]);
         }
@@ -272,7 +291,7 @@
 constexpr int EPI_RUNTIME = 0, EPI_FIXED = 1, EPI_SCALE = 2, EPI_DROPPATH = 4, EPI_RELU = 8, EPI_GELU = 16;
 constexpr int EPI_STATS = 32;
 
-template <int TM, int CH, bool RESID, int EF = EPI_RUNTIME>
+template <int TM, int CH, bool RESID, int EF = EPI_RUNTIME, bool PERM = false>
 __device__ __forceinline__ void conv_epilogue_rows2_impl(const KArgs& k, f32x16_t (&acc)[TM][2], int m0, int n0, int wm, int wn,
                                                         int lane, int64_t out_zoff, unsigned char* lds) {
 #pragma clang fp contract(off)
@@ -302,7 +321,7 @@
   }
   constexpr int RW = 4;
   constexpr int OES = CH == 8 ? 2 : 4;
-  const int m_w = m0 + wm * TM * 32;
+  const int m_w = PERM ? 0 : m0 + wm * TM * 32;
   const __amdgpu_buffer_rsrc_t res_rs = __builtin_amdgcn_make_buffer_rsrc(
       (void*)((const unsigned char*)a.resid + ((int64_t)m_w * a.res_sW + n0 + wn * 64) * OES), 0, 0x7fffffff, 0x00020000);
   const __amdgpu_buffer_rsrc_t out_rs = __builtin_amdgcn_make_buffer_rsrc(
@@ -310,23 +329,37 @@
   const unsigned res_lo = (unsigned)((srow * (int)a.res_sW + CH * slot) * OES);
   const unsigned out_lo = (unsigned)((srow * (int)a.out_sW + CH * slot) * OES);
   typedef __attribute__((ext_vector_type(4))) unsigned epi_u4;
+  float rs0 = 1.f, rs1 = 1.f;
+  int rem0 = 0;
+  int d0 = 0, d1 = 0;
+  if (has_bs) {
+    const int b0 = m0 / HoWo;
+    rem0 = m0 - b0 * HoWo;
+    int p0 = b0, p1 = b0 + 1;
+    if constexpr (PERM) {
+      p0 = a.batch_perm[b0];
+      p1 = b0 + 1 < a.B ? a.batch_perm[b0 + 1] : p0;
+      d0 = (p0 - b0) * HoWo;
+      d1 = (p1 - b0 - 1) * HoWo;
+    }
+    rs0 = a.batch_scale[p0];
+    rs1 = b0 + 1 < a.B ? a.batch_scale[p1] : 0.f;
+  }
+  auto shift_rows = [&](int row) { return rem0 + row >= HoWo ? d1 : d0; };
   auto load_resid_t = [&](int mp, int t, uint32_t (&rw)[NT][RW]) {
-    const unsigned ru = (unsigned)((mp - m_w + (64 / LPR) * t) * (int)a.res_sW * OES);
-    const epi_u4 u = __builtin_amdgcn_raw_buffer_load_b128(res_rs, res_lo, ru, 0);
+    unsigned ru = (unsigned)((mp - m_w + (64 / LPR) * t) * (int)a.res_sW * OES);
+    unsigned lo = res_lo;
+    if constexpr (PERM) {
+      lo += (unsigned)((mp + (64 / LPR) * t + shift_rows(mp - m0 + srow + (64 / LPR) * t)) * (int)a.res_sW * OES);
+      ru = 0;
+    }
+    const epi_u4 u = __builtin_amdgcn_raw_buffer_load_b128(res_rs, lo, ru, 0);
     rw[t][0] = u.x; rw[t][1] = u.y; rw[t][2] = u.z; rw[t][3] = u.w;
   };
   auto resid_value = [&](const uint32_t (&w)[RW], int e) -> float {
     if constexpr (CH == 8) return __uint_as_float((e & 1) ? (w[e >> 1] & 0xffff0000u) : (w[e >> 1] << 16));
     else return __uint_as_float(w[e]);
   };
-  float rs0 = 1.f, rs1 = 1.f;
-  int rem0 = 0;
-  if (has_bs) {
-    const int b0 = m0 / HoWo;
-    rem0 = m0 - b0 * HoWo;
-    rs0 = a.batch_scale[b0];
-    rs1 = b0 + 1 < a.B ? a.batch_scale[b0 + 1] : 0.f;
-  }
   float st1[8] = {0.f, 0.f, 0.f, 0.f, 0.f, 0.f, 0.f, 0.f}, st2[8] = {0.f, 0.f, 0.f, 0.f, 0.f, 0.f, 0.f, 0.f};
   uint32_t rva[NT][RW];
   if constexpr (RESID) {
@@ -387,7 +420,8 @@
           if (i + 1 < TM) load_resid_t(mp + 32, t, rva);
         }
       }
-      const unsigned ou = (unsigned)((i * 32 + (64 / LPR) * t) * (int)a.out_sW * OES);
+      unsigned ou = (unsigned)((i * 32 + (64 / LPR) * t) * (int)a.out_sW * OES);
+      if constexpr (PERM) ou = (unsigned)((mp + (64 / LPR) * t + shift_rows((wm * TM + i) * 32 + rr)) * (int)a.out_sW * OES);
       epi_u4 o;
       if constexpr (CH == 8) {
         o = epi_u4{pack_bf16x2(v[0], v[1]), pack_bf16x2(v[2], v[3]), pack_bf16x2(v[4], v[5]), pack_bf16x2(v[6], v[7])};
@@ -436,7 +470,13 @@
   if (!k.epi_v2 || a.aux_out || a.act == GDL_ACT_MUL_GELU_GRAD ||
       !(k.out_dense && k.res_dense && vec_ok && res_ok && vecs_ok && (!a.batch_scale || HoWo >= 256)))
     return false;
-  if (m0 + (wm + 1) * TM * 32 > k.M || n0 + (wn + 1) * 64 > a.N) return false;
+  if (m0 + (wm + 1) * TM * 32 > live_rows(k) || n0 + (wn + 1) * 64 > a.N) return false;
+  if (a.batch_perm) {
+    if (k.epi_v2 == 2 || !GDL_EPI_ON(8) || !a.resid || !a.scale || !a.batch_scale || a.act != GDL_ACT_NONE || out_bf16 || a.stats_partial)
+      return false;
+    conv_epilogue_rows2_impl<TM, 4, true, EPI_FIXED | EPI_SCALE | EPI_DROPPATH, true>(k, acc, m0, n0, wm, wn, lane, out_zoff, lds);
+    return true;
+  }
   const bool sc = a.scale != nullptr, bs = a.batch_scale != nullptr, rs = a.resid != nullptr;
   if (a.stats_partial) {
     conv_epilogue_rows2_impl<TM, 8, false, EPI_FIXED | EPI_STATS>(k, acc, m0, n0, wm, wn, lane, out_zoff, lds);
@@ -494,17 +534,20 @@
   int64_t row_o[TM], row_r[TM];
   float row_s[TM];
   bool m_ok[TM];
+  const int M_live = live_rows(k);
 #pragma unroll
   for (int i = 0; i < TM; ++i) {
     const int m = m0 + (wm * TM + i) * 32 + frow;
-    m_ok[i] = m < k.M;
+    m_ok[i] = m < M_live;
     row_s[i] = 1.f;
-    if (k.out_dense && k.res_dense && !a.batch_scale) {
+    if (k.out_dense && k.res_dense && !a.batch_scale && !a.batch_perm) {
       row_o[i] = (int64_t)m * a.out_sW + out_zoff;
       row_r[i] = (int64_t)m * a.res_sW;
     } else {
       const int mm = m_ok[i] ? m : 0;
-      const int b = mm / HoWo, rem = mm - b * HoWo, oy = rem / a.Wo, ox = rem - oy * a.Wo;
+      int b = mm / HoWo;
+      const int rem = mm - b * HoWo, oy = rem / a.Wo, ox = rem - oy * a.Wo;
+      if (a.batch_perm) b = a.batch_perm[b];
       row_o[i] = (int64_t)b * a.out_sB + (int64_t)oy * a.out_sH + (int64_t)ox * a.out_sW + out_zoff;
       row_r[i] = (int64_t)b * a.res_sB + (int64_t)oy * a.res_sH + (int64_t)ox * a.res_sW;
       if (a.batch_scale) row_s[i] = a.batch_scale[b];
diff --git a/geo-deep-learning_amd/csrc/conv_gemm_dual.hip b/geo-deep-learning_amd/csrc/conv_gemm_dual.hip
--- a/geo-deep-learning_amd/csrc/conv_gemm_dual.hip
+++ b/geo-deep-learning_amd/csrc/conv_gemm_dual.hip
@@ -22,9 +22,11 @@
   const int wave = __builtin_amdgcn_readfirstlane(tid >> 6);
   const int wm = wave / WARPS_N, wn = wave % WARPS_N;
 
-  const int lid = xcd_remap(blockIdx.x, k.tiles_m * k.tiles_n);
+  const int tiles_m = live_tiles_m(k, DBM);
+  if ((int)blockIdx.x >= tiles_m * k.tiles_n) return;
+  const int lid = xcd_remap(blockIdx.x, tiles_m * k.tiles_n);
   int tile_m, tile_n;
-  tile_order(k, lid, tile_m, tile_n);
+  tile_order(k, tiles_m, lid, tile_m, tile_n);
   const int m0 = tile_m * DBM, n0 = tile_n * DBN;
   const int z = blockIdx.y;
   const int z0 = z / a.nz_inner, z1 = z % a.nz_inner;
diff --git a/geo-deep-learning_amd/csrc/conv_gemm_persist.hip b/geo-deep-learning_amd/csrc/conv_gemm_persist.hip
--- a/geo-deep-learning_amd/csrc/conv_gemm_persist.hip
+++ b/geo-deep-learning_amd/csrc/conv_gemm_persist.hip
@@ -27,7 +27,9 @@
     const int lane = tid & 63;
     const int wave = __builtin_amdgcn_readfirstlane(tid >> 6);
     const int wm = wave / WARPS_N, wn = wave % WARPS_N;
-    const int ntiles = k.tiles_m * k.tiles_n;
+    const int tiles_m = live_tiles_m(k, 256);
+    const int ntiles = tiles_m * k.tiles_n;
+    if (v >= ntiles) return;
     const srd_t srd_a = make_srd(a.in, k.in_span);
     const srd_t srd_b = make_srd(a.w, k.w_span);
     const unsigned lds_base =
@@ -72,7 +74,7 @@
     };
 
     int tile_m, tile_n;
-    tile_order(k, xcd_remap(v, ntiles), tile_m, tile_n);
+    tile_order(k, tiles_m, xcd_remap(v, ntiles), tile_m, tile_n);
     const int m0 = tile_m * 256, n0 = tile_n * 256;
     const unsigned a_v = a_lane + (unsigned)m0 * a_row, b_v = b_lane + (unsigned)n0 * b_row;
     if (first_tile && half == 0) issue(0, a_v, b_v, 0u);
@@ -115,7 +117,7 @@
     const bool more = vn < ntiles;
     if (more && half == 0 && k.dbg != 11) {
       int tm2, tn2;
-      tile_order(k, xcd_remap(vn, ntiles), tm2, tn2);
+      tile_order(k, tiles_m, xcd_remap(vn, ntiles), tm2, tn2);
       issue(0, a_lane + (unsigned)(tm2 * 256) * a_row, b_lane + (unsigned)(tn2 * 256) * b_row, 0u);
     }
     {
diff --git a/geo-deep-learning_amd/csrc/conv_gemm_w4.hip b/geo-deep-learning_amd/csrc/conv_gemm_w4.hip
--- a/geo-deep-learning_amd/csrc/conv_gemm_w4.hip
+++ b/geo-deep-learning_amd/csrc/conv_gemm_w4.hip
@@ -18,9 +18,11 @@
   const int wave = __builtin_amdgcn_readfirstlane(tid >> 6);
   const int wm = wave >> 1, wn = wave & 1;
 
-  const int lid = xcd_remap(blockIdx.x, k.tiles_m * k.tiles_n);
+  const int tiles_m = live_tiles_m(k, 256);
+  if ((int)blockIdx.x >= tiles_m * k.tiles_n) return;
+  const int lid = xcd_remap(blockIdx.x, tiles_m * k.tiles_n);
   int tile_m, tile_n;
-  tile_order(k, lid, tile_m, tile_n);
+  tile_order(k, tiles_m, lid, tile_m, tile_n);
   const int m0 = tile_m * 256, n0 = tile_n * 256;
   const int z = blockIdx.y;
   const int z0 = z / a.nz_inner, z1 = z % a.nz_inner;
diff --git a/geo-deep-learning_amd/csrc/conv_gemm_w4p.hip b/geo-deep-learning_amd/csrc/conv_gemm_w4p.hip
--- a/geo-deep-learning_amd/csrc/conv_gemm_w4p.hip
+++ b/geo-deep-learning_amd/csrc/conv_gemm_w4p.hip
@@ -272,7 +272,7 @@
   int v = blockIdx.x;
   {
     int tm, tn;
-    tile_order(k, xcd_remap(v, ntiles), tm, tn);
+    tile_order(k, k.tiles_m, xcd_remap(v, ntiles), tm, tn);
     unsigned a_lane, b_lane;
     lane_ab(a_lane, b_lane);
     a_v = a_lane + (unsigned)(tm * 256) * a_row;
@@ -285,7 +285,7 @@
   }
   for (;;) {
     int tile_m, tile_n;
-    tile_order(k, xcd_remap(v, ntiles), tile_m, tile_n);
+    tile_order(k, k.tiles_m, xcd_remap(v, ntiles), tile_m, tile_n);
     const int m0 = tile_m * 256, n0 = tile_n * 256;
     cc = 1;
     const unsigned long long t0c = k.probe ? __builtin_readcyclecounter() : 0;
@@ -339,7 +339,7 @@
     const bool more = vn < ntiles;
     if (more) {
       int tm2, tn2;
-      tile_order(k, xcd_remap(vn, ntiles), tm2, tn2);
+      tile_order(k, k.tiles_m, xcd_remap(vn, ntiles), tm2, tn2);
       unsigned a_lane, b_lane;
       lane_ab(a_lane, b_lane);
       a_v = a_lane + (unsigned)(tm2 * 256) * a_row;
diff --git a/geo-deep-learning_amd/csrc/misc.hip b/geo-deep-learning_amd/csrc/misc.hip
--- a/geo-deep-learning_amd/csrc/misc.hip
+++ b/geo-deep-learning_amd/csrc/misc.hip
@@ -1404,3 +1404,64 @@
   GDL_CHECK_LAUNCH("gdl_iou_counts");
   return GDL_OK;
 }
+
+namespace {
+
+__global__ __launch_bounds__(1024) void droppath_live_order_kernel(const float* __restrict__ scales, int B, int tokens,
+                                                                   int* __restrict__ perm, int* __restrict__ counts) {
+  __shared__ int wave_live[16];
+  const int r = blockIdx.x, i = threadIdx.x, lane = i & 63, wave = i >> 6;
+  const bool live = i < B && scales[(int64_t)r * B + i] != 0.f;
+  const unsigned long long mask = __ballot(live);
+  if (lane == 0) wave_live[wave] = __popcll(mask);
+  __syncthreads();
+  int before = 0, total = 0;
+  for (int w = 0; w < 16; ++w) {
+    const int c = wave_live[w];
+    if (w < wave) before += c;
+    total += c;
+  }
+  const int rank = before + __popcll(mask & ((1ull << lane) - 1ull));
+  if (i < B) perm[(int64_t)r * B + (live ? rank : total + (i - rank))] = i;
+  if (i == 0) {
+    counts[2 * r] = total * tokens;
+    counts[2 * r + 1] = total;
+  }
+}
+
+__global__ __launch_bounds__(256) void copy_dropped_samples_kernel(const float4* __restrict__ src, float4* __restrict__ dst,
+                                                                   int64_t sample_vecs, const int* __restrict__ perm,
+                                                                   const int* __restrict__ live) {
+  const int j = blockIdx.y;
+  if (j < *live) return;
+  const int64_t base = (int64_t)perm[j] * sample_vecs;
+  for (int64_t v = (int64_t)blockIdx.x * 256 + threadIdx.x; v < sample_vecs; v += (int64_t)gridDim.x * 256)
+    dst[base + v] = src[base + v];
+}
+
+}
+
+extern "C" int gdl_droppath_live_order(const float* scales, int R, int B, int tokens, int* perm, int* counts,
+                                       gdl_stream_t stream) {
+  GDL_CHECK_ARG(scales && perm && counts, "gdl_droppath_live_order: null pointer");
+  GDL_CHECK_ARG(R > 0 && B > 0 && B <= 1024 && tokens > 0, "gdl_droppath_live_order: needs R > 0, 0 < B <= 1024, tokens > 0");
+  GDL_CHECK_ARG((int64_t)B * tokens < (1ll << 31), "gdl_droppath_live_order: B * tokens must fit 31 bits");
+  hipLaunchKernelGGL(droppath_live_order_kernel, dim3((unsigned)R), dim3(1024), 0, (hipStream_t)stream, scales, B, tokens, perm,
+                     counts);
+  GDL_CHECK_LAUNCH("gdl_droppath_live_order");
+  return GDL_OK;
+}
+
+extern "C" int gdl_copy_dropped_samples(const float* src, float* dst, int B, int64_t sample_elems, const int* perm,
+                                        const int* live, gdl_stream_t stream) {
+  GDL_CHECK_ARG(src && dst && perm && live, "gdl_copy_dropped_samples: null pointer");
+  GDL_CHECK_ARG(B > 0 && B <= 65535 && sample_elems > 0 && sample_elems % 4 == 0, "gdl_copy_dropped_samples: bad dims");
+  GDL_CHECK_ARG(((uintptr_t)src % 16 == 0) && ((uintptr_t)dst % 16 == 0), "gdl_copy_dropped_samples: 16-byte alignment");
+  const int64_t vecs = sample_elems / 4;
+  int64_t chunks = (vecs + 2047) / 2048;
+  if (chunks > 256) chunks = 256;
+  hipLaunchKernelGGL(copy_dropped_samples_kernel, dim3((unsigned)chunks, (unsigned)B), dim3(256), 0, (hipStream_t)stream,
+                     (const float4*)src, (float4*)dst, vecs, perm, live);
+  GDL_CHECK_LAUNCH("gdl_copy_dropped_samples");
+  return GDL_OK;
+}
diff --git a/geo-deep-learning_amd/csrc/norm.hip b/geo-deep-learning_amd/csrc/norm.hip
--- a/geo-deep-learning_amd/csrc/norm.hip
+++ b/geo-deep-learning_amd/csrc/norm.hip
@@ -2,13 +2,14 @@
 
 namespace {
 
-template <int VPL>
+template <int VPL, bool GATHER = false>
 __global__ __launch_bounds__(256) void layernorm_fwd_kernel(const float* __restrict__ x,
                                                             int64_t x_stride,
                                                             const float* __restrict__ gamma,
                                                             const float* __restrict__ beta, void* y,
                                                             int y_dtype, int64_t rows, int D,
-                                                            float eps) {
+                                                            float eps, const int* __restrict__ perm = nullptr,
+                                                            const int* __restrict__ live = nullptr, int n = 0) {
   const int lane = threadIdx.x & 63;
   const int lpp = (VPL == 1 && D <= 128) ? (D <= 64 ? 16 : 32) : 64;
   const int nsub = 64 / lpp, cl = lane % lpp;
@@ -18,7 +19,13 @@
     for (int o = lpp >> 1; o > 0; o >>= 1) t += __shfl_xor(t, o, 64);
     return t;
   };
-  const float* xr = x + row * x_stride;
+  int64_t src_row = row;
+  if constexpr (GATHER) {
+    const int j = (int)(row / n);
+    if (j >= *live) return;
+    src_row = (int64_t)perm[j] * n + (row - (int64_t)j * n);
+  }
+  const float* xr = x + src_row * x_stride;
   float4 v[VPL];
   float s = 0.f;
 #pragma unroll
@@ -966,13 +973,35 @@
   const int rpb = 4 * (D <= 64 ? 4 : (D <= 128 ? 2 : 1));
   const unsigned grid = (unsigned)((rows + rpb - 1) / rpb);
   const int vpl = (D + 255) / 256;
-#define LN_LAUNCH(V) hipLaunchKernelGGL(layernorm_fwd_kernel<V>, dim3(grid), dim3(256), 0, s, x, x_stride, gamma, beta, y, y_dtype, rows, D, eps)
+#define LN_LAUNCH(V) hipLaunchKernelGGL((layernorm_fwd_kernel<V, false>), dim3(grid), dim3(256), 0, s, x, x_stride, gamma, beta, y, y_dtype, rows, D, eps, nullptr, nullptr, 0)
   if (vpl <= 1) LN_LAUNCH(1);
   else if (vpl <= 2) LN_LAUNCH(2);
   else if (vpl <= 4) LN_LAUNCH(4);
   else LN_LAUNCH(8);
 #undef LN_LAUNCH
   GDL_CHECK_LAUNCH("gdl_layernorm_fwd");
+  return GDL_OK;
+}
+
+extern "C" int gdl_layernorm_fwd_gather(const float* x, int64_t x_stride, const float* gamma, const float* beta, void* y,
+                                        int y_dtype, int B, int n, int D, float eps, const int* perm, const int* live,
+                                        gdl_stream_t stream) {
+  GDL_CHECK_ARG(x && gamma && beta && y && perm && live, "gdl_layernorm_fwd_gather: null pointer");
+  GDL_CHECK_ARG(D > 0 && D % 4 == 0 && D <= 2048, "gdl_layernorm_fwd_gather: D=%d must be a multiple of 4, <= 2048", D);
+  GDL_CHECK_ARG(x_stride % 4 == 0, "gdl_layernorm_fwd_gather: x_stride must be a multiple of 4");
+  GDL_CHECK_ARG(B > 0 && n > 0, "gdl_layernorm_fwd_gather: bad dims");
+  hipStream_t s = (hipStream_t)stream;
+  const int64_t rows = (int64_t)B * n;
+  const int rpb = 4 * (D <= 64 ? 4 : (D <= 128 ? 2 : 1));
+  const unsigned grid = (unsigned)((rows + rpb - 1) / rpb);
+  const int vpl = (D + 255) / 256;
+#define LN_LAUNCH(V) hipLaunchKernelGGL((layernorm_fwd_kernel<V, true>), dim3(grid), dim3(256), 0, s, x, x_stride, gamma, beta, y, y_dtype, rows, D, eps, perm, live, n)
+  if (vpl <= 1) LN_LAUNCH(1);
+  else if (vpl <= 2) LN_LAUNCH(2);
+  else if (vpl <= 4) LN_LAUNCH(4);
+  else LN_LAUNCH(8);
+#undef LN_LAUNCH
+  GDL_CHECK_LAUNCH("gdl_layernorm_fwd_gather");
   return GDL_OK;
 }
 
diff --git a/geo-deep-learning_amd/gdlhip/_lib.py b/geo-deep-learning_amd/gdlhip/_lib.py
--- a/geo-deep-learning_amd/gdlhip/_lib.py
+++ b/geo-deep-learning_amd/gdlhip/_lib.py
@@ -28,6 +28,7 @@
         ("in_sZ0", c_l), ("in_sZ1", c_l), ("w_sZ0", c_l), ("w_sZ1", c_l),
         ("out_sZ0", c_l), ("out_sZ1", c_l),
         ("aux_out", c_p), ("stats_partial", c_p),
+        ("live_rows", c_p), ("batch_perm", c_p),
     ]
 
 
@@ -77,6 +78,9 @@
     "gdl_conv_wgrad_workspace": (c_l, [C.POINTER(WgradArgs)]),
     "gdl_conv_wgrad": (c_i, [C.POINTER(WgradArgs), c_p]),
     "gdl_layernorm_fwd": (c_i, [c_p, c_l, c_p, c_p, c_p, c_i, c_l, c_i, c_f, c_p]),
+    "gdl_layernorm_fwd_gather": (c_i, [c_p, c_l, c_p, c_p, c_p, c_i, c_i, c_i, c_i, c_f, c_p, c_p, c_p]),
+    "gdl_droppath_live_order": (c_i, [c_p, c_i, c_i, c_i, c_p, c_p, c_p]),
+    "gdl_copy_dropped_samples": (c_i, [c_p, c_p, c_i, c_l, c_p, c_p, c_p]),
     "gdl_colreduce_workspace": (c_l, [c_l, c_i, c_i]),
     "gdl_layernorm_bwd": (c_i, [c_p, c_l, c_p, c_i, c_p, c_p, c_l, c_p, c_l, c_l, c_i, c_f, c_p, c_p, c_i, c_p, c_l,
                                 c_p]),
@@ -140,6 +144,7 @@
     "gdl_softmax_rows": (c_i, [c_p, c_p, c_i, c_l, c_i, c_i, c_p]),
     "gdl_flash_attn_fwd": (c_i, [c_p, c_l, c_l, c_p, c_l, c_l, c_p, c_p, c_i, c_i, c_i, c_i, c_i, c_f, c_p]),
     "gdl_flash_attn_fwd2": (c_i, [c_p, c_l, c_l, c_p, c_l, c_l, c_p, c_l, c_l, c_p, c_l, c_l, c_p, c_i, c_i, c_i, c_i, c_f, c_p]),
+    "gdl_flash_attn_fwd2_live": (c_i, [c_p, c_l, c_l, c_p, c_l, c_l, c_p, c_l, c_l, c_p, c_l, c_l, c_p, c_i, c_i, c_i, c_i, c_f, c_p, c_p]),
     "gdl_flash_attn_bwd": (c_i, [c_p, c_l, c_l, c_p, c_l, c_l, c_p, c_l, c_l, c_p, c_l, c_l, c_p, c_l, c_l, c_p, c_p,
                                  c_p, c_l, c_l, c_p, c_l, c_l, c_p, c_l, c_l, c_i, c_i, c_i, c_i, c_f, c_p, c_l, c_p]),
     "gdl_flash_attn_bwd_workspace": (c_l, [c_i, c_i, c_i, c_i]),
diff --git a/geo-deep-learning_amd/gdlhip/nn.py b/geo-deep-learning_amd/gdlhip/nn.py
--- a/geo-deep-learning_amd/gdlhip/nn.py
+++ b/geo-deep-learning_amd/gdlhip/nn.py
@@ -30,6 +30,7 @@
 
 
 LAUNCH_FUSION = os.environ.get("GDL_LAUNCH_FUSION", "1") != "0"
+DROPPATH_SKIP = os.environ.get("GDL_DROPPATH_SKIP", "1") != "0"
 _COUNTER_BATCH: list | None = None
 
 
@@ -60,16 +61,28 @@
 _KEEP_CACHE: dict = {}
 
 
-def drop_path_scales(probs: list[float], batch: int, device) -> list[tuple[Tensor | None, Tensor | None]]:
+def drop_path_scales(probs: list[float], batch: int, device, tokens: int | None = None):
+    scales, rows = _drop_path_scales(probs, batch, device)
+    if tokens is None:
+        return scales
+    orders: list = [(None, None)] * len(probs)
+    if rows is not None:
+        lo = ops.droppath_live_order(rows, tokens)
+        for j, i in enumerate(i for i, p_ in enumerate(probs) if p_ > 0.0):
+            orders[i] = (lo[2 * j], lo[2 * j + 1])
+    return scales, orders
+
+
+def _drop_path_scales(probs: list[float], batch: int, device):
     live = [i for i, p_ in enumerate(probs) if p_ > 0.0]
     out: list[tuple[Tensor | None, Tensor | None]] = [(None, None)] * len(probs)
     if not live:
-        return out
+        return out, None
     if not LAUNCH_FUSION:
         for i in live:
             out[i] = tuple((torch.empty(batch, device=device, dtype=torch.float32).bernoulli_(1.0 - probs[i]) / (1.0 - probs[i]))
                            for _ in (0, 1))
-        return out
+        return out, None
     key = (str(device), tuple(probs[i] for i in live))
     keep = _KEEP_CACHE.get(key)
     if keep is None:
@@ -78,7 +91,7 @@
     scales = torch.bernoulli(keep.expand(-1, batch)) / keep
     for j, i in enumerate(live):
         out[i] = (scales[2 * j], scales[2 * j + 1])
-    return out
+    return out, scales
 
 
 def compute_dtype() -> torch.dtype:
diff --git a/geo-deep-learning_amd/gdlhip/ops.py b/geo-deep-learning_amd/gdlhip/ops.py
--- a/geo-deep-learning_amd/gdlhip/ops.py
+++ b/geo-deep-learning_amd/gdlhip/ops.py
@@ -81,7 +81,8 @@
               bias: Tensor | None = None, scale: Tensor | None = None, shift: Tensor | None = None,
               act: int = ACT_NONE, batch_scale: Tensor | None = None, resid: Tensor | None = None,
               out: Tensor | None = None, out_dtype: torch.dtype | None = None,
-              alpha: float = 1.0, aux_out: Tensor | None = None, want_stats: bool = False):
+              alpha: float = 1.0, aux_out: Tensor | None = None, want_stats: bool = False,
+              live: "LiveOrder | None" = None, remap: bool = False):
     _need_cuda(x, w)
     two_d = x.dim() == 2
     x4 = _nhwc4(x, "conv_gemm input")
@@ -126,6 +127,11 @@
             raise ValueError("conv_gemm: aux_out must match out in shape, strides and dtype")
         a.aux_out = x4a.data_ptr()
     a.nz, a.nz_inner = 1, 1
+    if live is not None:
+        if remap and live.perm.numel() != B:
+            raise ValueError(f"conv_gemm: live.perm has {live.perm.numel()} entries for {B} images")
+        a.live_rows = live.rows_ptr
+        a.batch_perm = live.perm.data_ptr() if remap else None
     partials, rows = None, 0
     if want_stats:
         rows = int(_lib.load().gdl_conv_gemm_stats_rows(C.byref(a)))
@@ -308,11 +314,63 @@
     return dw
 
 
-def layernorm(x: Tensor, gamma: Tensor, beta: Tensor, eps: float, out_dtype: torch.dtype) -> Tensor:
+class LiveOrder:
+
+    __slots__ = ("perm", "counts")
+
+    def __init__(self, perm: Tensor, counts: Tensor) -> None:
+        if perm.dtype != torch.int32 or counts.dtype != torch.int32 or not perm.is_contiguous() or counts.numel() != 2 \
+                or not counts.is_contiguous():
+            raise ValueError("LiveOrder: perm / counts must be contiguous int32 ([B] / [2])")
+        _need_cuda(perm, counts)
+        self.perm, self.counts = perm, counts
+
+    @property
+    def rows_ptr(self) -> int:
+        return self.counts.data_ptr()
+
+    @property
+    def live_ptr(self) -> int:
+        return self.counts.data_ptr() + 4
+
+
+def droppath_live_order(scales: Tensor, tokens: int) -> list[LiveOrder]:
+    _need_cuda(scales)
+    if scales.dim() != 2 or scales.dtype != torch.float32 or not scales.is_contiguous():
+        raise ValueError("droppath_live_order: contiguous f32 [R, B] expected")
+    R, B = scales.shape
+    perm = torch.empty((R, B), device=scales.device, dtype=torch.int32)
+    counts = torch.empty((R, 2), device=scales.device, dtype=torch.int32)
+    check(_lib.load().gdl_droppath_live_order(_p(scales), R, B, tokens, _p(perm), _p(counts), _stream()),
+          "gdl_droppath_live_order")
+    return [LiveOrder(perm[r], counts[r]) for r in range(R)]
+
+
+def copy_dropped_samples(src: Tensor, dst: Tensor, live: LiveOrder) -> Tensor:
+    _need_cuda(src, dst)
+    if src.shape != dst.shape or src.dtype != torch.float32 or dst.dtype != torch.float32 or not src.is_contiguous() \
+            or not dst.is_contiguous() or live.perm.numel() != src.shape[0]:
+        raise ValueError("copy_dropped_samples: contiguous f32 tensors of one shape [B, ...] expected")
+    B = src.shape[0]
+    check(_lib.load().gdl_copy_dropped_samples(_p(src), _p(dst), B, src.numel() // B, _p(live.perm), live.live_ptr,
+                                               _stream()), "gdl_copy_dropped_samples")
+    return dst
+
+
+def layernorm(x: Tensor, gamma: Tensor, beta: Tensor, eps: float, out_dtype: torch.dtype,
+              live: LiveOrder | None = None) -> Tensor:
     _need_cuda(x)
     if x.dtype != torch.float32 or x.stride(-1) != 1:
         raise ValueError("layernorm: x must be f32 with unit last stride")
     D = x.shape[-1]
+    if live is not None:
+        if x.dim() != 3 or not x.is_contiguous() or live.perm.numel() != x.shape[0]:
+            raise ValueError("layernorm(live=): contiguous [B, n, D] input and a LiveOrder of B samples expected")
+        y = torch.empty(x.shape, device=x.device, dtype=out_dtype)
+        check(_lib.load().gdl_layernorm_fwd_gather(_p(x), D, _p(_f32vec(gamma, D, "gamma")), _p(_f32vec(beta, D, "beta")),
+                                                   _p(y), dt(y), x.shape[0], x.shape[1], D, eps, _p(live.perm),
+                                                   live.live_ptr, _stream()), "gdl_layernorm_fwd_gather")
+        return y
     x2 = x.reshape(-1, D)
     y = torch.empty((x2.shape[0], D), device=x.device, dtype=out_dtype)
     check(_lib.load().gdl_layernorm_fwd(_p(x2), x2.stride(0), _p(_f32vec(gamma, D, "gamma")),
@@ -978,15 +1036,17 @@
     return out
 
 
-def attention_flash(q: Tensor, k: Tensor, v: Tensor, num_heads: int, return_lse: bool = False):
+def attention_flash(q: Tensor, k: Tensor, v: Tensor, num_heads: int, return_lse: bool = False,
+                    live: LiveOrder | None = None):
     B, Nq, Nkv, D, hd = _attn_check(q, k, v, num_heads)
     if q.dtype != torch.bfloat16 or hd != 64:
         raise ValueError("attention_flash: needs bf16 and head_dim 64")
     out = torch.empty((B, Nq, D), device=q.device, dtype=q.dtype)
     lse = torch.empty((B, num_heads, Nq), device=q.device, dtype=torch.float32) if return_lse else None
-    check(_lib.load().gdl_flash_attn_fwd2(_p(q), q.stride(0), q.stride(1), _p(k), k.stride(0), k.stride(1),
-                                          _p(v), v.stride(0), v.stride(1), _p(out), out.stride(0), out.stride(1),
-                                          _p(lse), B, num_heads, Nq, Nkv, float(hd) ** -0.5, _stream()),
+    check(_lib.load().gdl_flash_attn_fwd2_live(_p(q), q.stride(0), q.stride(1), _p(k), k.stride(0), k.stride(1),
+                                               _p(v), v.stride(0), v.stride(1), _p(out), out.stride(0), out.stride(1),
+                                               _p(lse), B, num_heads, Nq, Nkv, float(hd) ** -0.5,
+                                               None if live is None else live.live_ptr, _stream()),
           "gdl_flash_attn_fwd2")
     return (out, lse) if return_lse else out
 
@@ -1006,9 +1066,9 @@
     return q.dtype == torch.bfloat16 and q.shape[2] // num_heads == 64
 
 
-def attention(q: Tensor, k: Tensor, v: Tensor, num_heads: int, return_lse: bool = False):
+def attention(q: Tensor, k: Tensor, v: Tensor, num_heads: int, return_lse: bool = False, live: LiveOrder | None = None):
     if flash_ok(q, num_heads):
-        return attention_flash(q, k, v, num_heads, return_lse)
+        return attention_flash(q, k, v, num_heads, return_lse, live)
     out = attention_unfused(q, k, v, num_heads)
     return (out, None) if return_lse else out
 
diff --git a/geo-deep-learning_amd/gdlhip/tnn.py b/geo-deep-learning_amd/gdlhip/tnn.py
--- a/geo-deep-learning_amd/gdlhip/tnn.py
+++ b/geo-deep-learning_amd/gdlhip/tnn.py
@@ -5,6 +5,7 @@
 from torch import Tensor
 from torch.autograd import Function
 
+from . import nn as _nn
 from . import ops
 from .nn import cached, conv_weight_matrix, gemm_weight, to_compute
 from .ops import ACT_GELU, ACT_MUL_GELU_GRAD, ACT_NONE
@@ -309,15 +310,46 @@
 class _VitBlock(Function):
 
     @staticmethod
-    def forward(ctx, x, s1, s2, heads, eps, cd, *prm):
+    def _frozen_branches(x, s1, s2, orders, heads, eps, cd, prm, d):
+        n1w, n1b, qkvw, qkvb, pw, pb, g1, n2w, n2b, f1w, f1b, f2w, f2b, g2 = prm
+        b, n, c = x.shape
+        o1, o2 = orders if orders is not None else (None, None)
+
+        def order(s, o):
+            if s is None:
+                return None
+            return o if o is not None else ops.droppath_live_order(s.view(1, b), n)[0]
+        o1, o2 = order(s1, o1), order(s2, o2)
+        h1 = ops.layernorm(x, d[0], d[1], eps, cd, live=o1)
+        qkv = ops.linear(h1, gemm_weight(qkvw, cd), d[3], live=o1)
+        qv, kv_, vv = ops.split_qkv(qkv)
+        a = ops.attention(qv, kv_, vv, heads, live=o1)
+        x1 = torch.empty_like(x)
+        ops.conv_gemm(a.view(b, 1, n, c), gemm_weight(pw, cd), bias=d[5], scale=d[6], batch_scale=s1,
+                      resid=x.view(b, 1, n, c), out=x1.view(b, 1, n, c), live=o1, remap=o1 is not None)
+        if o1 is not None:
+            ops.copy_dropped_samples(x, x1, o1)
+        h2 = ops.layernorm(x1, d[7], d[8], eps, cd, live=o2)
+        f = ops.linear(h2, gemm_weight(f1w, cd), d[10], act=ACT_GELU, live=o2)
+        x2 = torch.empty_like(x)
+        ops.conv_gemm(f.view(b, 1, n, -1), gemm_weight(f2w, cd), bias=d[12], scale=d[13], batch_scale=s2,
+                      resid=x1.view(b, 1, n, c), out=x2.view(b, 1, n, c), live=o2, remap=o2 is not None)
+        if o2 is not None:
+            ops.copy_dropped_samples(x1, x2, o2)
+        return x2
+
+    @staticmethod
+    def forward(ctx, x, s1, s2, orders, heads, eps, cd, *prm):
         n1w, n1b, qkvw, qkvb, pw, pb, g1, n2w, n2b, f1w, f1b, f2w, f2b, g2 = prm
         b, n, c = x.shape
         d = [None if p is None else p.detach() for p in prm]
+        train = any(ctx.needs_input_grad)
+        if not train and (s1 is not None or s2 is not None) and _nn.DROPPATH_SKIP and x.is_contiguous():
+            return _VitBlock._frozen_branches(x, s1, s2, orders, heads, eps, cd, prm, d)
         h1 = ops.layernorm(x, d[0], d[1], eps, cd)
         qkv = ops.linear(h1, gemm_weight(qkvw, cd), d[3])
         qv, kv_, vv = ops.split_qkv(qkv)
         a, lse = ops.attention(qv, kv_, vv, heads, return_lse=True)
-        train = any(ctx.needs_input_grad)
         x1, z1 = torch.empty_like(x), (torch.empty_like(x) if train else None)
         ops.conv_gemm(a.view(b, 1, n, c), gemm_weight(pw, cd), bias=d[5], scale=d[6], batch_scale=s1,
                       resid=x.view(b, 1, n, c), out=x1.view(b, 1, n, c),
@@ -357,12 +389,12 @@
         dqkvw, dqkvb = linear_dw(h1, dqkv)
         dh1 = linear_dx(dqkv, qkvw)
         gx, dn1w, dn1b = ops.layernorm_bwd(x, dh1, n1w.detach(), eps, dres=gx1)
-        return (gx, None, None, None, None, None,
+        return (gx, None, None, None, None, None, None,
                 dn1w, dn1b, dqkvw, dqkvb, dpw, dpb, dg1, dn2w, dn2b, df1w, df1b, df2w, df2b, dg2)
 
 
-def vit_block(x: Tensor, s1, s2, heads: int, eps: float, cd: torch.dtype, params: tuple) -> Tensor:
-    return _VitBlock.apply(x, s1, s2, heads, eps, cd, *params)
+def vit_block(x: Tensor, s1, s2, heads: int, eps: float, cd: torch.dtype, params: tuple, orders=None) -> Tensor:
+    return _VitBlock.apply(x, s1, s2, orders, heads, eps, cd, *params)
 
 
 class _DofaTokens(Function):
diff --git a/geo-deep-learning_amd/geo_deep_learning/models/encoders/dofa_v2.py b/geo-deep-learning_amd/geo_deep_learning/models/encoders/dofa_v2.py
--- a/geo-deep-learning_amd/geo_deep_learning/models/encoders/dofa_v2.py
+++ b/geo-deep-learning_amd/geo_deep_learning/models/encoders/dofa_v2.py
@@ -206,18 +206,19 @@
         return (mask.to(device=device, dtype=torch.float32) / keep).contiguous()
 
     def forward(self, x: Tensor, masks: tuple[Tensor, Tensor] | None = None,
-                scales: tuple[Tensor | None, Tensor | None] | None = None) -> Tensor:
+                scales: tuple[Tensor | None, Tensor | None] | None = None, orders=None) -> Tensor:
         b = x.shape[0]
         if scales is not None and masks is None:
             s1, s2 = scales
         else:
+            orders = None
             s1 = self._drop_scale(b, x.device, None if masks is None else masks[0])
             s2 = self._drop_scale(b, x.device, None if masks is None else masks[1])
         at, m = self.attn, self.mlp
         prm = (self.norm1.weight, self.norm1.bias, at.qkv.weight, at.qkv.bias, at.proj.weight, at.proj.bias,
                self.ls1.gamma, self.norm2.weight, self.norm2.bias, m.fc1.weight, m.fc1.bias, m.fc2.weight, m.fc2.bias,
                self.ls2.gamma)
-        return tnn.vit_block(x, s1, s2, at.num_heads, self.norm1.eps, gnn.compute_dtype(), prm)
+        return tnn.vit_block(x, s1, s2, at.num_heads, self.norm1.eps, gnn.compute_dtype(), prm, orders)
 
 
 class DOFAv2(nn.Module):
@@ -415,11 +416,16 @@
             wq, bias = self._dynamic_operands(wavelengths, x.device, cd)
         cols = ops.patchify(ops.image_f32(x, "DOFAv2"), k, 1, gh, gw, wq.shape[1], cd)
         tok = tnn.dofa_tokens(cols.view(b, n, -1), wq, bias, self.cls_token, self.pos_embed)
-        scales = None
+        scales = orders = None
         if self.training and drop_masks is None:
-            scales = gnn.drop_path_scales([blk.drop_prob for blk in self.blocks], b, tok.device)
+            probs = [blk.drop_prob for blk in self.blocks]
+            if gnn.DROPPATH_SKIP and not (torch.is_grad_enabled() and any(p.requires_grad for p in self.blocks.parameters())):
+                scales, orders = gnn.drop_path_scales(probs, b, tok.device, tokens=n + 1)
+            else:
+                scales = gnn.drop_path_scales(probs, b, tok.device)
         for i, blk in enumerate(self.blocks):
-            tok = blk(tok, None if drop_masks is None else drop_masks[i], None if scales is None else scales[i])
+            tok = blk(tok, None if drop_masks is None else drop_masks[i], None if scales is None else scales[i],
+                      None if orders is None else orders[i])
             yield i, tok
 
     def forward_features_nhwc(self, x: Tensor, wavelengths: Tensor, drop_masks=None) -> list[Tensor]:
diff --git a/include/gdlhip.h b/include/gdlhip.h
--- a/include/gdlhip.h
+++ b/include/gdlhip.h
@@ -52,6 +52,8 @@
   int64_t in_sZ0, in_sZ1, w_sZ0, w_sZ1, out_sZ0, out_sZ1;
   void* aux_out;
   float* stats_partial;
+  const int* live_rows;
+  const int* batch_perm;
 } gdl_conv_args;
 
 int gdl_conv_gemm(const gdl_conv_args* a, gdl_stream_t stream);
@@ -81,6 +83,12 @@
 
 int gdl_layernorm_fwd(const float* x, int64_t x_stride, const float* gamma, const float* beta,
                       void* y, int y_dtype, int64_t rows, int D, float eps, gdl_stream_t stream);
+int gdl_layernorm_fwd_gather(const float* x, int64_t x_stride, const float* gamma, const float* beta, void* y, int y_dtype,
+                             int B, int n, int D, float eps, const int* perm, const int* live, gdl_stream_t stream);
+
+int gdl_droppath_live_order(const float* scales, int R, int B, int tokens, int* perm, int* counts, gdl_stream_t stream);
+int gdl_copy_dropped_samples(const float* src, float* dst, int B, int64_t sample_elems, const int* perm, const int* live,
+                             gdl_stream_t stream);
 
 int gdl_bn_stats(const void* x, int dtype, int64_t P, int C, int64_t x_sP, float* mean,
                  float* var_biased, float* running_mean, float* running_var, float momentum,
@@ -231,6 +239,9 @@
 int gdl_flash_attn_fwd2(const void* q, int64_t q_sB, int64_t q_sN, const void* k, int64_t k_sB, int64_t k_sN,
                         const void* v, int64_t v_sB, int64_t v_sN, void* o, int64_t o_sB, int64_t o_sN, float* lse,
                         int B, int H, int Nq, int Nkv, float scale, gdl_stream_t stream);
+int gdl_flash_attn_fwd2_live(const void* q, int64_t q_sB, int64_t q_sN, const void* k, int64_t k_sB, int64_t k_sN,
+                             const void* v, int64_t v_sB, int64_t v_sN, void* o, int64_t o_sB, int64_t o_sN, float* lse,
+                             int B, int H, int Nq, int Nkv, float scale, const int* live_batch, gdl_stream_t stream);
 int gdl_flash_attn_bwd(const void* q, int64_t q_sB, int64_t q_sN, const void* k, int64_t k_sB, int64_t k_sN,
                        const void* v, int64_t v_sB, int64_t v_sN, const void* o, int64_t o_sB, int64_t o_sN,
                        const void* dout, int64_t do_sB, int64_t do_sN, const float* lse, float* dvec,
```
